# rubengooj/stvo-pl

Hardware: AMD Instinct MI355X
Metric: stereo frames/s (match+optimizePose) (higher is better)
Workload: dtype u8/fp4+f64; 1 GPU; BASELINE configs[2]: KITTI-00-shaped stereo with points + lines (ORB + LBD rows), grid-windowed stereo match (points and lines) + f2f brute-force mutual-NNR match (points and lines) + full GN optimizePose (config_kitti.yaml), device-resident per-frame pipeline; the streams cycle through the 8 sequence ids / 3 KITTI calibrations of configs[4] (sequence s on rank s mod G); streams_per_gpu=3072, parallelism=seq-shard x1

## Files before the change

stvo-pl_amd/csrc/ctx_internal.h:

```cpp
#pragma once
#include <hip/hip_runtime.h>

#include <cstdio>
#include <cstring>
#include <vector>

#include "kernels.h"

struct stvo_ctx {
    int device = 0;
    hipStream_t stream = nullptr;
    bool own_stream = false;
    bool stream_retained = false;
    int max_rows = 0, max_batch = 0;
    uint2* knn12 = nullptr;
    uint2* knn21 = nullptr;
    size_t knn_capacity = 0;
    int32_t *cand = nullptr, *need = nullptr, *qsel = nullptr, *nsel = nullptr;
    char* arena = nullptr;
    char* arena_host = nullptr;
    size_t arena_size = 0, arena_off = 0, upload_hi = 0;
    uint32_t* probe_sink = nullptr;
    int overlap = 0;
    hipStream_t aux_stream = nullptr;
    hipEvent_t ev_match_done = nullptr, ev_pose_done = nullptr;
    bool pose_pending = false;
    int timing = 0;
    std::vector<hipEvent_t> ev_pool;
    size_t ev_used = 0;
    char last_error[256] = {0};
};

namespace stvo_detail {

inline bool hip_ok(stvo_ctx* ctx, hipError_t e, const char* what) {
    if (e == hipSuccess) return true;
    if (ctx) std::snprintf(ctx->last_error, sizeof(ctx->last_error), "%s: %s", what, hipGetErrorString(e));
    return false;
}
#define HIP_TRY(ctx, call)                                   \
    do {                                                     \
        if (!hip_ok((ctx), (call), #call)) return STVO_ERR_HIP; \
    } while (0)

inline bool zero_device(stvo_ctx* ctx, void* p, size_t bytes, const char* what) {
    return hip_ok(ctx, hipMemsetAsync(p, 0, bytes, ctx->stream), what) && hip_ok(ctx, hipStreamSynchronize(ctx->stream), what);
}

inline bool upload_now(stvo_ctx* ctx, void* dst, const void* src, size_t bytes, const char* what) {
    return hip_ok(ctx, hipMemcpyAsync(dst, src, bytes, hipMemcpyHostToDevice, ctx->stream), what) && hip_ok(ctx, hipStreamSynchronize(ctx->stream), what);
}

template <typename T>
inline T* arena_alloc(stvo_ctx* ctx, size_t count) {
    size_t bytes = (count * sizeof(T) + 255) & ~size_t(255);
    if (bytes == 0) bytes = 256;
    if (ctx->arena_off + bytes > ctx->arena_size) return nullptr;
    T* p = reinterpret_cast<T*>(ctx->arena + ctx->arena_off);
    ctx->arena_off += bytes;
    return p;
}

template <typename T>
inline int upload(stvo_ctx* ctx, T** dst, const T* src, size_t count, size_t count_alloc = 0) {
    *dst = arena_alloc<T>(ctx, count_alloc > count ? count_alloc : count);
    if (!*dst) return STVO_ERR_CAPACITY;
    if (count && src) {
        const size_t off = (size_t)(reinterpret_cast<char*>(*dst) - ctx->arena);
        std::memcpy(ctx->arena_host + off, src, count * sizeof(T));
        if (off + count * sizeof(T) > ctx->upload_hi) ctx->upload_hi = off + count * sizeof(T);
    }
    return STVO_OK;
}

inline int flush_uploads(stvo_ctx* ctx) {
    if (ctx->upload_hi) {
        if (ctx->upload_hi <= ((size_t)4 << 20))
            stvo::launch_copy16(ctx->stream, ctx->arena_host, ctx->arena, ctx->upload_hi);
        else
            HIP_TRY(ctx, hipMemcpyAsync(ctx->arena, ctx->arena_host, ctx->upload_hi, hipMemcpyHostToDevice, ctx->stream));
        ctx->upload_hi = 0;
    }
    return STVO_OK;
}

inline int download_begin(stvo_ctx* ctx, const void* dev, size_t bytes) {
    const size_t off = (size_t)(reinterpret_cast<const char*>(dev) - ctx->arena);
    if (bytes == 0) return STVO_OK;
    if (bytes <= ((size_t)256 << 10) && (off & 15) == 0)
        stvo::launch_copy16(ctx->stream, dev, ctx->arena_host + off, bytes);
    else
        HIP_TRY(ctx, hipMemcpyAsync(ctx->arena_host + off, dev, bytes, hipMemcpyDeviceToHost, ctx->stream));
    return STVO_OK;
}
template <typename T>
inline const T* host_mirror(stvo_ctx* ctx, const T* dev) {
    return reinterpret_cast<const T*>(ctx->arena_host + (reinterpret_cast<const char*>(dev) - ctx->arena));
}
#define TRY(expr)                \
    do {                         \
        int _rc = (expr);        \
        if (_rc != STVO_OK) return _rc; \
    } while (0)

inline int check_launch(stvo_ctx* ctx) {
    HIP_TRY(ctx, hipGetLastError());
    return STVO_OK;
}

}
using namespace stvo_detail;
```

stvo-pl_amd/csrc/kernels.h:

```cpp
#pragma once

#include <hip/hip_runtime.h>
#include <stdint.h>

#include <cstdlib>
#include <map>
#include <mutex>
#include <utility>

#include "../../include/stvo_hip.h"
#include "debug_switches.h"
#include "point_tail.h"

namespace stvo {

inline bool lds_opt_in(const void* kernel, int bytes) {
    static std::mutex mu;
    static std::map<std::pair<const void*, int>, int> granted;
    int dev = 0;
    if (hipGetDevice(&dev) != hipSuccess) return false;
    std::lock_guard<std::mutex> lk(mu);
    const auto key = std::make_pair(kernel, dev);
    const auto it = granted.find(key);
    if (it != granted.end() && (it->second >= bytes || it->second < 0)) return it->second >= bytes;
    const bool ok = hipFuncSetAttribute(kernel, hipFuncAttributeMaxDynamicSharedMemorySize, bytes) == hipSuccess;
    if (ok) granted[key] = bytes;
    else if (it == granted.end()) granted[key] = -1;
    return ok;
}

constexpr int KNN_MIN_NSEG = 2, KNN_MAX_NSEG = 16;
inline int knn_pick_nseg(int B, int max_n, size_t capacity) {
    const int tiles = (max_n + 255) / 256;
    int nseg = (2048 + B * tiles - 1) / (B * tiles > 0 ? B * tiles : 1);
    nseg = nseg < KNN_MIN_NSEG ? KNN_MIN_NSEG : (nseg > KNN_MAX_NSEG ? KNN_MAX_NSEG : nseg);
    if ((long long)B * tiles >= 4096) nseg = 1;
    if (dbg().knn_nseg != DBG_UNSET && dbg().knn_nseg > 0) nseg = dbg().knn_nseg;
    const size_t per_seg = (size_t)(B > 0 ? B : 1) * (size_t)(max_n > 0 ? max_n : 1);
    while (nseg > 1 && (size_t)nseg * per_seg > capacity) --nseg;
    return nseg;
}

inline int device_cu_count() {
    static std::mutex mu;
    static std::map<int, int> cus;
    int dev = 0;
    if (hipGetDevice(&dev) != hipSuccess) return 256;
    std::lock_guard<std::mutex> lk(mu);
    const auto it = cus.find(dev);
    if (it != cus.end()) return it->second;
    int n = 0;
    if (hipDeviceGetAttribute(&n, hipDeviceAttributeMultiprocessorCount, dev) != hipSuccess || n <= 0) n = 256;
    cus[dev] = n;
    return n;
}

void launch_hamming_knn2(hipStream_t s, int B, int row_stride, int max_n, const uint8_t* d1, const int32_t* n1,
                         const uint8_t* d2, const int32_t* n2, uint2* knn12, uint2* knn21, int both_directions,
                         int lds_pad_bytes = 0, int dir0 = 0, const int32_t* qsel = nullptr,
                         const int32_t* nsel = nullptr, int nseg = KNN_MIN_NSEG, uint32_t* claim_init = nullptr);
constexpr int REV_MAX_SEG = 8;
__host__ __device__ inline int rev_segments(int train_rows) {
    const int s = (train_rows + 255) / 256;
    return s < 1 ? 1 : (s > REV_MAX_SEG ? REV_MAX_SEG : s);
}
void launch_hamming_knn2_mfma_reverse(hipStream_t s, int B, int row_stride, const uint8_t* d1, const int32_t* n1, const uint8_t* d2, const int32_t* qsel,
                                      const int32_t* nsel, const int32_t* tsel, const uint32_t* claim, float nnr, int32_t* m12, int slots);
void launch_hamming_knn2_mfma(hipStream_t s, int B, int row_stride, int max_n, const uint8_t* d1, const int32_t* n1,
                              const uint8_t* d2, const int32_t* n2, uint2* knn12, uint2* knn21, int both_directions,
                              int dir0, const int32_t* qsel, const int32_t* nsel, int nseg, uint32_t* claim_init, int qb,
                              int qsel_from_back = 0, const int32_t* tsel = nullptr, const int32_t* ntsel = nullptr);
int knn_mfma_qb(int max_n);
struct LazyScratch {
    uint2* knn12;
    uint2* knn21;
    int32_t* cand;
    int32_t* need;
    int32_t* qsel;
    int32_t* nsel;
    size_t knn_capacity;
};
void launch_match_mutual_lazy(hipStream_t s, int B, int row_stride, const uint8_t* d1, const int32_t* n1,
                              const uint8_t* d2, const int32_t* n2, float nnr, const LazyScratch& w, int32_t* m12,
                              int lds_pad_bytes, hipEvent_t wait_before_m12_write, hipEvent_t* timing_events = nullptr);
void launch_hamming_verify(hipStream_t s, int B, int row_stride, const uint8_t* d1, const int32_t* n1, const uint8_t* d2,
                           float nnr, const LazyScratch& w, int lds_pad_bytes, int nseg, int32_t* m12);
bool match_small_ok(int row_stride);
void launch_match_small(hipStream_t s, int B, int row_stride, const uint8_t* d1, const int32_t* n1, const uint8_t* d2,
                        const int32_t* n2, float nnr, int mutual, int32_t* m12, int cap = 0 );
void launch_nnr_mutual(hipStream_t s, int B, int row_stride, const uint2* knn12, const uint2* knn21, const int32_t* n1,
                       const int32_t* n2, float nnr, int mutual, int32_t* m12, int nseg = KNN_MIN_NSEG);
void launch_valu_probe(hipStream_t s, int blocks, int iters, uint32_t* sink);
void launch_copy16(hipStream_t s, const void* src, void* dst, size_t bytes);
extern const double kValuProbeOpsPerThreadIter;

struct PoseArgs {
    int B, max_pts, max_lines;
    const int32_t* n_prev_pts;
    const double* prev_P;
    const double* prev_s2p;
    const double* curr_pl;
    const int32_t* m12p;
    const int32_t* init_inl_p;
    const int32_t* n_prev_lines;
    const double* prev_sP;
    const double* prev_eP;
    const double* prev_spl;
    const double* prev_epl;
    const double* prev_s2l;
    const double* curr_le;
    const int32_t* m12l;
    const int32_t* init_inl_l;
    const double* init_T;
    double* next_T;
    stvo_cam cam;
    const stvo_cam* cams;
    int lds_cap_pts, lds_cap_lines;
    stvo_opt_params prm;
    stvo_pose_result* results;
    int32_t* inl_p_out;
    int32_t* inl_l_out;
    int eval_only;
    int eval_robust;
    double* eval_out;
    long long* prof_out;
    const float4* prev_rc;
    const float4* curr_rc;
    const double* q_tab;
    double level_scale;
    const unsigned* wait_flag;
    unsigned wait_value;
    int lazy_eig;
    int lines_on_solver;
    const uint4* fetch_src;
    uint4* fetch_dst;
    unsigned fetch_n16;
    unsigned* fetch_flag;
    unsigned fetch_value;
    unsigned* start_flag;
    unsigned start_value;
};
bool pose_start_flag_ok(const PoseArgs& a);
void launch_stream_gate(hipStream_t s, const unsigned* flag, unsigned value);
constexpr int STVO_POSE_QTAB = 16;
constexpr int PATH_EIG_PENDING = 1 << 30;
bool pose_inline_sync_ok(int B);
void launch_stream_signal(hipStream_t s, unsigned* flag, unsigned value);
int launch_pose(hipStream_t s, const PoseArgs& a);
int launch_pose2p(hipStream_t s, const PoseArgs& a);
void pose2p_retain_stream(hipStream_t s);
void pose2p_release_stream(hipStream_t s);
inline void pose_retain_stream(hipStream_t s) { pose2p_retain_stream(s); }
inline void pose_release_stream(hipStream_t s) { pose2p_release_stream(s); }

void launch_blur7_u8(hipStream_t s, int B, int cols, int rows, const uint8_t* src, uint8_t* dst, const int* k7);
void launch_resize_linear_u8(hipStream_t s, int B, int scols, int srows, int dcols, int drows, const uint8_t* src, uint8_t* dst, double fx = 0.0,
                             double fy = 0.0);

constexpr int GRID_LW = STVO_GRID_COLS + 16, GRID_LCELLS = STVO_GRID_ROWS * GRID_LW, GRID_LSTART_STRIDE = GRID_LCELLS + 4;
struct PointCells {
    int K, ws;
    const float* kp_l;
    const float* kp_r;
    const int32_t* n_kp_l;
    const int32_t* n_kp_r;
    const double* inv_wh;
    int32_t* pstart;
    uint32_t* plstart;
    int32_t* plperm;
    int32_t* pperm;
    int32_t* pcell;
    int32_t* pxy_l;
    unsigned long long* top2_p;
    int32_t* govf_p;
    int32_t* prange;
    int32_t* pitems;
    int32_t* prank;
};

struct GridBatch {
    int B, stride1, stride2;
    int xy_width;
    int items_stride;
    int words64, n1p;
    const int32_t* cell_xy1;
    const uint8_t* d1;
    const int32_t* n1;
    const int32_t* cell_start;
    const int32_t* cell_items;
    const uint8_t* d2;
    const int32_t* n2;
    const double* dir2;
    stvo_grid_window w;
    double ratio, line_sim_th;
    int mutual;
    unsigned long long* cover;
    const int32_t* rank;
    const int32_t* perm;
    unsigned long long* top2;
    int32_t* owner2;
    int32_t* m12;
    int range_points;
    const int32_t* range1;
    const int32_t* cell2;
    const uint32_t* lstart;
    const int32_t* lperm;
    uint32_t* elig;
    int32_t* elig_cnt;
    int32_t* ovf;
    int32_t* misfit;
    int lean_cells;
    int has_tail;
    PointTail tail;
    int fused_cells;
    PointCells cells;
};
constexpr int GRID_ELIG = 16;
void launch_grid_batch(hipStream_t s, const GridBatch& g, bool lines, hipEvent_t* scan_events = nullptr);
bool grid_points_fused_ok(const GridBatch& g);
void launch_grid_range_debug(hipStream_t s, const GridBatch& g);

}
```

stvo-pl_amd/csrc/match_kernels.hip:

```cpp
#include "kernels.h"

#include <stdlib.h>

namespace stvo {

__device__ __forceinline__ uint32_t med3_u32(uint32_t a, uint32_t b, uint32_t c) {
    uint32_t r;
    asm("v_med3_u32 %0, %1, %2, %3" : "=v"(r) : "v"(a), "v"(b), "v"(c));
    return r;
}

__device__ __forceinline__ uint32_t bcnt_acc(uint32_t x, uint32_t acc) {
    uint32_t r;
    asm("v_bcnt_u32_b32 %0, %1, %2" : "=v"(r) : "v"(x), "v"(acc));
    return r;
}
__device__ __forceinline__ uint32_t pack_key(uint32_t d, uint32_t j_uniform) {
    uint32_t r;
    asm("v_lshl_or_b32 %0, %1, 16, %2" : "=v"(r) : "v"(d), "s"(j_uniform));
    return r;
}
__device__ __forceinline__ uint32_t bcnt0(uint32_t x) {
    uint32_t r;
    asm("v_bcnt_u32_b32 %0, %1, 0" : "=v"(r) : "v"(x));
    return r;
}

__device__ __forceinline__ uint32_t hamming256(const uint4& q0, const uint4& q1, const uint32_t* __restrict__ t) {
    uint32_t d = bcnt0(q0.x ^ t[0]);
    d = bcnt_acc(q0.y ^ t[1], d);
    d = bcnt_acc(q0.z ^ t[2], d);
    d = bcnt_acc(q0.w ^ t[3], d);
    d = bcnt_acc(q1.x ^ t[4], d);
    d = bcnt_acc(q1.y ^ t[5], d);
    d = bcnt_acc(q1.z ^ t[6], d);
    d = bcnt_acc(q1.w ^ t[7], d);
    return d;
}

constexpr int KNN_BLOCK = 256;

__device__ __forceinline__ uint2 merged_knn(const uint2* __restrict__ knn, size_t seg_stride, size_t idx, int nseg) {
    uint2 r = knn[idx];
    for (int sgm = 1; sgm < nseg; ++sgm) {
        const uint2 o = knn[(size_t)sgm * seg_stride + idx];
        const uint32_t hi = r.x > o.x ? r.x : o.x;
        uint32_t sec = r.y < o.y ? r.y : o.y;
        sec = sec < hi ? sec : hi;
        r.x = r.x < o.x ? r.x : o.x;
        r.y = sec;
    }
    return r;
}

__global__ __launch_bounds__(KNN_BLOCK) void hamming_knn2_kernel(int B, int tiles, int ndir, int dir0, int nseg, int row_stride,
                                                                 const uint8_t* __restrict__ d1,
                                                                 const int32_t* __restrict__ n1,
                                                                 const uint8_t* __restrict__ d2,
                                                                 const int32_t* __restrict__ n2,
                                                                 uint2* __restrict__ knn12, uint2* __restrict__ knn21,
                                                                 const int32_t* __restrict__ qsel,
                                                                 const int32_t* __restrict__ nsel,
                                                                 uint32_t* __restrict__ claim_init) {
    const int per_frame = tiles * ndir * nseg;
    const int L = blockIdx.x;
    const int xcd = L & 7, k = L >> 3;
    const int b = (k / per_frame) * 8 + xcd;
    if (b >= B) return;
    const int local = k % per_frame;
    const int seg = local % nseg;
    const int dir = dir0 + (local / nseg) / tiles;
    const int tile = (local / nseg) % tiles;
    const int na = n1[b], nb = n2[b];
    const int nq = qsel ? nsel[b] : (dir == 0 ? na : nb);
    const int nt_all = dir == 0 ? nb : na;
    const int seg_len = (((nt_all + nseg - 1) / nseg) + 3) & ~3;
    const int j0 = min(seg * seg_len, nt_all);
    const int nt = min(j0 + seg_len, nt_all);
    const int q_base = tile * KNN_BLOCK;
    const size_t frame_off = (size_t)b * row_stride;
    if (claim_init && seg == 0 && dir == dir0 && q_base + (int)threadIdx.x < row_stride)
        claim_init[frame_off + q_base + threadIdx.x] = 0xFFFFFFFFu;
    if (q_base + (int)(threadIdx.x & ~63u) >= nq) return;
    const uint8_t* Q = (dir == 0 ? d1 : d2) + frame_off * STVO_DESC_BYTES;
    const uint32_t* __restrict__ T = reinterpret_cast<const uint32_t*>((dir == 0 ? d2 : d1) + frame_off * STVO_DESC_BYTES);
    uint2* __restrict__ out = (dir == 0 ? knn12 : knn21) + (size_t)seg * B * row_stride + frame_off;

    const int q = q_base + threadIdx.x;
    const int qc = q < nq ? q : nq - 1;
    const int qi = qsel ? qsel[frame_off + qc] : qc;
    const uint4 q0 = reinterpret_cast<const uint4*>(Q)[2 * qi];
    const uint4 q1 = reinterpret_cast<const uint4*>(Q)[2 * qi + 1];

    uint32_t best = 0xFFFFFFFFu, second = 0xFFFFFFFFu;
    uint32_t second_d = 0xFFFFu;
    int j = j0;
    auto update = [&](uint32_t d, uint32_t jj) {
        if (__builtin_amdgcn_ballot_w64(d < second_d) != 0ull) {
            const uint32_t key = pack_key(d, jj);
            second = med3_u32(best, second, key);
            best = best < key ? best : key;
            second_d = second >> 16;
        }
    };
    for (; j + 4 <= nt; j += 4) {
        uint32_t t[32];
#pragma unroll
        for (int k = 0; k < 32; ++k) t[k] = T[8 * j + k];
        uint32_t d[4];
#pragma unroll
        for (int u = 0; u < 4; ++u) d[u] = hamming256(q0, q1, t + 8 * u);
#pragma unroll
        for (int u = 0; u < 4; ++u) update(d[u], (uint32_t)(j + u));
    }
    for (; j < nt; ++j) update(hamming256(q0, q1, T + 8 * j), (uint32_t)j);
    if (q < nq) out[qi] = make_uint2(best, second);
}

int knn_mfma_qb(int max_n) {
    const int qb = dbg().knn_mfma != DBG_UNSET ? dbg().knn_mfma : 2;
    return max_n <= 8192 ? qb : 0;
}

void launch_hamming_knn2(hipStream_t s, int B, int row_stride, int max_n, const uint8_t* d1, const int32_t* n1,
                         const uint8_t* d2, const int32_t* n2, uint2* knn12, uint2* knn21, int both_directions,
                         int lds_pad_bytes, int dir0, const int32_t* qsel, const int32_t* nsel, int nseg, uint32_t* claim_init) {
    if (B <= 0 || max_n <= 0) return;
    const int mfma_qb = knn_mfma_qb(max_n);
    if (mfma_qb > 0) {
        launch_hamming_knn2_mfma(s, B, row_stride, max_n, d1, n1, d2, n2, knn12, knn21, both_directions, dir0, qsel, nsel, nseg,
                                 claim_init, mfma_qb);
        return;
    }
    const int tiles = (max_n + KNN_BLOCK - 1) / KNN_BLOCK, ndir = both_directions ? 2 : 1;
    const int groups = (B + 7) / 8;
    dim3 grid((unsigned)(groups * 8 * tiles * ndir * nseg));
    hipLaunchKernelGGL(hamming_knn2_kernel, grid, dim3(KNN_BLOCK), (size_t)lds_pad_bytes, s, B, tiles, ndir, dir0,
                       nseg, row_stride, d1, n1, d2, n2, knn12, knn21, qsel, nsel, claim_init);
}

__global__ __launch_bounds__(256) void nnr_mutual_kernel(int nseg, int row_stride, const uint2* __restrict__ knn12,
                                                         const uint2* __restrict__ knn21,
                                                         const int32_t* __restrict__ n1, const int32_t* __restrict__ n2,
                                                         float nnr, int mutual, int32_t* __restrict__ m12) {
    const int b = blockIdx.y;
    const int i = blockIdx.x * 256 + threadIdx.x;
    if (i >= row_stride) return;
    const int na = n1[b], nb = n2[b];
    const size_t off = (size_t)b * row_stride;
    int m = -1;
    if (i < na && nb >= 2) {
        const uint2 k = merged_knn(knn12, (size_t)gridDim.y * row_stride, off + i, nseg);
        const float f0 = (float)(k.x >> 16), f1 = (float)(k.y >> 16);
        if (f0 < f1 * nnr) m = (int)(k.x & 0xFFFFu);
        if (mutual && m >= 0) {
            bool keep = false;
            if (na >= 2) {
                const uint2 r = merged_knn(knn21, (size_t)gridDim.y * row_stride, off + m, nseg);
                const float r0 = (float)(r.x >> 16), r1 = (float)(r.y >> 16);
                keep = (r0 < r1 * nnr) && ((int)(r.x & 0xFFFFu) == i);
            }
            if (!keep) m = -1;
        }
    }
    m12[off + i] = m;
}

void launch_nnr_mutual(hipStream_t s, int B, int row_stride, const uint2* knn12, const uint2* knn21, const int32_t* n1,
                       const int32_t* n2, float nnr, int mutual, int32_t* m12, int nseg) {
    if (B <= 0 || row_stride <= 0) return;
    dim3 grid((row_stride + 255) / 256, B);
    hipLaunchKernelGGL(nnr_mutual_kernel, grid, dim3(256), 0, s, nseg, row_stride, knn12, knn21, n1, n2, nnr, mutual, m12);
}

__global__ __launch_bounds__(256) void nnr_forward_kernel(int nseg, int row_stride, const uint2* __restrict__ knn12,
                                                          const int32_t* __restrict__ n1, const int32_t* __restrict__ n2,
                                                          float nnr, int32_t* __restrict__ cand,
                                                          uint32_t* __restrict__ claim ) {
    const int b = blockIdx.y;
    const int i = blockIdx.x * 256 + threadIdx.x;
    if (i >= row_stride) return;
    const int na = n1[b], nb = n2[b];
    const size_t off = (size_t)b * row_stride;
    int m = -1;
    if (i < na && nb >= 2) {
        const uint2 k = merged_knn(knn12, (size_t)gridDim.y * row_stride, off + i, nseg);
        const float f0 = (float)(k.x >> 16), f1 = (float)(k.y >> 16);
        if (f0 < f1 * nnr) {
            m = (int)(k.x & 0xFFFFu);
            atomicMin(&claim[off + m], (k.x & 0xFFFF0000u) | (uint32_t)i);
        }
    }
    cand[off + i] = m;
}

__global__ __launch_bounds__(256) void compact_need_kernel(int row_stride, const uint32_t* __restrict__ claim,
                                                           const int32_t* __restrict__ n2, int32_t* __restrict__ qsel,
                                                           int32_t* __restrict__ nsel, int32_t* __restrict__ blocked) {
    __shared__ int s_wave[4];
    const int b = blockIdx.x, tid = threadIdx.x, lane = tid & 63, wv = tid >> 6;
    const size_t off = (size_t)b * row_stride;
    const int nb = n2[b];
    const int per = (row_stride + 255) / 256;
    const int lo = tid * per, hi = min(lo + per, nb);
    int cnt = 0;
    for (int j = lo; j < hi; ++j) cnt += claim[off + j] != 0xFFFFFFFFu;
    int incl = cnt;
#pragma unroll
    for (int o = 1; o < 64; o <<= 1) {
        const int v = __shfl_up(incl, o, 64);
        if (lane >= o) incl += v;
    }
    if (lane == 63) s_wave[wv] = incl;
    __syncthreads();
    int base = 0, tot = 0;
#pragma unroll
    for (int w = 0; w < 4; ++w) {
        if (w < wv) base += s_wave[w];
        tot += s_wave[w];
    }
    int pos = base + incl - cnt;
    for (int j = lo; j < hi; ++j)
        if (claim[off + j] != 0xFFFFFFFFu) {
            qsel[off + pos++] = j;
            blocked[off + j] = 0;
        }
    if (tid == 0) nsel[b] = tot;
}

__device__ __forceinline__ uint32_t hamming128_lo(const uint4& q0, const uint32_t* __restrict__ t) {
    uint32_t d = bcnt0(q0.x ^ t[0]);
    d = bcnt_acc(q0.y ^ t[1], d);
    d = bcnt_acc(q0.z ^ t[2], d);
    d = bcnt_acc(q0.w ^ t[3], d);
    return d;
}
__device__ __forceinline__ uint32_t hamming128_hi(const uint4& q1, const uint32_t* __restrict__ t, uint32_t d) {
    d = bcnt_acc(q1.x ^ t[4], d);
    d = bcnt_acc(q1.y ^ t[5], d);
    d = bcnt_acc(q1.z ^ t[6], d);
    d = bcnt_acc(q1.w ^ t[7], d);
    return d;
}

__global__ __launch_bounds__(KNN_BLOCK) void hamming_verify_kernel(int B, int tiles, int nseg, int row_stride,
                                                                   const uint8_t* __restrict__ d1,
                                                                   const int32_t* __restrict__ n1,
                                                                   const uint8_t* __restrict__ d2,
                                                                   const uint32_t* __restrict__ claim,
                                                                   const int32_t* __restrict__ qsel,
                                                                   const int32_t* __restrict__ nsel, float nnr,
                                                                   int32_t* __restrict__ blocked) {
    const int per_frame = tiles * nseg;
    const int L = blockIdx.x;
    const int xcd = L & 7, k = L >> 3;
    const int b = (k / per_frame) * 8 + xcd;
    if (b >= B) return;
    const int local = k % per_frame;
    const int seg = local % nseg;
    const int tile = local / nseg;
    const int nq = nsel[b];
    const int nt_all = n1[b];
    const int seg_len = (((nt_all + nseg - 1) / nseg) + 3) & ~3;
    const int j0 = min(seg * seg_len, nt_all);
    const int nt = min(j0 + seg_len, nt_all);
    const int q_base = tile * KNN_BLOCK;
    if (q_base + (int)(threadIdx.x & ~63u) >= nq) return;
    const size_t frame_off = (size_t)b * row_stride;
    const uint32_t* __restrict__ T = reinterpret_cast<const uint32_t*>(d1 + frame_off * STVO_DESC_BYTES);

    const int q = q_base + threadIdx.x;
    const int qc = q < nq ? q : nq - 1;
    const int qi = qsel[frame_off + qc];
    const uint4 q0 = reinterpret_cast<const uint4*>(d2 + frame_off * STVO_DESC_BYTES)[2 * qi];
    const uint4 q1 = reinterpret_cast<const uint4*>(d2 + frame_off * STVO_DESC_BYTES)[2 * qi + 1];
    const uint32_t c = claim[frame_off + qi];
    const uint32_t istar = c & 0xFFFFu;
    uint32_t thr = c >> 16;
    {
        const float f0 = (float)thr;
        while (thr < 256u && !(f0 < (float)(thr + 1u) * nnr)) ++thr;
    }
    bool blk = false;
    auto step4 = [&](const uint32_t* __restrict__ t, int jb) {
        uint32_t p[4];
#pragma unroll
        for (int u = 0; u < 4; ++u) p[u] = hamming128_lo(q0, t + 8 * u);
        unsigned long long any = 0ull;
#pragma unroll
        for (int u = 0; u < 4; ++u) any |= __builtin_amdgcn_ballot_w64(p[u] <= thr);
        if (any != 0ull) {
            unsigned long long other = 0ull;
#pragma unroll
            for (int u = 0; u < 4; ++u) other |= __builtin_amdgcn_ballot_w64(p[u] <= thr && (uint32_t)(jb + u) != istar);
            if (other != 0ull) {
#pragma unroll
                for (int u = 0; u < 4; ++u) {
                    const uint32_t d = hamming128_hi(q1, t + 8 * u, p[u]);
                    blk = blk || (d <= thr && (uint32_t)(jb + u) != istar);
                }
            }
        }
    };
    int j = j0;
    if (j + 4 <= nt) {
        uint32_t ta[32], tb[32];
#pragma unroll
        for (int w = 0; w < 32; ++w) ta[w] = T[8 * j + w];
        for (; j + 8 <= nt; j += 8) {
#pragma unroll
            for (int w = 0; w < 32; ++w) tb[w] = T[8 * (j + 4) + w];
            step4(ta, j);
            const int jn = (j + 12 <= nt) ? j + 8 : j;
#pragma unroll
            for (int w = 0; w < 32; ++w) ta[w] = T[8 * jn + w];
            step4(tb, j + 4);
        }
        if (j + 4 <= nt) {
            step4(ta, j);
            j += 4;
        }
    }
    for (; j < nt; ++j) {
        const uint32_t d = hamming256(q0, q1, T + 8 * j);
        blk = blk || (d <= thr && (uint32_t)j != istar);
    }
    if (q < nq && blk) blocked[frame_off + qi] = 1;
}

__global__ __launch_bounds__(1024) void nnr_reverse_check_kernel(int row_stride, const uint32_t* __restrict__ claim,
                                                                 const int32_t* __restrict__ blocked, const int32_t* __restrict__ n1,
                                                                 int32_t* __restrict__ m12) {
    const int b = blockIdx.x;
    const size_t off = (size_t)b * row_stride;
    for (int i = threadIdx.x; i < row_stride; i += 1024) m12[off + i] = -1;
    __syncthreads();
    if (n1[b] < 2) return;
    for (int j = threadIdx.x; j < row_stride; j += 1024) {
        const uint32_t c = claim[off + j];
        if (c != 0xFFFFFFFFu && blocked[off + j] == 0) m12[off + (c & 0xFFFFu)] = j;
    }
}

__device__ __forceinline__ uint32_t block_threshold(uint32_t d0, float nnr) {
    const float f0 = (float)d0;
    uint32_t thr = d0;
    while (thr < 256u && !(f0 < (float)(thr + 1u) * nnr)) ++thr;
    return thr;
}

constexpr int PLAN_BLOCK = 512;
__global__ __launch_bounds__(PLAN_BLOCK) void forward_plan_kernel(int B, int nseg, int row_stride, uint2* __restrict__ knn12,
                                                                  const int32_t* __restrict__ n1,
                                                                  const int32_t* __restrict__ n2, float nnr,
                                                                  int32_t* __restrict__ m12, uint32_t* __restrict__ claim_g,
                                                                  int32_t* __restrict__ qsel, int32_t* __restrict__ tsel,
                                                                  int32_t* __restrict__ nsel) {
    extern __shared__ uint32_t plan_lds[];
    uint32_t* claim = plan_lds;
    uint16_t* Tc = reinterpret_cast<uint16_t*>(claim + row_stride);
    uint8_t* blk = reinterpret_cast<uint8_t*>(Tc + row_stride);
    __shared__ int hT[257], hS[257], s_cnt[3];
    __shared__ unsigned long long s_best;
    const int b = blockIdx.x, tid = threadIdx.x;
    const size_t off = (size_t)b * row_stride;
    const int na = n1[b], nb = n2[b];
    for (int j = tid; j < row_stride; j += PLAN_BLOCK) {
        claim[j] = 0xFFFFFFFFu;
        blk[j] = 0;
    }
    if (tid < 257) hT[tid] = hS[tid] = 0;
    if (tid < 3) s_cnt[tid] = 0;
    if (tid == 0) s_best = ~0ull;
    __syncthreads();
    const bool active = nb >= 2 && na >= 1;
    for (int i = tid; i < row_stride; i += PLAN_BLOCK) {
        if (active && i < na) {
            const uint2 k = merged_knn(knn12, (size_t)B * row_stride, off + i, nseg);
            if (nseg > 1) knn12[off + i] = k;
            const float f0 = (float)(k.x >> 16), f1 = (float)(k.y >> 16);
            if (f0 < f1 * nnr) atomicMin(&claim[k.x & 0xFFFFu], (k.x & 0xFFFF0000u) | (uint32_t)i);
        }
        m12[off + i] = -1;
    }
    __syncthreads();
    for (int j = tid; j < row_stride; j += PLAN_BLOCK) {
        const uint32_t c = claim[j];
        claim_g[off + j] = c;
        if (c != 0xFFFFFFFFu) {
            const uint32_t T = block_threshold(c >> 16, nnr);
            Tc[j] = (uint16_t)T;
            atomicAdd(&hT[T], 1);
        }
    }
    __syncthreads();
    if (active)
        for (int i = tid; i < na; i += PLAN_BLOCK) {
            const uint2 k = knn12[off + i];
            const uint32_t key[2] = {k.x, k.y};
#pragma unroll
            for (int e = 0; e < 2; ++e) {
                if (key[e] == 0xFFFFFFFFu) continue;
                const uint32_t j = key[e] & 0xFFFFu, c = claim[j];
                if (c != 0xFFFFFFFFu && (c & 0xFFFFu) != (uint32_t)i && (key[e] >> 16) <= (uint32_t)Tc[j]) blk[j] = 1;
            }
            if (k.y != 0xFFFFFFFFu) atomicAdd(&hS[min(k.y >> 16, 256u)], 1);
        }
    __syncthreads();
    if (tid < 64) {
        int vT[5], vS[5], sT = 0, sS = 0;
#pragma unroll
        for (int e = 0; e < 5; ++e) {
            const int t = tid * 5 + e;
            vT[e] = t < 257 ? hT[t] : 0;
            vS[e] = t < 257 ? hS[t] : 0;
            sT += vT[e];
            sS += vS[e];
        }
        int iT = sT, iS = sS;
#pragma unroll
        for (int o = 1; o < 64; o <<= 1) {
            const int a = __shfl_up(iT, o, 64), c = __shfl_up(iS, o, 64);
            if (tid >= o) {
                iT += a;
                iS += c;
            }
        }
        int eT = iT - sT, eS = iS - sS;
#pragma unroll
        for (int e = 0; e < 5; ++e) {
            const int t = tid * 5 + e;
            if (t < 257) {
                hT[t] = eT;
                hS[t] = eS;
            }
            eT += vT[e];
            eS += vS[e];
        }
        if (tid == 63) s_cnt[0] = iT;
    }
    __syncthreads();
    if (tid < 256) {
        const int C = s_cnt[0], cT = hT[tid], cS = hS[tid];
        const unsigned long long cost = (unsigned long long)(C - cT) * (unsigned)na + (unsigned long long)cT * (unsigned)cS;
        atomicMin(&s_best, (cost << 9) | (unsigned)tid);
    }
    __syncthreads();
    if (tid == 0) s_cnt[0] = 0;
    __syncthreads();
    const int tau = (int)(s_best & 511ull) - 1;
    for (int j = tid; j < row_stride; j += PLAN_BLOCK) {
        const uint32_t c = claim[j];
        if (c == 0xFFFFFFFFu) continue;
        if (!blk[j] && na >= 2) m12[off + (c & 0xFFFFu)] = j;
        if ((int)Tc[j] <= tau)
            qsel[off + atomicAdd(&s_cnt[0], 1)] = j;
        else
            qsel[off + row_stride - 1 - atomicAdd(&s_cnt[1], 1)] = j;
    }
    if (active)
        for (int i = tid; i < na; i += PLAN_BLOCK) {
            const uint2 k = knn12[off + i];
            if (k.y != 0xFFFFFFFFu && (int)(k.y >> 16) <= tau) tsel[off + atomicAdd(&s_cnt[2], 1)] = i;
        }
    __syncthreads();
    if (tid == 0) {
        nsel[b] = s_cnt[0] + s_cnt[1];
        nsel[(size_t)B + b] = s_cnt[0];
        nsel[2 * (size_t)B + b] = s_cnt[1];
        nsel[3 * (size_t)B + b] = s_cnt[2];
        nsel[4 * (size_t)B + b] = tau;
    }
}

struct ReversePlan {
    int32_t* tsel;
};
constexpr int KNN_REV_SLOTS = 4;
static ReversePlan reverse_plan(const LazyScratch& w, int B, int row_stride) {
    const size_t per = (size_t)B * row_stride;
    ReversePlan p;
    p.tsel = reinterpret_cast<int32_t*>(w.knn21 + (w.knn_capacity - per)) + per;
    return p;
}

static void launch_reverse_scans(hipStream_t s, int B, int row_stride, const uint8_t* d1, const int32_t* n1, const uint8_t* d2, float nnr,
                                 const LazyScratch& w, const ReversePlan& rp, int32_t* m12) {
    launch_hamming_knn2_mfma_reverse(s, B, row_stride, d1, n1, d2, w.qsel, w.nsel, rp.tsel, reinterpret_cast<const uint32_t*>(w.need), nnr, m12,
                                     KNN_REV_SLOTS);
}

void launch_hamming_verify(hipStream_t s, int B, int row_stride, const uint8_t* d1, const int32_t* n1, const uint8_t* d2,
                           float nnr, const LazyScratch& w, int lds_pad_bytes, int nseg, int32_t* m12) {
    if (B <= 0 || row_stride <= 0) return;
    const int mfma_qb = knn_mfma_qb(row_stride);
    if (mfma_qb > 0) {
        launch_reverse_scans(s, B, row_stride, d1, n1, d2, nnr, w, reverse_plan(w, B, row_stride), m12);
        return;
    }
    const int tiles = (row_stride + KNN_BLOCK - 1) / KNN_BLOCK, groups = (B + 7) / 8;
    hipLaunchKernelGGL(hamming_verify_kernel, dim3((unsigned)(groups * 8 * tiles * nseg)), dim3(KNN_BLOCK),
                       (size_t)lds_pad_bytes, s, B, tiles, nseg, row_stride, d1, n1, d2,
                       reinterpret_cast<const uint32_t*>(w.need), w.qsel, w.nsel, nnr, reinterpret_cast<int32_t*>(w.knn21));
}

void launch_match_mutual_lazy(hipStream_t s, int B, int row_stride, const uint8_t* d1, const int32_t* n1,
                              const uint8_t* d2, const int32_t* n2, float nnr, const LazyScratch& w, int32_t* m12,
                              int lds_pad_bytes, hipEvent_t wait_before_m12_write, hipEvent_t* tev) {
    if (B <= 0 || row_stride <= 0) return;
    const dim3 grid2((row_stride + 255) / 256, B);
    const int nseg = knn_pick_nseg(B, row_stride, w.knn_capacity);
    uint32_t* claim = reinterpret_cast<uint32_t*>(w.need);
    int32_t* blocked = reinterpret_cast<int32_t*>(w.knn21);
    if (tev) (void)hipEventRecord(tev[0], s);
    launch_hamming_knn2(s, B, row_stride, row_stride, d1, n1, d2, n2, w.knn12, w.knn21, 0, lds_pad_bytes, 0, nullptr,
                        nullptr, nseg, knn_mfma_qb(row_stride) > 0 ? nullptr : claim);
    if (tev) (void)hipEventRecord(tev[1], s);
    const int mfma_qb = knn_mfma_qb(row_stride);
    if (mfma_qb > 0) {
        const ReversePlan rp = reverse_plan(w, B, row_stride);
        if (wait_before_m12_write) (void)hipStreamWaitEvent(s, wait_before_m12_write, 0);
        if (tev && tev[2]) (void)hipEventRecord(tev[2], s);
        hipLaunchKernelGGL(forward_plan_kernel, dim3(B), dim3(PLAN_BLOCK), (size_t)row_stride * 7, s, B, nseg, row_stride, w.knn12,
                           n1, n2, nnr, m12, claim, w.qsel, rp.tsel, w.nsel);
        launch_reverse_scans(s, B, row_stride, d1, n1, d2, nnr, w, rp, m12);
        if (tev && tev[3]) (void)hipEventRecord(tev[3], s);
        return;
    }
    hipLaunchKernelGGL(nnr_forward_kernel, grid2, dim3(256), 0, s, nseg, row_stride, w.knn12, n1, n2, nnr, w.cand, claim);
    hipLaunchKernelGGL(compact_need_kernel, dim3(B), dim3(256), 0, s, row_stride, claim, n2, w.qsel, w.nsel, blocked);
    if (tev && tev[2]) (void)hipEventRecord(tev[2], s);
    launch_hamming_verify(s, B, row_stride, d1, n1, d2, nnr, w, lds_pad_bytes, nseg, m12);
    if (tev && tev[3]) (void)hipEventRecord(tev[3], s);
    if (wait_before_m12_write) (void)hipStreamWaitEvent(s, wait_before_m12_write, 0);
    hipLaunchKernelGGL(nnr_reverse_check_kernel, dim3(B), dim3(1024), 0, s, row_stride, claim, blocked, n1, m12);
}

const double kValuProbeOpsPerThreadIter = 19.0 * 8.0;

__global__ __launch_bounds__(256) void valu_probe_kernel(int iters, uint32_t* sink) {
    uint4 q0 = make_uint4(threadIdx.x * 2654435761u, blockIdx.x * 40503u + 1u, 0x9E3779B9u ^ threadIdx.x, 0x85EBCA6Bu);
    uint4 q1 = make_uint4(q0.y * 3u, q0.z * 5u, q0.w * 7u, q0.x * 11u);
    uint32_t best = 0xFFFFFFFFu, second = 0xFFFFFFFFu;
    uint32_t t[8];
    const uint32_t seed = __builtin_amdgcn_readfirstlane(blockIdx.x * 7919u + 13u);
#pragma unroll
    for (int k = 0; k < 8; ++k) t[k] = seed * (2 * k + 3);
    for (int it = 0; it < iters; ++it) {
#pragma unroll
        for (int u = 0; u < 8; ++u) {
#pragma unroll
            for (int k = 0; k < 8; ++k) t[k] = __builtin_amdgcn_readfirstlane(t[k] + 0x01010101u * (k + 1));
            const uint32_t d = hamming256(q0, q1, t);
            const uint32_t key = pack_key(d, (uint32_t)(it * 8 + u));
            second = med3_u32(best, second, key);
            best = best < key ? best : key;
        }
    }
    if ((best ^ second) == 0x12345u) sink[0] = best;
}

__global__ __launch_bounds__(256) void copy16_kernel(const uint4* __restrict__ src, uint4* __restrict__ dst, size_t n16) {
    for (size_t i = (size_t)blockIdx.x * 256 + threadIdx.x; i < n16; i += (size_t)gridDim.x * 256) dst[i] = src[i];
}

void launch_copy16(hipStream_t s, const void* src, void* dst, size_t bytes) {
    const size_t n16 = (bytes + 15) / 16;
    if (n16 == 0) return;
    const size_t blocks = (n16 + 255) / 256;
    hipLaunchKernelGGL(copy16_kernel, dim3((unsigned)(blocks < 256 ? blocks : 256)), dim3(256), 0, s,
                       reinterpret_cast<const uint4*>(src), reinterpret_cast<uint4*>(dst), n16);
}

void launch_valu_probe(hipStream_t s, int blocks, int iters, uint32_t* sink) {
    hipLaunchKernelGGL(valu_probe_kernel, dim3(blocks), dim3(256), 0, s, iters, sink);
}

__global__ __launch_bounds__(256) void match_small_kernel(int row_stride, int cap, const uint8_t* __restrict__ d1,
                                                          const int32_t* __restrict__ n1, const uint8_t* __restrict__ d2,
                                                          const int32_t* __restrict__ n2, float nnr, int mutual,
                                                          int32_t* __restrict__ m12) {
    extern __shared__ uint2 s_knn[];
    const int b = blockIdx.x, tid = threadIdx.x, lane = tid & 63;
    const int na = min(n1[b], cap), nb = min(n2[b], cap);
    const size_t off = (size_t)b * row_stride;
    uint2* k12 = s_knn;
    uint2* k21 = s_knn + cap;
    const int tiles_a = (na + 63) >> 6, tiles_b = mutual ? (nb + 63) >> 6 : 0;
    for (int item = tid >> 6; item < tiles_a + tiles_b; item += 4) {
        const int it = __builtin_amdgcn_readfirstlane(item);
        const bool fwd = it < tiles_a;
        const int q = (fwd ? it : it - tiles_a) * 64 + lane;
        const int nq = fwd ? na : nb, nt = fwd ? nb : na;
        const uint8_t* Q = (fwd ? d1 : d2) + off * STVO_DESC_BYTES;
        const uint32_t* __restrict__ T = reinterpret_cast<const uint32_t*>((fwd ? d2 : d1) + off * STVO_DESC_BYTES);
        const int qc = q < nq ? q : nq - 1;
        const uint4 q0 = reinterpret_cast<const uint4*>(Q)[2 * qc];
        const uint4 q1 = reinterpret_cast<const uint4*>(Q)[2 * qc + 1];
        uint32_t best = 0xFFFFFFFFu, second = 0xFFFFFFFFu;
        auto update = [&](uint32_t d, uint32_t jj) {
            const uint32_t key = pack_key(d, jj);
            second = med3_u32(best, second, key);
            best = best < key ? best : key;
        };
        int j = 0;
        for (; j + 4 <= nt; j += 4) {
            uint32_t t[32];
#pragma unroll
            for (int k = 0; k < 32; ++k) t[k] = T[8 * j + k];
            uint32_t d[4];
#pragma unroll
            for (int u = 0; u < 4; ++u) d[u] = hamming256(q0, q1, t + 8 * u);
#pragma unroll
            for (int u = 0; u < 4; ++u) update(d[u], (uint32_t)(j + u));
        }
        for (; j < nt; ++j) update(hamming256(q0, q1, T + 8 * j), (uint32_t)j);
        if (q < nq) (fwd ? k12 : k21)[q] = make_uint2(best, second);
    }
    __syncthreads();
    for (int i = tid; i < row_stride; i += 256) {
        int m = -1;
        if (i < na && nb >= 2) {
            const uint2 fk = k12[i];
            const float f0 = (float)(fk.x >> 16), f1 = (float)(fk.y >> 16);
            if (f0 < f1 * nnr) m = (int)(fk.x & 0xFFFFu);
            if (mutual && m >= 0) {
                bool keep = false;
                if (na >= 2) {
                    const uint2 rk = k21[m];
                    const float r0 = (float)(rk.x >> 16), r1 = (float)(rk.y >> 16);
                    keep = (r0 < r1 * nnr) && ((int)(rk.x & 0xFFFFu) == i);
                }
                if (!keep) m = -1;
            }
        }
        m12[off + i] = m;
    }
}

bool match_small_ok(int row_stride) { return row_stride > 0 && row_stride <= 512; }

void launch_match_small(hipStream_t s, int B, int row_stride, const uint8_t* d1, const int32_t* n1, const uint8_t* d2,
                        const int32_t* n2, float nnr, int mutual, int32_t* m12, int cap) {
    if (B <= 0 || !match_small_ok(row_stride)) return;
    if (cap <= 0 || cap > row_stride) cap = row_stride;
    const size_t lds = (size_t)cap * 2 * sizeof(uint2);
    hipLaunchKernelGGL(match_small_kernel, dim3(B), dim3(256), lds, s, row_stride, cap, d1, n1, d2, n2, nnr, mutual, m12);
}

}
```

stvo-pl_amd/csrc/match_mfma.hip:

```cpp
#include <type_traits>

#include "kernels.h"

namespace stvo {

typedef int v4i __attribute__((ext_vector_type(4)));
typedef int v8i __attribute__((ext_vector_type(8)));
typedef int v16i __attribute__((ext_vector_type(16)));
typedef float v16f __attribute__((ext_vector_type(16)));

#ifndef MF_TPB
#define MF_TPB 2
#endif
#ifndef MF_FOLD_SLOTS
#define MF_FOLD_SLOTS 5
#endif
constexpr int MF_BLOCK = 256;
constexpr int MF_TILE = 32;
constexpr int MF_KEY_SHIFT = 13;
constexpr int MF_KEY_BIAS = 1 << 20;
constexpr int MF_NO_KEY = 0x7FFFFFFF;
constexpr int MF_NO_KEY_MIN = 0x40000000;

__device__ __forceinline__ v4i expand_fp4(uint32_t w) {
    v4i r;
    r.x = (int)(((w << 3) & 0x88888888u) | 0x66666666u);
    r.y = (int)(((w << 2) & 0x88888888u) | 0x66666666u);
    r.z = (int)(((w << 1) & 0x88888888u) | 0x66666666u);
    r.w = (int)((w & 0x88888888u) | 0x66666666u);
    return r;
}
__device__ __forceinline__ float med3_f32(float a, float b, float c) {
    float r;
    asm("v_med3_f32 %0, %1, %2, %3" : "=v"(r) : "v"(a), "v"(b), "v"(c));
    return r;
}
__device__ __forceinline__ float min_f32(float a, float b) {
    float r;
    asm("v_min_f32 %0, %1, %2" : "=v"(r) : "v"(a), "v"(b));
    return r;
}
__device__ __forceinline__ float max_f32(float a, float b) {
    float r;
    asm("v_max_f32 %0, %1, %2" : "=v"(r) : "v"(a), "v"(b));
    return r;
}
__device__ __forceinline__ float min3_f32(float a, float b, float c) {
    float r;
    asm("v_min3_f32 %0, %1, %2, %3" : "=v"(r) : "v"(a), "v"(b), "v"(c));
    return r;
}
constexpr float MF_NO_KEY_F = 1.0e30f;
constexpr float MF_NO_KEY_MIN_F = 1.0e29f;
constexpr int MF_SCALE_2_4 = 127 + 4;

__device__ __forceinline__ uint32_t key_to_knn(int key, int base) {
    if (key >= MF_NO_KEY_MIN) return 0xFFFFFFFFu;
    const uint32_t u = (uint32_t)(key + base + MF_KEY_BIAS);
    return ((u >> MF_KEY_SHIFT) << 16) | (u & ((1u << MF_KEY_SHIFT) - 1u));
}

template <int QB, int MODE>
__global__ __launch_bounds__(MF_BLOCK, (QB == 1 ? 4 : QB == 2 ? 3 : 1)) void hamming_knn2_mfma_kernel(int B, int tiles, int ndir, int dir0, int nseg, int row_stride,
                                                                      const uint8_t* __restrict__ d1,
                                                                      const int32_t* __restrict__ n1,
                                                                      const uint8_t* __restrict__ d2,
                                                                      const int32_t* __restrict__ n2,
                                                                      uint2* __restrict__ knn12, uint2* __restrict__ knn21,
                                                                      const int32_t* __restrict__ qsel,
                                                                      const int32_t* __restrict__ nsel,
                                                                      uint32_t* __restrict__ claim_init, int qsel_from_back,
                                                                      const int32_t* __restrict__ tsel,
                                                                      const int32_t* __restrict__ ntsel) {
    constexpr bool GATHER = MODE >= 1, TGATHER = MODE == 2;
    constexpr int ROWS = 4 * QB * 32;
    constexpr int KSTEPS = 4;
    using key_t = float;
    using acc_t = v16f;
    constexpr int NBUF = 2 * MF_TPB;
    __shared__ v4i s_tile[NBUF][KSTEPS * 2 * 32];
    const int per_frame = tiles * ndir * nseg;
    const int L = blockIdx.x;
    const int xcd = L & 7, k = L >> 3;
    int fb = k / per_frame, local = k % per_frame;
    if (MODE == 0 && ndir == 1 && tiles > 1) {
        const int groups = (int)(gridDim.x >> 3) / per_frame;
        const int full_pf = (tiles - 1) * nseg, full = full_pf * groups;
        if (k < full) {
            fb = k / full_pf;
            local = k % full_pf;
        } else {
            fb = (k - full) / nseg;
            local = full_pf + (k - full) % nseg;
        }
    }
    const int b = fb * 8 + xcd;
    if (b >= B) return;
    const int seg = local % nseg;
    const int dir = dir0 + (local / nseg) / tiles;
    const int tile = (local / nseg) % tiles;
    const size_t frame_off = (size_t)b * row_stride;
    const int tid = threadIdx.x, lane = tid & 63, wv = tid >> 6, col = lane & 31, hf = lane >> 5;
    const int q_base = tile * ROWS;
    const uint32_t* __restrict__ Q = reinterpret_cast<const uint32_t*>((dir == 0 ? d1 : d2) + frame_off * STVO_DESC_BYTES);
    uint4 qw[QB][2];
    if (!GATHER) {
#pragma unroll
        for (int qb = 0; qb < QB; ++qb) {
            const int qi = min(q_base + (wv * QB + qb) * 32 + col, row_stride - 1);
            qw[qb][0] = reinterpret_cast<const uint4*>(Q)[2 * qi];
            qw[qb][1] = reinterpret_cast<const uint4*>(Q)[2 * qi + 1];
        }
    }
    const int na = n1[b], nb = n2[b];
    const int nq = GATHER ? nsel[b] : (dir == 0 ? na : nb);
    const int nt_all = TGATHER ? ntsel[b] : (dir == 0 ? nb : na);
    if (TGATHER && nt_all == 0) return;
    const int seg_len = (((nt_all + nseg - 1) / nseg) + MF_TILE - 1) & ~(MF_TILE - 1);
    const int j0 = min(seg * seg_len, nt_all);
    const int nt = min(j0 + seg_len, nt_all);
    if (claim_init && seg == 0 && dir == dir0)
        for (int c = q_base + tid; c < min(q_base + ROWS, row_stride); c += MF_BLOCK) claim_init[frame_off + c] = 0xFFFFFFFFu;
    if (q_base >= nq) return;
    const uint32_t* __restrict__ T = reinterpret_cast<const uint32_t*>((dir == 0 ? d2 : d1) + frame_off * STVO_DESC_BYTES);
    uint2* __restrict__ out = (dir == 0 ? knn12 : knn21) + (size_t)seg * B * row_stride + frame_off;

    const bool wave_active = q_base + wv * QB * 32 < nq;
    v4i qf[QB][KSTEPS];
    auto query_row = [&](int qb) {
        const int q = q_base + (wv * QB + qb) * 32 + col;
        const int qc = q < nq ? q : nq - 1;
        return GATHER ? qsel[frame_off + (qsel_from_back ? row_stride - 1 - qc : qc)] : qc;
    };
    if (GATHER) {
#pragma unroll
        for (int qb = 0; qb < QB; ++qb) {
            const int qi = query_row(qb);
            qw[qb][0] = reinterpret_cast<const uint4*>(Q)[2 * qi];
            qw[qb][1] = reinterpret_cast<const uint4*>(Q)[2 * qi + 1];
        }
    }
#pragma unroll
    for (int qb = 0; qb < QB; ++qb) {
        const uint32_t w[8] = {qw[qb][0].x, qw[qb][0].y, qw[qb][0].z, qw[qb][0].w, qw[qb][1].x, qw[qb][1].y, qw[qb][1].z, qw[qb][1].w};
        const bool up = hf != 0;
        qf[qb][0] = expand_fp4(~(up ? w[1] : w[0]));
        qf[qb][1] = expand_fp4(~(up ? w[3] : w[2]));
        qf[qb][2] = expand_fp4(~(up ? w[5] : w[4]));
        qf[qb][3] = expand_fp4(~(up ? w[7] : w[6]));
    }
    acc_t cidx;
#pragma unroll
    for (int r = 0; r < 16; ++r) cidx[r] = (key_t)((r & 3) + 8 * (r >> 2) + 4 * hf);

    const key_t no_key = MF_NO_KEY_F;
    key_t best[QB], second[QB];
#pragma unroll
    for (int qb = 0; qb < QB; ++qb) best[qb] = second[qb] = no_key;

    const int xr = tid & 31, xk = tid >> 5;
    const int ntiles = (nt - j0 + MF_TILE - 1) / MF_TILE;
    auto fetch = [&](int t) -> uint32_t {
        const int j = j0 + t * MF_TILE + xr;
        if (j >= nt) return 0u;
        const int row = TGATHER ? tsel[frame_off + j] : j;
        return T[(size_t)row * 8 + xk];
    };
    auto stage = [&](int t, uint32_t w) {
        s_tile[t & (NBUF - 1)][xk * 32 + xr] = expand_fp4(w);
    };
#pragma unroll
    for (int i = 0; i < MF_TPB; ++i)
        if (i < ntiles) stage(i, fetch(i));
    __syncthreads();
    auto rebase = [&]() {
#pragma unroll
        for (int qb = 0; qb < QB; ++qb) {
            best[qb] -= (key_t)MF_TILE;
            second[qb] -= (key_t)MF_TILE;
        }
    };
    auto fold = [&](int qb, key_t key) {
        second[qb] = med3_f32(best[qb], second[qb], key);
        best[qb] = min_f32(best[qb], key);
    };
    auto mma = [&](const v4i& tf, const v4i& q, const acc_t& c) -> acc_t {
        const v8i a8 = {tf.x, tf.y, tf.z, tf.w, 0, 0, 0, 0}, b8 = {q.x, q.y, q.z, q.w, 0, 0, 0, 0};
        return __builtin_amdgcn_mfma_scale_f32_32x32x64_f8f6f4(a8, b8, c, 4, 4, 0, MF_SCALE_2_4, 0, MF_SCALE_2_4);
    };
    auto mma_fold = [&](acc_t (&cur)[QB], acc_t (&prev)[QB], int t) {
        if (wave_active) {
            const v4i* frag = s_tile[t & (NBUF - 1)];
            const bool fold_prev = t > 0;
            if (fold_prev) rebase();
            key_t node[QB][5];
            v4i tf = frag[lane];
#pragma unroll
            for (int kk = 0; kk < KSTEPS; ++kk) {
                v4i tf_ahead = tf;
                if (kk < KSTEPS - 1) tf_ahead = frag[(kk + 1) * 64 + lane];
#pragma unroll
                for (int qb = 0; qb < QB; ++qb) cur[qb] = mma(tf, qf[qb][kk], kk == 0 ? cidx : cur[qb]);
                if (fold_prev) {
                    if (QB == 1 && kk == 0) asm volatile("s_nop 7\n\ts_nop 7\n\ts_nop 2" : "+v"(prev[0]));
#pragma unroll
                    for (int qb = 0; qb < QB; ++qb) {
                        const acc_t& p = prev[qb];
                        key_t(&a)[5] = node[qb];
                        if (kk == 0) {
                            a[0] = min3_f32(p[0], p[1], p[2]);
                            a[1] = min3_f32(p[3], p[4], p[5]);
                            second[qb] = min3_f32(second[qb], med3_f32(p[0], p[1], p[2]), med3_f32(p[3], p[4], p[5]));
                        } else if (kk == 1) {
                            a[2] = min3_f32(p[6], p[7], p[8]);
                            a[3] = min3_f32(p[9], p[10], p[11]);
                            second[qb] = min3_f32(second[qb], med3_f32(p[6], p[7], p[8]), med3_f32(p[9], p[10], p[11]));
                        } else if (kk == 2) {
                            a[4] = min3_f32(p[12], p[13], p[14]);
                            const key_t b0 = min3_f32(a[0], a[1], a[2]);
                            second[qb] = min3_f32(second[qb], med3_f32(p[12], p[13], p[14]), med3_f32(a[0], a[1], a[2]));
                            a[0] = b0;
                        } else {
                            const key_t b1 = min3_f32(a[3], a[4], p[15]), n1 = med3_f32(a[3], a[4], p[15]);
                            second[qb] = min3_f32(second[qb], n1, med3_f32(a[0], b1, best[qb]));
                            best[qb] = min3_f32(a[0], b1, best[qb]);
                        }
                    }
                }
                if (kk < KSTEPS - 1) __builtin_amdgcn_sched_group_barrier(0x100, 1, 0);
#pragma unroll
                for (int qb = 0; qb < QB; ++qb) {
                    __builtin_amdgcn_sched_group_barrier(0x008, 1, 0);
                    __builtin_amdgcn_sched_group_barrier(0x002, MF_FOLD_SLOTS, 0);
                }
                tf = tf_ahead;
            }
        }
    };
    acc_t accA[QB], accB[QB];
#pragma unroll
    for (int qb = 0; qb < QB; ++qb)
#pragma unroll
        for (int r = 0; r < 16; ++r) accA[qb][r] = accB[qb][r] = 0;
    static_assert(MF_TPB % 2 == 0, "the accumulator sets alternate tile by tile");
    int t = 0;
    uint32_t w_near[MF_TPB];
#pragma unroll
    for (int i = 0; i < MF_TPB; ++i) {
        w_near[i] = 0;
        if (MF_TPB + i < ntiles) w_near[i] = fetch(MF_TPB + i);
    }
    for (; t + MF_TPB <= ntiles; t += MF_TPB) {
        uint32_t w_far[MF_TPB];
#pragma unroll
        for (int i = 0; i < MF_TPB; ++i) {
            w_far[i] = 0;
            if (t + 2 * MF_TPB + i < ntiles) w_far[i] = fetch(t + 2 * MF_TPB + i);
        }
#pragma unroll
        for (int i = 0; i < MF_TPB; ++i) {
            if ((i & 1) == 0) mma_fold(accA, accB, t + i);
            else mma_fold(accB, accA, t + i);
        }
#pragma unroll
        for (int i = 0; i < MF_TPB; ++i) {
            if (t + MF_TPB + i < ntiles) stage(t + MF_TPB + i, w_near[i]);
            w_near[i] = w_far[i];
        }
        __syncthreads();
    }
#pragma unroll
    for (int i = 0; i < MF_TPB - 1; ++i)
        if (t + i < ntiles) {
            if ((i & 1) == 0) mma_fold(accA, accB, t + i);
            else mma_fold(accB, accA, t + i);
        }
    if (wave_active && ntiles > 0) {
        const int jt = j0 + (ntiles - 1) * MF_TILE;
        const acc_t(&last)[QB] = (ntiles & 1) ? accA : accB;
        rebase();
#pragma unroll
        for (int qb = 0; qb < QB; ++qb)
#pragma unroll
            for (int r = 0; r < 16; ++r) {
                const int jr = jt + (r & 3) + 8 * (r >> 2) + 4 * hf;
                fold(qb, jr < nt ? last[qb][r] : no_key);
            }
    }
    if (!wave_active) return;
#pragma unroll
    for (int qb = 0; qb < QB; ++qb) {
        const int bi = best[qb] >= MF_NO_KEY_MIN_F ? MF_NO_KEY : (int)best[qb];
        const int si = second[qb] >= MF_NO_KEY_MIN_F ? MF_NO_KEY : (int)second[qb];
        const int ob = __shfl_xor(bi, 32), os = __shfl_xor(si, 32);
        const int hi = max(bi, ob);
        const int sec = min(min(si, os), hi);
        const int bst = min(bi, ob);
        const int q = q_base + (wv * QB + qb) * 32 + col;
        const int base = j0 + (ntiles - 1) * MF_TILE;
        if (hf == 0 && q < nq) out[query_row(qb)] = make_uint2(key_to_knn(bst, base), key_to_knn(sec, base));
    }
}

constexpr int REV_CHUNK_TILES = 8, REV_CHUNK = REV_CHUNK_TILES * MF_TILE;

__global__ __launch_bounds__(MF_BLOCK, 4) void hamming_knn2_mfma_reverse_kernel(int B, int slots, int row_stride, const uint8_t* __restrict__ d1,
                                                                                const int32_t* __restrict__ n1, const uint8_t* __restrict__ d2,
                                                                                const int32_t* __restrict__ qsel, const int32_t* __restrict__ nsel,
                                                                                const int32_t* __restrict__ tsel, const uint32_t* __restrict__ claim,
                                                                                float nnr, int32_t* __restrict__ m12) {
    constexpr int KSTEPS = 4;
    using key_t = float;
    using acc_t = v16f;
    __shared__ v4i s_tile[REV_CHUNK_TILES][KSTEPS * 2 * 32];
    __shared__ uint16_t s_thr[257];
    const int L = blockIdx.x;
    const int xcd = L & 7, k = L >> 3;
    const int b = (k / slots) * 8 + xcd, slot = k % slots;
    if (b >= B) return;
    const int na = n1[b];
    const int nl = nsel[(size_t)B + b], nh = nsel[2 * (size_t)B + b], ns = nsel[3 * (size_t)B + b];
    if ((ns == 0 || nl == 0) && nh == 0) return;
    {
        const float f0 = (float)threadIdx.x;
        uint32_t thr = threadIdx.x;
        while (thr < 256u && !(f0 < (float)(thr + 1u) * nnr)) ++thr;
        s_thr[threadIdx.x] = (uint16_t)thr;
        if (threadIdx.x == 0) s_thr[256] = 256;
    }
    const size_t frame_off = (size_t)b * row_stride;
    const int tid = threadIdx.x, lane = tid & 63, wv = tid >> 6, col = lane & 31, hf = lane >> 5;
    const int xr = tid & 31, xk = tid >> 5;
    const uint32_t* __restrict__ Q = reinterpret_cast<const uint32_t*>(d2 + frame_off * STVO_DESC_BYTES);
    const uint32_t* __restrict__ T = reinterpret_cast<const uint32_t*>(d1 + frame_off * STVO_DESC_BYTES);
    acc_t cidx;
#pragma unroll
    for (int r = 0; r < 16; ++r) cidx[r] = (key_t)((r & 3) + 8 * (r >> 2) + 4 * hf);
    auto mma = [&](const v4i& tf, const v4i& q, const acc_t& c) -> acc_t {
        const v8i a8 = {tf.x, tf.y, tf.z, tf.w, 0, 0, 0, 0}, b8 = {q.x, q.y, q.z, q.w, 0, 0, 0, 0};
        return __builtin_amdgcn_mfma_scale_f32_32x32x64_f8f6f4(a8, b8, c, 4, 4, 0, MF_SCALE_2_4, 0, MF_SCALE_2_4);
    };

    for (int list = 0; list < 2; ++list) {
        const bool light = list == 0;
        const int nq = light ? (ns > 0 ? nl : 0) : nh, nt_all = light ? ns : na;
        if (nq == 0) continue;
        const int nseg = rev_segments(nt_all);
        const int n_groups = (nq + 127) / 128;
        const int seg_len = (((nt_all + nseg - 1) / nseg) + MF_TILE - 1) & ~(MF_TILE - 1);
        auto column_of = [&](int g) -> int {
            const int q = (g * 4 + wv) * 32 + col;
            return q < nq ? q : nq - 1;
        };
        auto list_entry = [&](int g) -> int { return qsel[frame_off + (light ? column_of(g) : row_stride - 1 - column_of(g))]; };
        for (int seg = 0; seg < nseg; ++seg) {
            const int g_first = ((slot - seg) % slots + slots) % slots;
            if (g_first >= n_groups) continue;
            const int j0 = min(seg * seg_len, nt_all), nt = min(j0 + seg_len, nt_all);
            for (int c0 = j0; c0 < nt || c0 == j0; c0 += REV_CHUNK) {
                uint32_t w[REV_CHUNK_TILES];
#pragma unroll
                for (int t = 0; t < REV_CHUNK_TILES; ++t) {
                    const int j = c0 + t * MF_TILE + xr;
                    uint32_t v = 0u;
                    if (j < nt) v = T[(size_t)(light ? tsel[frame_off + j] : j) * 8 + xk];
                    w[t] = v;
                }
                int e_cur = list_entry(g_first);
                int e_next = g_first + slots < n_groups ? list_entry(g_first + slots) : 0;
                const int ntc = min((nt - c0 + MF_TILE - 1) / MF_TILE, REV_CHUNK_TILES);
#pragma unroll
                for (int t = 0; t < REV_CHUNK_TILES; ++t)
                    if (t < ntc) s_tile[t][xk * 32 + xr] = expand_fp4(w[t]);
                uint4 qw0 = reinterpret_cast<const uint4*>(Q)[2 * e_cur], qw1 = reinterpret_cast<const uint4*>(Q)[2 * e_cur + 1];
                uint32_t cw = claim[frame_off + e_cur];
                __syncthreads();
                for (int g = g_first; g < n_groups; g += slots) {
                    const bool up = hf != 0;
                    v4i qf[KSTEPS];
                    qf[0] = expand_fp4(~(up ? qw0.y : qw0.x));
                    qf[1] = expand_fp4(~(up ? qw0.w : qw0.z));
                    qf[2] = expand_fp4(~(up ? qw1.y : qw1.x));
                    qf[3] = expand_fp4(~(up ? qw1.w : qw1.z));
                    const uint32_t c_claim = cw;
                    const bool block_active = (g * 4 + wv) * 32 < nq;
                    if (g + slots < n_groups) {
                        qw0 = reinterpret_cast<const uint4*>(Q)[2 * e_next];
                        qw1 = reinterpret_cast<const uint4*>(Q)[2 * e_next + 1];
                        cw = claim[frame_off + e_next];
                        e_cur = e_next;
                        if (g + 2 * slots < n_groups) e_next = list_entry(g + 2 * slots);
                    }
                    if (!block_active) continue;
                    key_t best = MF_NO_KEY_F, second = MF_NO_KEY_F;
                    auto fold = [&](key_t key) {
                        second = med3_f32(best, second, key);
                        best = min_f32(best, key);
                    };
                    int last_base = c0;
                    if (ntc > 0) {
                        auto do_tile = [&](acc_t& cur, acc_t& prev, int t) {
                            key_t nd[5];
                            const v4i* frag = s_tile[t];
                            const bool fold_prev = t > 0;
                            if (fold_prev) {
                                best -= (key_t)MF_TILE;
                                second -= (key_t)MF_TILE;
                            }
                            v4i tf = frag[lane];
#pragma unroll
                            for (int kk = 0; kk < KSTEPS; ++kk) {
                                v4i tf_ahead = tf;
                                if (kk < KSTEPS - 1) tf_ahead = frag[(kk + 1) * 64 + lane];
                                cur = mma(tf, qf[kk], kk == 0 ? cidx : cur);
                                if (fold_prev) {
                                    if (kk == 0) {
                                        asm volatile("s_nop 7\n\ts_nop 7\n\ts_nop 2" : "+v"(prev));
                                        nd[0] = min3_f32(prev[0], prev[1], prev[2]);
                                        nd[1] = min3_f32(prev[3], prev[4], prev[5]);
                                        second = min3_f32(second, med3_f32(prev[0], prev[1], prev[2]), med3_f32(prev[3], prev[4], prev[5]));
                                    } else if (kk == 1) {
                                        nd[2] = min3_f32(prev[6], prev[7], prev[8]);
                                        nd[3] = min3_f32(prev[9], prev[10], prev[11]);
                                        second = min3_f32(second, med3_f32(prev[6], prev[7], prev[8]), med3_f32(prev[9], prev[10], prev[11]));
                                    } else if (kk == 2) {
                                        nd[4] = min3_f32(prev[12], prev[13], prev[14]);
                                        const key_t b0 = min3_f32(nd[0], nd[1], nd[2]);
                                        second = min3_f32(second, med3_f32(prev[12], prev[13], prev[14]), med3_f32(nd[0], nd[1], nd[2]));
                                        nd[0] = b0;
                                    } else {
                                        const key_t b1 = min3_f32(nd[3], nd[4], prev[15]), n1 = med3_f32(nd[3], nd[4], prev[15]);
                                        second = min3_f32(second, n1, med3_f32(nd[0], b1, best));
                                        best = min3_f32(nd[0], b1, best);
                                    }
                                }
                                if (kk < KSTEPS - 1) __builtin_amdgcn_sched_group_barrier(0x100, 1, 0);
                                __builtin_amdgcn_sched_group_barrier(0x008, 1, 0);
                                __builtin_amdgcn_sched_group_barrier(0x002, MF_FOLD_SLOTS, 0);
                                tf = tf_ahead;
                            }
                        };
                        acc_t accA, accB;
#pragma unroll
                        for (int r = 0; r < 16; ++r) accA[r] = accB[r] = 0;
                        int t = 0;
                        for (; t + 2 <= ntc; t += 2) {
                            do_tile(accA, accB, t);
                            do_tile(accB, accA, t + 1);
                        }
                        if (t < ntc) do_tile(accA, accB, t);
                        acc_t& last = (ntc & 1) ? accA : accB;
                        asm volatile("s_nop 7\n\ts_nop 7\n\ts_nop 2" : "+v"(last));
                        best -= (key_t)MF_TILE;
                        second -= (key_t)MF_TILE;
                        last_base = c0 + (ntc - 1) * MF_TILE;
#pragma unroll
                        for (int r = 0; r < 16; ++r) {
                            const int jr = last_base + (r & 3) + 8 * (r >> 2) + 4 * hf;
                            fold(jr < nt ? last[r] : MF_NO_KEY_F);
                        }
                    }
                    const int bi = best >= MF_NO_KEY_MIN_F ? MF_NO_KEY : (int)best;
                    const int si = second >= MF_NO_KEY_MIN_F ? MF_NO_KEY : (int)second;
                    const int ob = __shfl_xor(bi, 32), os = __shfl_xor(si, 32);
                    const int hi = max(bi, ob);
                    const int sec = min(min(si, os), hi);
                    const int bst = min(bi, ob);
                    if (hf == 0 && (g * 4 + wv) * 32 + col < nq) {
                        const uint32_t x = key_to_knn(bst, last_base), y = key_to_knn(sec, last_base);
                        if (x != 0xFFFFFFFFu) {
                            const uint32_t T = s_thr[c_claim >> 16], istar = c_claim & 0xFFFFu;
                            bool blk = false;
                            if ((x >> 16) <= T) {
                                const uint32_t pos = x & 0xFFFFu;
                                const uint32_t row = light ? (uint32_t)tsel[frame_off + pos] : pos;
                                blk = row != istar || (y != 0xFFFFFFFFu && (y >> 16) <= T);
                            }
                            if (blk) m12[frame_off + istar] = -1;
                        }
                    }
                }
                __syncthreads();
            }
        }
    }
}

void launch_hamming_knn2_mfma_reverse(hipStream_t s, int B, int row_stride, const uint8_t* d1, const int32_t* n1, const uint8_t* d2, const int32_t* qsel,
                                      const int32_t* nsel, const int32_t* tsel, const uint32_t* claim, float nnr, int32_t* m12, int slots) {
    if (B <= 0 || row_stride <= 0) return;
    const dim3 grid((unsigned)(((B + 7) / 8) * 8 * slots));
    hipLaunchKernelGGL(hamming_knn2_mfma_reverse_kernel, grid, dim3(MF_BLOCK), 0, s, B, slots, row_stride, d1, n1, d2, qsel, nsel, tsel, claim, nnr, m12);
}

int mfma_rows_per_block(int qb) { return 4 * qb * 32; }

template <int QB, int MODE>
static void launch_mf(dim3 grid, hipStream_t s, int B, int tiles, int ndir, int dir0, int nseg, int row_stride, const uint8_t* d1,
                      const int32_t* n1, const uint8_t* d2, const int32_t* n2, uint2* knn12, uint2* knn21, const int32_t* qsel,
                      const int32_t* nsel, uint32_t* claim_init, int qsel_from_back, const int32_t* tsel, const int32_t* ntsel) {
    hipLaunchKernelGGL((hamming_knn2_mfma_kernel<QB, MODE>), grid, dim3(MF_BLOCK), 0, s, B, tiles, ndir, dir0, nseg, row_stride, d1, n1, d2, n2,
                       knn12, knn21, qsel, nsel, claim_init, qsel_from_back, tsel, ntsel);
}

void launch_hamming_knn2_mfma(hipStream_t s, int B, int row_stride, int max_n, const uint8_t* d1, const int32_t* n1,
                              const uint8_t* d2, const int32_t* n2, uint2* knn12, uint2* knn21, int both_directions,
                              int dir0, const int32_t* qsel, const int32_t* nsel, int nseg, uint32_t* claim_init, int qb,
                              int qsel_from_back, const int32_t* tsel, const int32_t* ntsel) {
    if (B <= 0 || max_n <= 0) return;
    const int rows = mfma_rows_per_block(qb);
    const int tiles = (max_n + rows - 1) / rows, ndir = both_directions ? 2 : 1;
    const int groups = (B + 7) / 8;
    const dim3 grid((unsigned)(groups * 8 * tiles * ndir * nseg));
#define STVO_MF_ARGS grid, s, B, tiles, ndir, dir0, nseg, row_stride, d1, n1, d2, n2, knn12, knn21, qsel, nsel, claim_init, qsel_from_back, tsel, ntsel
    if (qsel || tsel) return;
    if (qb == 1) launch_mf<1, 0>(STVO_MF_ARGS);
    else if (qb == 2) launch_mf<2, 0>(STVO_MF_ARGS);
    else launch_mf<4, 0>(STVO_MF_ARGS);
#undef STVO_MF_ARGS
}

}
```

stvo-pl_amd/csrc/seq_pipeline.hip:

```cpp
#include <algorithm>
#include <atomic>
#include <chrono>
#include <cstdio>
#include <cstdlib>
#include <vector>

#include "ctx_internal.h"
#include "point_cells.h"
#include "pose_math.h"

#pragma clang fp contract(off)

namespace stvo {
namespace {

constexpr int LENT = STVO_GRID_COLS + STVO_GRID_ROWS + 4;

struct SeqDev {
    int B, K, M;
    const stvo_cam* cams;
    const double* inv_wh;
    stvo_match_params mp;
    const float* kp_l;
    const int32_t* oct_l;
// ... 386 lines not shown
    auto in_window = [&](int j, int row_off, int q) -> bool {
        const uint32_t run = __builtin_amdgcn_perm(0u, (uint32_t)rows[row_off + j], 0x0c010c00u);
        const i16x2 d = __builtin_bit_cast(i16x2, q) - __builtin_bit_cast(i16x2, run);
        return (__builtin_bit_cast(uint32_t, d) & 0x80008000u) == 0u;
    };
    const int words = (nl + 31) >> 5;
    for (int e = tid; e < words * M; e += T) {
        const int w = e / M, j = e - w * M;
        uint32_t bits = 0u;
        if (j < nr) {
            const int i_end = min(32, nl - 32 * w);
#pragma unroll 4
            for (int k = 0; k < i_end; ++k) {
                const int4 c = cxy[32 * w + k];
                if (in_window(j, c.x, c.y) || in_window(j, c.z, c.w)) bits |= 1u << k;
            }
        }
        cand[e] = bits;
    }
    __syncthreads();
    auto walk = [&](int j, const u32x4 t0, const u32x4 t1, const double dirx, const double diry, auto f) {
        int run_min = 0x7FFFFFFF;
        for (int w = 0; w < words; ++w) {
            for (uint32_t bits = cand[w * M + j]; bits; bits &= bits - 1u) {
                const int i1 = 32 * w + __builtin_ctz(bits);
                const double2 v = vdir[i1];
                const double dot = v.x * dirx + v.y * diry;
                if (fabs(dot) < sim_th) continue;
                const u32x4 q0 = dl[2 * i1], q1 = dl[2 * i1 + 1];
                const int d = __builtin_popcount(q0.x ^ t0.x) + __builtin_popcount(q0.y ^ t0.y) + __builtin_popcount(q0.z ^ t0.z) +
                              __builtin_popcount(q0.w ^ t0.w) + __builtin_popcount(q1.x ^ t1.x) + __builtin_popcount(q1.y ^ t1.y) +
                              __builtin_popcount(q1.z ^ t1.z) + __builtin_popcount(q1.w ^ t1.w);
                if (mutual) {
                    if (d >= run_min) continue;
                    run_min = d;
                }
                f(i1, d);
            }
        }
    };
    auto right_line = [&](int j, u32x4& t0, u32x4& t1, double& dirx, double& diry) {
        const float* kl = s.kl_r + (off + j) * 4;
        const double vx = (double)(kl[2] - kl[0]) * inv_w;
        const double vy = (double)(kl[3] - kl[1]) * inv_h;
        const double mag = sqrt(vx * vx + vy * vy);
        dirx = vx / mag;
        diry = vy / mag;
        const u32x4* g = reinterpret_cast<const u32x4*>(s.ldesc_r + (off + j) * STVO_DESC_BYTES);
        t0 = g[0];
        t1 = g[1];
    };
    for (int j = tid; j < nr; j += T) {
        u32x4 t0, t1;
        double dirx, diry;
        right_line(j, t0, t1, dirx, diry);
        int own = 0xFFFF;
        walk(j, t0, t1, dirx, diry, [&](int i1, int d) {
            own = i1;
            atomicMin(&best[i1], ((uint32_t)d << 16) | (uint32_t)j);
        });
        owner[j] = (unsigned short)own;
    }
    __syncthreads();
    for (int j = tid; j < nr; j += T) {
        u32x4 t0, t1;
        double dirx, diry;
        right_line(j, t0, t1, dirx, diry);
        walk(j, t0, t1, dirx, diry, [&](int i1, int d) {
            const uint32_t bk = best[i1];
            if (bk != (((uint32_t)d << 16) | (uint32_t)j)) {
                const double best_d = (double)(int)(bk >> 16), d2 = (double)d;
                if (!(best_d < d2 * ratio)) blocked[i1] = 1;
            }
        });
    }
    __syncthreads();
    for (int i1 = tid; i1 < s.M; i1 += T) {
        int m = -1;
        if (i1 < nl) {
            const uint32_t bk = best[i1];
            if (bk != 0xFFFFFFFFu && !blocked[i1] && (double)(int)(bk >> 16) < 2147483647.0 * ratio) {
                const int j = (int)(bk & 0xFFFFu);
                if (!mutual || (int)owner[j] == i1) m = j;
            }
        }
        if (i1 < M) mm[i1] = (short)m;
        const_cast<int32_t*>(s.m12s_l)[off + i1] = m;
    }
    __syncthreads();
    line_tail_frame<T>(s, b, [&](int i) { return i < M ? (int)mm[i] : -1; }, s_wave, &s_run);
}

}
}

struct stvo_seq {
    stvo_ctx* ctx = nullptr;
    int B = 0, K = 0, M = 0, frame_idx = 0;
    stvo_match_params mp{};
    stvo_opt_params op{};
    double ratio_grid = 0;
    stvo_cam* d_cams = nullptr;
    double* d_inv_wh = nullptr;
    double* d_qtab = nullptr;
    double* d_motion_T = nullptr;
    long long* d_prof = nullptr;
    char* dev = nullptr;
    size_t dev_bytes = 0;
    char* raw_host[2] = {nullptr, nullptr};
    hipEvent_t ev_stage[2] = {nullptr, nullptr};
    unsigned long long stage_upload[2] = {0, 0};
    unsigned long long uploads = 0, uploads_done = 0;
    int stage_next = 0;
    bool st_dirty = false;
    unsigned* d_join_flag = nullptr;
    unsigned join_epoch = 0;
    unsigned fetch_epoch = 0;
    bool fetch_by_pose = false;
    unsigned fetch_value = 0;
    std::vector<char> raw_split;
    size_t raw_bytes = 0;
    stvo::SeqDev d{};
    std::vector<char*> raw_dev;
    char* extra_raw = nullptr;
    struct Set {
        float4* rc;
        uint8_t* desc;
        int32_t* n;
        double *spl, *epl, *sP, *eP, *le, *s2l, *s2lm;
        uint8_t* ldesc;
        int32_t* nl;
    } set[3];
    int cur = 0;
    int prev_set() const { return (cur + 2) % 3; }
    unsigned long long *cover, *top2;
    uint32_t *elig = nullptr, *elig_l = nullptr;
    int32_t *elig_cnt = nullptr, *elig_cnt_l = nullptr, *govf = nullptr, *govf_l = nullptr;
    int32_t *owner2, *m12s_p, *m12s_l, *m12p, *m12l, *inlp, *inll, *counts;
    int32_t* m12l_alt = nullptr;
    unsigned* d_pose_flag = nullptr;
    unsigned pose_epoch = 0;
    long long fork_rec_frame = -2;
    long long pose_flag_frame = -2;
    unsigned pose_flag_value = 0;
    stvo_pose_result* results;
    char* out_host = nullptr;
    hipStream_t line_stream = nullptr;
    hipEvent_t ev_fork = nullptr, ev_join = nullptr;
    hipEvent_t ev_cells = nullptr, ev_upload = nullptr;
    unsigned long long upload_seq = 0, upload_seen = 0;
    long long sl_forked_frame = -2;
    struct CellsBuf {
        int32_t *pstart, *pperm, *pcell, *plperm;
        uint32_t* plstart;
    } cells_buf[2] = {};
    unsigned long long *cover_l = nullptr, *top2_l = nullptr;
    int32_t* owner2_l = nullptr;
    stvo::LazyScratch lazy_l{};
    bool fetch = false;
    char* fetch_host = nullptr;
    hipEvent_t ev_fetch = nullptr;
    size_t m12_span = 0, inl_span = 0;
    int timing = 0;
    std::vector<hipEvent_t> tev;
    size_t tev_used = 0;
    bool zero_copy = false;
    std::vector<char> raw_lines;
    std::vector<int> raw_max_lines;
    int set_lines_cap[3] = {0, 0, 0};
    bool set_lines[3] = {false, false, false};
    bool last_lines = false;
    int last_slot = 0;
    stvo::GridBatch last_point_grid{};
    stvo::GridBatch last_line_grid{};
    bool last_line_fused = false;
    size_t off_kp_l, off_oct_l, off_desc_l, off_nkl, off_kp_r, off_desc_r, off_nkr, off_kl_l, off_oct_ll, off_ldesc_l,
        off_nll, off_kl_r, off_ldesc_r, off_nlr;
};

namespace {

struct IngestArgs {
    int B, K, M, has_points, has_lines;
    stvo_frame_features f;
    float* kp_l; int32_t* oct_l; uint8_t* desc_l; int32_t* n_kp_l;
    float* kp_r; uint8_t* desc_r; int32_t* n_kp_r;
    float* kl_l; int32_t* oct_ll; uint8_t* ldesc_l; int32_t* n_kl_l;
    float* kl_r; uint8_t* ldesc_r; int32_t* n_kl_r;
};
__global__ __launch_bounds__(256) void seq_ingest_kernel(IngestArgs a) {
    const int b = blockIdx.x, tid = threadIdx.x;
    auto count = [&](const int32_t* n, int cap, int stride) { return n ? min(max(n[b], 0), min(cap, stride)) : 0; };
    const int nl = a.has_points ? count(a.f.n_kp_l, a.K, a.f.stride_kp) : 0, nr = a.has_points ? count(a.f.n_kp_r, a.K, a.f.stride_kp) : 0;
    const int ml = a.has_lines ? count(a.f.n_kl_l, a.M, a.f.stride_kl) : 0, mr = a.has_lines ? count(a.f.n_kl_r, a.M, a.f.stride_kl) : 0;
    if (tid == 0) {
        a.n_kp_l[b] = nl;
        a.n_kp_r[b] = nr;
        a.n_kl_l[b] = ml;
        a.n_kl_r[b] = mr;
    }
    const size_t sp = (size_t)b * a.f.stride_kp, dp = (size_t)b * a.K, sl = (size_t)b * a.f.stride_kl, dl = (size_t)b * a.M;
    auto rows32 = [&](const uint8_t* src, uint8_t* dst, int n) {
        const uint4* s4 = reinterpret_cast<const uint4*>(src);
        uint4* d4 = reinterpret_cast<uint4*>(dst);
        for (int i = tid; i < 2 * n; i += 256) d4[i] = s4[i];
    };
    for (int i = tid; i < 2 * nl; i += 256) a.kp_l[dp * 2 + i] = a.f.kp_l[sp * 2 + i];
    for (int i = tid; i < nl; i += 256) a.oct_l[dp + i] = a.f.oct_l ? a.f.oct_l[sp + i] : 0;
    rows32(a.f.desc_l + sp * 32, a.desc_l + dp * 32, nl);
    for (int i = tid; i < 2 * nr; i += 256) a.kp_r[dp * 2 + i] = a.f.kp_r[sp * 2 + i];
    rows32(a.f.desc_r + sp * 32, a.desc_r + dp * 32, nr);
    for (int i = tid; i < 4 * ml; i += 256) a.kl_l[dl * 4 + i] = a.f.kl_l[sl * 4 + i];
    for (int i = tid; i < ml; i += 256) a.oct_ll[dl + i] = a.f.oct_ll ? a.f.oct_ll[sl + i] : 0;
    if (ml) rows32(a.f.ldesc_l + sl * 32, a.ldesc_l + dl * 32, ml);
    for (int i = tid; i < 4 * mr; i += 256) a.kl_r[dl * 4 + i] = a.f.kl_r[sl * 4 + i];
    if (mr) rows32(a.f.ldesc_r + sl * 32, a.ldesc_r + dl * 32, mr);
}

struct Carver {
    size_t off = 0;
    size_t take(size_t bytes) {
        const size_t o = off;
        off += (bytes + 255) & ~size_t(255);
        return o;
    }
};

}

extern "C" {

int stvo_seq_create_multi(stvo_ctx* ctx, int B, int max_keypoints, int max_keylines, const int32_t* img_cols,
                          const int32_t* img_rows, const stvo_cam* cams, const stvo_match_params* mp,
                          const stvo_opt_params* op, stvo_seq** out) {
    if (!ctx || !out || B <= 0 || max_keypoints <= 0 || max_keylines < 0 || !img_cols || !img_rows || !cams || !mp || !op)
        return STVO_ERR_INVALID_ARG;
    for (int b = 0; b < B; ++b)
        if (img_cols[b] <= 0 || img_rows[b] <= 0) return STVO_ERR_INVALID_ARG;
    if (max_keypoints > STVO_POSE_MAX_POINTS || max_keylines > STVO_POSE_MAX_LINES) return STVO_ERR_CAPACITY;
    const int K = (max_keypoints + 63) & ~63;
    const int M = max_keylines > 0 ? ((max_keylines + 63) & ~63) : 64;
    if (B > ctx->max_batch || K > ctx->max_rows || (size_t)B * (size_t)K > (size_t)ctx->max_batch * (size_t)ctx->max_rows)
        return STVO_ERR_CAPACITY;
    if ((size_t)2 * B * K > ctx->knn_capacity) return STVO_ERR_CAPACITY;
    if (!(mp->min_ratio_12_p <= 1.0f) || !(mp->min_ratio_12_l <= 1.0f)) return STVO_ERR_INVALID_ARG;
    HIP_TRY(ctx, hipSetDevice(ctx->device));
    stvo_seq* s = new (std::nothrow) stvo_seq();
    if (!s) return STVO_ERR_HIP;
    s->ctx = ctx;
    s->B = B;
    s->K = K;
    s->M = M;
    s->mp = *mp;
    s->op = *op;
    s->ratio_grid = mp->min_ratio_12_p_d > 0.0 ? mp->min_ratio_12_p_d : (double)mp->min_ratio_12_p;
    if (!(s->ratio_grid <= 1.0)) {
        delete s;
        return STVO_ERR_INVALID_ARG;
    }
    const size_t nb = (size_t)B;
    Carver rc;
    s->off_kp_l = rc.take(nb * K * 2 * 4);
    s->off_oct_l = rc.take(nb * K * 4);
    s->off_desc_l = rc.take(nb * K * 32);
    s->off_nkl = rc.take(nb * 4);
    s->off_kp_r = rc.take(nb * K * 2 * 4);
    s->off_desc_r = rc.take(nb * K * 32);
    s->off_nkr = rc.take(nb * 4);
    s->off_kl_l = rc.take(nb * M * 4 * 4);
    s->off_oct_ll = rc.take(nb * M * 4);
    s->off_ldesc_l = rc.take(nb * M * 32);
    s->off_nll = rc.take(nb * 4);
    s->off_kl_r = rc.take(nb * M * 4 * 4);
    s->off_ldesc_r = rc.take(nb * M * 32);
    s->off_nlr = rc.take(nb * 4);
    s->raw_bytes = rc.off;
    Carver c;
    const size_t o_raw = c.take(s->raw_bytes), o_raw1 = c.take(s->raw_bytes);
    const size_t o_cams = c.take(nb * sizeof(stvo_cam)), o_invwh = c.take(nb * 2 * 8), o_qtab = c.take(stvo::STVO_POSE_QTAB * 8),
                 o_joinflag = c.take(64), o_poseflag = c.take(64);
    const size_t o_pxy = c.take(nb * K * 2 * 4), o_pstart = c.take(nb * (STVO_GRID_CELLS + 1) * 4), o_pitems = c.take(nb * K * 4),
                 o_prank = c.take(nb * K * 4), o_pperm = c.take(nb * K * 4), o_prange = c.take(nb * K * 2 * 4), o_pcell = c.take(nb * K * 4);
    const bool lsort = K <= 2048 && mp->matching_s_ws >= 0 && mp->matching_s_ws <= stvo::GRID_LW - STVO_GRID_COLS;
    const size_t o_plstart = c.take(lsort ? nb * stvo::GRID_LSTART_STRIDE * 4 : 0), o_plperm = c.take(lsort ? nb * K * 4 : 0);
    const bool cells2 = lsort && B >= 64;
    const size_t o_pstart2 = c.take(cells2 ? nb * (STVO_GRID_CELLS + 1) * 4 : 0), o_pperm2 = c.take(cells2 ? nb * K * 4 : 0),
                 o_pcell2 = c.take(cells2 ? nb * K * 4 : 0), o_plstart2 = c.take(cells2 ? nb * stvo::GRID_LSTART_STRIDE * 4 : 0),
                 o_plperm2 = c.take(cells2 ? nb * K * 4 : 0);
    const size_t o_lxy = c.take(nb * M * 4 * 4), o_lstart = c.take(nb * (STVO_GRID_CELLS + 1) * 4),
                 o_litems = c.take(nb * M * stvo::LENT * 4), o_lrank = c.take(nb * M * 4), o_lperm = c.take(nb * M * 4),
                 o_ldir = c.take(nb * M * 2 * 8);
    const int R = K > M ? K : M;
    const size_t o_cover = c.take(nb * (size_t)(R / 64) * R * 8), o_top2 = c.take(nb * R * 8), o_owner = c.take(nb * R * 4);
    const size_t o_elig = c.take(nb * stvo::GRID_ELIG * (size_t)K * 4), o_eligc = c.take(nb * K * 4), o_govf = c.take(nb * 8);
    const size_t o_elig_l = c.take(nb * stvo::GRID_ELIG * (size_t)M * 4), o_eligc_l = c.take(nb * M * 4), o_govf_l = c.take(nb * 4);
    const size_t o_m12sp = c.take(nb * K * 4), o_m12sl = c.take(nb * M * 4), o_m12p = c.take(nb * K * 4), o_m12l = c.take(nb * M * 4),
                 o_inlp = c.take(nb * K * 4), o_inll = c.take(nb * M * 4), o_res = c.take(nb * sizeof(stvo_pose_result)),
                 o_counts = c.take(nb * 4 * 4);
    const bool alt_l = B >= 64;
    const size_t o_m12l_alt = c.take(alt_l ? nb * M * 4 : 0);
    const size_t cap_l = nb * (size_t)M * 4;
    const size_t o_cover_l = c.take(nb * (size_t)(M / 64) * M * 8), o_top2_l = c.take(nb * M * 8), o_owner_l = c.take(nb * M * 4),
                 o_knn12_l = c.take(cap_l * 8), o_knn21_l = c.take(cap_l * 8), o_cand_l = c.take(nb * M * 4),
                 o_need_l = c.take(nb * M * 4), o_qsel_l = c.take(nb * M * 4), o_nsel_l = c.take(nb * 4 * 5);
    size_t o_set[3][14];
    for (int t = 0; t < 3; ++t) {
        o_set[t][0] = c.take(nb * K * 16);
        o_set[t][1] = o_set[t][2] = 0;
        o_set[t][3] = c.take(nb * K * 32);
        o_set[t][4] = c.take(nb * 4);
        o_set[t][5] = c.take(nb * M * 2 * 8);
        o_set[t][6] = c.take(nb * M * 2 * 8);
        o_set[t][7] = c.take(nb * M * 3 * 8);
        o_set[t][8] = c.take(nb * M * 3 * 8);
        o_set[t][9] = c.take(nb * M * 3 * 8);
        o_set[t][10] = c.take(nb * M * 8);
        o_set[t][11] = c.take(nb * M * 8);
        o_set[t][12] = c.take(nb * M * 32);
        o_set[t][13] = c.take(nb * 4);
    }
    s->dev_bytes = c.off;
    bool ok = hip_ok(ctx, hipMalloc((void**)&s->dev, s->dev_bytes), "hipMalloc seq") &&
              zero_device(ctx, s->dev, s->dev_bytes, "hipMemset seq") &&
              hip_ok(ctx, hipHostMalloc((void**)&s->raw_host[0], s->raw_bytes, hipHostMallocDefault), "hipHostMalloc seq") &&
              hip_ok(ctx, hipHostMalloc((void**)&s->raw_host[1], s->raw_bytes, hipHostMallocDefault), "hipHostMalloc seq") &&
              hip_ok(ctx, hipHostMalloc((void**)&s->out_host, nb * (sizeof(stvo_pose_result) + 16), hipHostMallocDefault),
                     "hipHostMalloc seq out") &&
              hip_ok(ctx, hipStreamCreateWithFlags(&s->line_stream, hipStreamNonBlocking), "hipStreamCreate seq") &&
              hip_ok(ctx, hipEventCreateWithFlags(&s->ev_fork, hipEventDisableTiming), "hipEventCreate seq") &&
              hip_ok(ctx, hipEventCreateWithFlags(&s->ev_join, hipEventDisableTiming), "hipEventCreate seq") &&
              hip_ok(ctx, hipEventCreateWithFlags(&s->ev_cells, hipEventDisableTiming), "hipEventCreate seq") &&
              hip_ok(ctx, hipEventCreateWithFlags(&s->ev_upload, hipEventDisableTiming), "hipEventCreate seq") &&
              hip_ok(ctx, hipEventCreateWithFlags(&s->ev_stage[0], hipEventDisableTiming), "hipEventCreate seq") &&
              hip_ok(ctx, hipEventCreateWithFlags(&s->ev_stage[1], hipEventDisableTiming), "hipEventCreate seq");
    s->zero_copy = B <= 16;
    if (!ok) {
        stvo_seq_destroy(s);
        return STVO_ERR_HIP;
    }
    std::memset(s->raw_host[0], 0, s->raw_bytes);
    std::memset(s->raw_host[1], 0, s->raw_bytes);
    char* D = s->dev;
    s->raw_dev = {D + o_raw, D + o_raw1};
    s->raw_lines.assign(2, 0);
    s->raw_max_lines.assign(2, 0);
    s->raw_split.assign(2, 0);
    s->d_cams = (stvo_cam*)(D + o_cams);
    s->d_inv_wh = (double*)(D + o_invwh);
    s->d_qtab = (double*)(D + o_qtab);
    s->d_join_flag = (unsigned*)(D + o_joinflag);
    s->d_pose_flag = (unsigned*)(D + o_poseflag);
    if (alt_l) s->m12l_alt = (int32_t*)(D + o_m12l_alt);
    {
        std::vector<double> iw(2 * nb);
        for (int b = 0; b < B; ++b) {
            iw[2 * b + 0] = STVO_GRID_COLS / (double)img_cols[b];
            iw[2 * b + 1] = STVO_GRID_ROWS / (double)img_rows[b];
        }
        double qtab[stvo::STVO_POSE_QTAB];
        for (int l = 0; l < stvo::STVO_POSE_QTAB; ++l) qtab[l] = std::sqrt(pm::level_sigma2(l, s->mp.orb_scale_factor));
        ok = upload_now(ctx, s->d_qtab, qtab, sizeof(qtab), "hipMemcpy qtab") &&
             upload_now(ctx, s->d_cams, cams, nb * sizeof(stvo_cam), "hipMemcpy cams") &&
             upload_now(ctx, s->d_inv_wh, iw.data(), iw.size() * sizeof(double), "hipMemcpy inv_wh");
        if (!ok) {
            stvo_seq_destroy(s);
            return STVO_ERR_HIP;
        }
    }
    stvo::SeqDev& d = s->d;
    d.B = B; d.K = K; d.M = M;
    d.cams = s->d_cams; d.inv_wh = s->d_inv_wh;
    d.mp = s->mp;
    d.pxy_l = (int32_t*)(D + o_pxy); d.pstart = (int32_t*)(D + o_pstart); d.pitems = (int32_t*)(D + o_pitems);
    d.prank = (int32_t*)(D + o_prank); d.pperm = (int32_t*)(D + o_pperm);
    d.lxy_l = (int32_t*)(D + o_lxy); d.lstart = (int32_t*)(D + o_lstart); d.litems = (int32_t*)(D + o_litems);
    d.lrank = (int32_t*)(D + o_lrank); d.lperm = (int32_t*)(D + o_lperm); d.ldir = (double*)(D + o_ldir);
    s->cover = (unsigned long long*)(D + o_cover); s->top2 = (unsigned long long*)(D + o_top2);
    s->owner2 = (int32_t*)(D + o_owner);
    s->elig = (uint32_t*)(D + o_elig); s->elig_cnt = (int32_t*)(D + o_eligc); s->govf = (int32_t*)(D + o_govf);
    s->elig_l = (uint32_t*)(D + o_elig_l); s->elig_cnt_l = (int32_t*)(D + o_eligc_l); s->govf_l = (int32_t*)(D + o_govf_l);
    s->cover_l = (unsigned long long*)(D + o_cover_l); s->top2_l = (unsigned long long*)(D + o_top2_l);
    s->owner2_l = (int32_t*)(D + o_owner_l);
    s->lazy_l = stvo::LazyScratch{(uint2*)(D + o_knn12_l), (uint2*)(D + o_knn21_l), (int32_t*)(D + o_cand_l), (int32_t*)(D + o_need_l),
                                  (int32_t*)(D + o_qsel_l), (int32_t*)(D + o_nsel_l), cap_l};
    s->m12s_p = (int32_t*)(D + o_m12sp); s->m12s_l = (int32_t*)(D + o_m12sl);
    s->m12p = (int32_t*)(D + o_m12p); s->m12l = (int32_t*)(D + o_m12l);
    s->inlp = (int32_t*)(D + o_inlp); s->inll = (int32_t*)(D + o_inll);
    s->results = (stvo_pose_result*)(D + o_res); s->counts = (int32_t*)(D + o_counts);
    s->m12_span = o_inlp - o_m12sp;
    s->inl_span = o_res - o_inlp;
    d.m12s_p = s->m12s_p; d.m12s_l = s->m12s_l;
    d.top2_p = s->top2; d.govf_p = s->govf; d.prange = (int32_t*)(D + o_prange); d.pcell = (int32_t*)(D + o_pcell);
    if (lsort) {
        d.plstart = (uint32_t*)(D + o_plstart); d.plperm = (int32_t*)(D + o_plperm);
    }
    s->cells_buf[0] = {d.pstart, d.pperm, d.pcell, d.plperm, d.plstart};
    s->cells_buf[1] = s->cells_buf[0];
    if (cells2)
        s->cells_buf[1] = {(int32_t*)(D + o_pstart2), (int32_t*)(D + o_pperm2), (int32_t*)(D + o_pcell2), (int32_t*)(D + o_plperm2),
                           (uint32_t*)(D + o_plstart2)};
    for (int t = 0; t < 3; ++t) {
        stvo_seq::Set& q = s->set[t];
        q.rc = (float4*)(D + o_set[t][0]);
        q.desc = (uint8_t*)(D + o_set[t][3]); q.n = (int32_t*)(D + o_set[t][4]);
        q.spl = (double*)(D + o_set[t][5]); q.epl = (double*)(D + o_set[t][6]); q.sP = (double*)(D + o_set[t][7]);
        q.eP = (double*)(D + o_set[t][8]); q.le = (double*)(D + o_set[t][9]); q.s2l = (double*)(D + o_set[t][10]);
        q.s2lm = (double*)(D + o_set[t][11]); q.ldesc = (uint8_t*)(D + o_set[t][12]); q.nl = (int32_t*)(D + o_set[t][13]);
    }
    *out = s;
    return STVO_OK;
}

int stvo_seq_create(stvo_ctx* ctx, int B, int max_keypoints, int max_keylines, int img_cols, int img_rows,
                    const stvo_cam* cam, const stvo_match_params* mp, const stvo_opt_params* op, stvo_seq** out) {
    if (B <= 0 || !cam) return STVO_ERR_INVALID_ARG;
    const std::vector<int32_t> cols((size_t)B, img_cols), rows((size_t)B, img_rows);
    const std::vector<stvo_cam> cams((size_t)B, *cam);
    return stvo_seq_create_multi(ctx, B, max_keypoints, max_keylines, cols.data(), rows.data(), cams.data(), mp, op, out);
}

int stvo_seq_set_slots(stvo_seq* s, int n_slots) {
    if (!s || n_slots < 2 || n_slots > STVO_SEQ_MAX_SLOTS) return STVO_ERR_INVALID_ARG;
    stvo_ctx* ctx = s->ctx;
    HIP_TRY(ctx, hipSetDevice(ctx->device));
    HIP_TRY(ctx, hipStreamSynchronize(ctx->stream));
    if (s->extra_raw) {
        HIP_TRY(ctx, hipFree(s->extra_raw));
        s->extra_raw = nullptr;
    }
    s->raw_dev.resize(2);
    s->raw_lines.resize(2);
    s->raw_max_lines.resize(2);
    s->raw_split.assign(2, 0);
    if (n_slots > 2) {
        HIP_TRY(ctx, hipMalloc((void**)&s->extra_raw, (size_t)(n_slots - 2) * s->raw_bytes));
        if (!zero_device(ctx, s->extra_raw, (size_t)(n_slots - 2) * s->raw_bytes, "hipMemset seq raw")) return STVO_ERR_HIP;
        for (int k = 2; k < n_slots; ++k) {
            s->raw_dev.push_back(s->extra_raw + (size_t)(k - 2) * s->raw_bytes);
            s->raw_lines.push_back(0);
            s->raw_max_lines.push_back(0);
            s->raw_split.push_back(0);
        }
    }
    return STVO_OK;
}

int stvo_seq_destroy(stvo_seq* s) {
    if (!s) return STVO_OK;
    (void)hipSetDevice(s->ctx->device);
    (void)hipStreamSynchronize(s->ctx->stream);
    if (s->d_prof) (void)hipFree(s->d_prof);
    if (s->d_motion_T) (void)hipFree(s->d_motion_T);
    if (s->line_stream) {
        (void)hipStreamSynchronize(s->line_stream);
        (void)hipStreamDestroy(s->line_stream);
    }
    if (s->ev_fork) (void)hipEventDestroy(s->ev_fork);
    if (s->ev_join) (void)hipEventDestroy(s->ev_join);
    if (s->ev_cells) (void)hipEventDestroy(s->ev_cells);
    if (s->ev_upload) (void)hipEventDestroy(s->ev_upload);
    for (auto e : s->ev_stage)
        if (e) (void)hipEventDestroy(e);
    for (auto e : s->tev) (void)hipEventDestroy(e);
    if (s->ev_fetch) (void)hipEventDestroy(s->ev_fetch);
    if (s->fetch_host) (void)hipHostFree(s->fetch_host);
    if (s->dev) (void)hipFree(s->dev);
    if (s->extra_raw) (void)hipFree(s->extra_raw);
    for (auto h : s->raw_host)
        if (h) (void)hipHostFree(h);
    if (s->out_host) (void)hipHostFree(s->out_host);
    delete s;
    return STVO_OK;
}

namespace {

void bind_raw(stvo_seq* s, stvo::SeqDev& d, int slot) {
    char* Rw = s->raw_dev[slot];
    d.kp_l = (const float*)(Rw + s->off_kp_l); d.oct_l = (const int32_t*)(Rw + s->off_oct_l);
    d.desc_l = (const uint8_t*)(Rw + s->off_desc_l); d.n_kp_l = (const int32_t*)(Rw + s->off_nkl);
    d.kp_r = (const float*)(Rw + s->off_kp_r); d.desc_r = (const uint8_t*)(Rw + s->off_desc_r);
    d.n_kp_r = (const int32_t*)(Rw + s->off_nkr);
    d.kl_l = (const float*)(Rw + s->off_kl_l); d.oct_ll = (const int32_t*)(Rw + s->off_oct_ll);
    d.ldesc_l = (const uint8_t*)(Rw + s->off_ldesc_l); d.n_kl_l = (const int32_t*)(Rw + s->off_nll);
    d.kl_r = (const float*)(Rw + s->off_kl_r); d.ldesc_r = (const uint8_t*)(Rw + s->off_ldesc_r);
    d.n_kl_r = (const int32_t*)(Rw + s->off_nlr);
}

}

int stvo_seq_upload(stvo_seq* s, int slot, const stvo_frame_features* f) {
    if (!s || !f || slot < 0 || slot >= (int)s->raw_dev.size()) return STVO_ERR_INVALID_ARG;
    stvo_ctx* ctx = s->ctx;
    HIP_TRY(ctx, hipSetDevice(ctx->device));
    const int B = s->B, K = s->K, M = s->M;
    for (int b = 0; b < B; ++b) {
        const bool kl = f->n_kp_l && f->n_kp_l[b] > 0, kr = f->n_kp_r && f->n_kp_r[b] > 0;
        const bool ll = f->n_kl_l && f->n_kl_l[b] > 0 && s->op.has_lines, lr = f->n_kl_r && f->n_kl_r[b] > 0 && s->op.has_lines;
        if ((kl && (!f->kp_l || !f->oct_l || !f->desc_l)) || (kr && (!f->kp_r || !f->desc_r)) ||
            (ll && (!f->kl_l || !f->oct_ll || !f->ldesc_l)) || (lr && (!f->kl_r || !f->ldesc_r)))
            return STVO_ERR_INVALID_ARG;
    }
    const int sb = s->stage_next;
    s->stage_next ^= 1;
    if (s->stage_upload[sb] > s->uploads_done) {
        HIP_TRY(ctx, hipEventRecord(s->ev_stage[sb], ctx->stream));
        HIP_TRY(ctx, hipEventSynchronize(s->ev_stage[sb]));
        if (s->line_stream) HIP_TRY(ctx, hipStreamSynchronize(s->line_stream));
        s->uploads_done = s->uploads;
    }
    char* H = s->raw_host[sb];
    int32_t* nkl = (int32_t*)(H + s->off_nkl);
    int32_t* nkr = (int32_t*)(H + s->off_nkr);
    int32_t* nll = (int32_t*)(H + s->off_nll);
    int32_t* nlr = (int32_t*)(H + s->off_nlr);
    int max_lines = 0;
    for (int b = 0; b < B; ++b) {
        const int a = f->n_kp_l ? f->n_kp_l[b] : 0, r = f->n_kp_r ? f->n_kp_r[b] : 0;
        const int la = (f->n_kl_l && s->op.has_lines) ? f->n_kl_l[b] : 0, lr = (f->n_kl_r && s->op.has_lines) ? f->n_kl_r[b] : 0;
        if (a < 0 || r < 0 || la < 0 || lr < 0 || a > K || r > K || la > M || lr > M || a > f->stride_kp || r > f->stride_kp ||
            la > f->stride_kl || lr > f->stride_kl)
            return STVO_ERR_CAPACITY;
        nkl[b] = s->op.has_points ? a : 0;
        nkr[b] = s->op.has_points ? r : 0;
        nll[b] = la;
        nlr[b] = lr;
        max_lines = std::max(max_lines, std::max(la, lr));
        const size_t so = (size_t)b * f->stride_kp, dof = (size_t)b * K;
        if (nkl[b]) {
            std::memcpy(H + s->off_kp_l + dof * 8, f->kp_l + so * 2, (size_t)a * 8);
            std::memcpy(H + s->off_oct_l + dof * 4, f->oct_l + so, (size_t)a * 4);
            std::memcpy(H + s->off_desc_l + dof * 32, f->desc_l + so * 32, (size_t)a * 32);
        }
        if (nkr[b]) {
            std::memcpy(H + s->off_kp_r + dof * 8, f->kp_r + so * 2, (size_t)r * 8);
            std::memcpy(H + s->off_desc_r + dof * 32, f->desc_r + so * 32, (size_t)r * 32);
        }
        const size_t sl = (size_t)b * f->stride_kl, dl = (size_t)b * M;
        if (la) {
            std::memcpy(H + s->off_kl_l + dl * 16, f->kl_l + sl * 4, (size_t)la * 16);
            std::memcpy(H + s->off_oct_ll + dl * 4, f->oct_ll + sl, (size_t)la * 4);
            std::memcpy(H + s->off_ldesc_l + dl * 32, f->ldesc_l + sl * 32, (size_t)la * 32);
        }
        if (lr) {
            std::memcpy(H + s->off_kl_r + dl * 16, f->kl_r + sl * 4, (size_t)lr * 16);
            std::memcpy(H + s->off_ldesc_r + dl * 32, f->ldesc_r + sl * 32, (size_t)lr * 32);
        }
    }
    bool any_lines = false;
    for (int b = 0; b < B; ++b) any_lines = any_lines || (nll[b] > 0 && nlr[b] > 0);
    s->raw_lines[slot] = any_lines;
    s->raw_max_lines[slot] = max_lines;
    s->raw_split[slot] = 0;
    if (s->raw_bytes <= (size_t)4 << 20) {
        if (any_lines && s->op.has_points && !s->st_dirty && s->line_stream) {
            stvo::launch_copy16(ctx->stream, H, s->raw_dev[slot], s->off_kl_l);
            stvo::launch_copy16(s->line_stream, H + s->off_kl_l, s->raw_dev[slot] + s->off_kl_l, s->raw_bytes - s->off_kl_l);
            s->raw_split[slot] = 1;
        } else {
            stvo::launch_copy16(ctx->stream, H, s->raw_dev[slot], s->raw_bytes);
        }
    } else {
        HIP_TRY(ctx, hipMemcpyAsync(s->raw_dev[slot], H, s->raw_bytes, hipMemcpyHostToDevice, ctx->stream));
    }
    s->stage_upload[sb] = ++s->uploads;
    if (s->B >= 64 && s->line_stream) {
        HIP_TRY(ctx, hipEventRecord(s->ev_upload, ctx->stream));
        ++s->upload_seq;
    }
    return STVO_OK;
}

int stvo_seq_upload_dev(stvo_seq* s, int slot, const stvo_frame_features* f) {
    if (!s || !f || slot < 0 || slot >= (int)s->raw_dev.size()) return STVO_ERR_INVALID_ARG;
    if (f->stride_kp < 0 || f->stride_kl < 0) return STVO_ERR_INVALID_ARG;
    const bool pts = s->op.has_points && f->n_kp_l && f->n_kp_r, lns = s->op.has_lines && f->n_kl_l && f->n_kl_r;
    if ((pts && (!f->kp_l || !f->desc_l || !f->kp_r || !f->desc_r)) || (lns && (!f->kl_l || !f->ldesc_l || !f->kl_r || !f->ldesc_r)))
        return STVO_ERR_INVALID_ARG;
    stvo_ctx* ctx = s->ctx;
    HIP_TRY(ctx, hipSetDevice(ctx->device));
    char* Rw = s->raw_dev[slot];
    IngestArgs a{};
    a.B = s->B; a.K = s->K; a.M = s->M; a.has_points = pts; a.has_lines = lns; a.f = *f;
    a.kp_l = (float*)(Rw + s->off_kp_l); a.oct_l = (int32_t*)(Rw + s->off_oct_l); a.desc_l = (uint8_t*)(Rw + s->off_desc_l);
    a.n_kp_l = (int32_t*)(Rw + s->off_nkl); a.kp_r = (float*)(Rw + s->off_kp_r); a.desc_r = (uint8_t*)(Rw + s->off_desc_r);
    a.n_kp_r = (int32_t*)(Rw + s->off_nkr); a.kl_l = (float*)(Rw + s->off_kl_l); a.oct_ll = (int32_t*)(Rw + s->off_oct_ll);
    a.ldesc_l = (uint8_t*)(Rw + s->off_ldesc_l); a.n_kl_l = (int32_t*)(Rw + s->off_nll); a.kl_r = (float*)(Rw + s->off_kl_r);
    a.ldesc_r = (uint8_t*)(Rw + s->off_ldesc_r); a.n_kl_r = (int32_t*)(Rw + s->off_nlr);
    hipLaunchKernelGGL(seq_ingest_kernel, dim3(s->B), dim3(256), 0, ctx->stream, a);
    if (s->B >= 64 && s->line_stream) {
        HIP_TRY(ctx, hipEventRecord(s->ev_upload, ctx->stream));
        ++s->upload_seq;
    }
    s->st_dirty = true;
    s->raw_split[slot] = 0;
    s->raw_max_lines[slot] = s->M;
    s->raw_lines[slot] = lns;
    return check_launch(ctx);
}

namespace {

struct StepFlags {
    bool lines_now, lines_prev, track;
};

struct StepPub {
    bool fork_recorded = false;
    bool pose_flagged = false;
    unsigned pose_flag_value = 0;
    bool line_forked = false;
    bool fetch_by_pose = false;
    unsigned fetch_value = 0;
};

int seq_enqueue_step(stvo_seq* s, int slot, const StepFlags& fl, StepPub& pub) {
    stvo_ctx* ctx = s->ctx;
    const int B = s->B, K = s->K, M = s->M;
    hipStream_t st = ctx->stream;
    hipEvent_t* tev = nullptr;
    if (s->timing) {
        while (s->tev.size() < s->tev_used + 2 * STVO_SEQ_NSTAGE) {
            hipEvent_t e;
            if (hipEventCreate(&e) != hipSuccess) break;
            s->tev.push_back(e);
        }
        if (s->tev.size() >= s->tev_used + 2 * STVO_SEQ_NSTAGE) {
            tev = s->tev.data() + s->tev_used;
            s->tev_used += 2 * STVO_SEQ_NSTAGE;
        }
    }
    const bool light = tev && s->timing == 2;
    auto mark = [&](int k, hipStream_t q) {
        if (tev && !(light && k < 2)) (void)hipEventRecord(tev[k], q);
    };
    pub = StepPub{};
    const bool alt_ok = s->m12l_alt != nullptr && !s->fetch;
    int32_t* const m12l_use = (alt_ok && (s->frame_idx & 1)) ? s->m12l_alt : s->m12l;
    stvo_seq::Set& cs = s->set[s->cur];
    stvo_seq::Set& ps = s->set[s->prev_set()];
    stvo::SeqDev d = s->d;
    bind_raw(s, d, slot);
    d.rc = cs.rc; d.desc = cs.desc; d.n = cs.n;
    d.spl = cs.spl; d.epl = cs.epl; d.sP = cs.sP; d.eP = cs.eP; d.le = cs.le; d.s2l = cs.s2l; d.s2lm = cs.s2lm;
    d.ldesc = cs.ldesc; d.nl = cs.nl;
    const size_t res_bytes = (size_t)B * sizeof(stvo_pose_result);
    d.host_n = s->zero_copy ? reinterpret_cast<int32_t*>(s->out_host + res_bytes) : nullptr;
    d.host_nl = s->zero_copy ? reinterpret_cast<int32_t*>(s->out_host + res_bytes + (size_t)B * 4) : nullptr;
    const bool lines_now = fl.lines_now, lines_prev = fl.lines_prev;
    const bool par = lines_now && s->op.has_points;
    hipStream_t sl = par ? s->line_stream : st;
    const bool mid_fork = par && B >= 64;
    const bool fork_free = par && s->raw_split[slot] && !s->st_dirty;
    pub.line_forked = par && (mid_fork || !fork_free);
    if (par && !mid_fork && !fork_free) {
        HIP_TRY(ctx, hipEventRecord(s->ev_fork, st));
        HIP_TRY(ctx, hipStreamWaitEvent(sl, s->ev_fork, 0));
    }
    d.zero_nl = (!lines_now && s->op.has_points) ? 1 : 0;
    auto point_stage = [&]() -> int {
        if (s->op.has_points) {
            mark(0, st);
            stvo::GridBatch g;
            std::memset(&g, 0, sizeof(g));
            g.B = B; g.stride1 = K; g.stride2 = K; g.xy_width = 2; g.items_stride = K; g.words64 = K / 64; g.n1p = K;
            g.cell_xy1 = d.pxy_l; g.d1 = d.desc_l; g.n1 = d.n_kp_l; g.cell_start = d.pstart; g.cell_items = d.pitems;
            g.d2 = d.desc_r; g.n2 = d.n_kp_r; g.dir2 = nullptr;
            g.w = stvo_grid_window{s->mp.matching_s_ws, 0, 0, 0};
            g.ratio = s->ratio_grid; g.line_sim_th = 0.0; g.mutual = s->mp.best_lr_matches;
            g.cover = s->cover; g.rank = d.prank; g.perm = d.pperm; g.top2 = s->top2; g.owner2 = s->owner2; g.m12 = s->m12s_p;
            if (g.mutual) { g.elig = s->elig; g.elig_cnt = s->elig_cnt; g.ovf = s->govf; }
            g.misfit = s->govf + s->B;
            g.range_points = 1;
            g.range1 = d.prange;
            g.cell2 = d.pcell;
            g.lstart = d.plstart; g.lperm = d.plperm;
            g.lean_cells = stvo::grid_points_fused_ok(g) ? 1 : 0;
            g.has_tail = g.lean_cells;
            if (stvo::dbg().grid_tail == 0) g.has_tail = 0;
            if (g.has_tail) g.tail = stvo::point_tail_args(d);
            g.fused_cells = g.lean_cells && B <= stvo::device_cu_count() && stvo::dbg().grid_cells != 0;
            const bool cells_ahead = mid_fork && g.lean_cells && !g.fused_cells && (!tev || light) &&
                                     s->cells_buf[0].pstart != s->cells_buf[1].pstart && s->sl_forked_frame == (long long)s->frame_idx - 1 &&
                                     stvo::dbg().cells_ahead != 0;
            const int la_sw = stvo::dbg().lines_ahead;
            const bool la_pays = s->pose_flag_frame == (long long)s->frame_idx - 1 && B > 2 * stvo::device_cu_count() &&
                                 std::max(s->raw_max_lines[slot], s->set_lines_cap[s->prev_set()]) <= 128;
            const bool lines_ahead = cells_ahead && alt_ok && s->fork_rec_frame == (long long)s->frame_idx - 1 && la_sw != 0 &&
                                     (la_sw == 1 || la_pays);
            if (lines_ahead) HIP_TRY(ctx, hipStreamWaitEvent(sl, s->ev_fork, 0));
            if (g.fused_cells)
                g.cells = stvo::point_cells_args(d);
            else if (g.lean_cells)
                hipLaunchKernelGGL(stvo::point_cells_kernel<true>, dim3(B), dim3(256), 0, cells_ahead ? sl : st, d);
            else
                hipLaunchKernelGGL(stvo::point_cells_kernel<false>, dim3(B), dim3(256), 0, st, d);
            if (cells_ahead) {
                HIP_TRY(ctx, hipEventRecord(s->ev_cells, sl));
                HIP_TRY(ctx, hipStreamWaitEvent(st, s->ev_cells, 0));
            }
            hipEvent_t gev_light[2] = {nullptr, tev ? tev[3] : nullptr};
            if (light) (void)hipEventRecord(tev[2], st);
            if (mid_fork) {
                HIP_TRY(ctx, hipEventRecord(s->ev_fork, st));
                pub.fork_recorded = true;
                if (!lines_ahead)
                    HIP_TRY(ctx, hipStreamWaitEvent(sl, s->ev_fork, 0));
                else if (s->pose_flag_frame == (long long)s->frame_idx - 1)
                    stvo::launch_stream_gate(sl, s->d_pose_flag, s->pose_flag_value);
            }
            s->last_point_grid = g;
            stvo::launch_grid_batch(st, g, false, tev ? (light ? gev_light : tev + 2) : nullptr);
            if (!g.has_tail) hipLaunchKernelGGL(stvo::point_tail_kernel, dim3(B), dim3(stvo::TAIL_BLOCK), 0, st, d);
            mark(1, st);
        } else {
            HIP_TRY(ctx, hipMemsetAsync(cs.n, 0, (size_t)B * 4, st));
        }
        return STVO_OK;
    };
    auto line_stage = [&]() -> int {
        if (lines_now) {
            stvo::GridBatch g;
            std::memset(&g, 0, sizeof(g));
            g.B = B; g.stride1 = M; g.stride2 = M; g.xy_width = 4; g.items_stride = M * stvo::LENT; g.words64 = M / 64; g.n1p = M;
            g.cell_xy1 = d.lxy_l; g.d1 = d.ldesc_l; g.n1 = d.n_kl_l; g.cell_start = d.lstart; g.cell_items = d.litems;
            g.d2 = d.ldesc_r; g.n2 = d.n_kl_r; g.dir2 = d.ldir;
            g.w = stvo_grid_window{s->mp.matching_s_ws, 0, 0, 0};
            g.ratio = s->ratio_grid ; g.line_sim_th = s->mp.line_sim_th;
            g.mutual = s->mp.best_lr_matches;
            g.cover = s->cover_l; g.rank = d.lrank; g.perm = d.lperm; g.top2 = s->top2_l; g.owner2 = s->owner2_l; g.m12 = s->m12s_l;
            if (g.mutual) { g.elig = s->elig_l; g.elig_cnt = s->elig_cnt_l; g.ovf = s->govf_l; }
            s->last_line_grid = g;
            const int Mk = std::min(M, std::max(64, (s->raw_max_lines[slot] + 63) & ~63));
            s->set_lines_cap[s->cur] = Mk;
            const size_t lds = (size_t)Mk * stvo::LSF_BYTES_PER_LINE + 4 + (size_t)Mk * (Mk / 32) * 4;
            const int ef = stvo::dbg().line_fused;
            s->last_line_fused = M <= stvo::LSF_MAX_LINES && (ef != stvo::DBG_UNSET ? ef != 0 : (B >= 16 || Mk <= 128)) &&
                                 (lds <= (48u << 10) || stvo::lds_opt_in(reinterpret_cast<const void*>(stvo::line_stereo_fused_kernel<256>), (int)lds));
            if (s->last_line_fused) {
                hipLaunchKernelGGL(stvo::line_stereo_fused_kernel<256>, dim3(B), dim3(256), lds, sl, d, Mk, (int)s->mp.best_lr_matches, s->ratio_grid);
            } else {
                hipLaunchKernelGGL(stvo::line_cells_kernel, dim3(B), dim3(256), 0, sl, d);
                stvo::launch_grid_batch(sl, g, true);
                hipLaunchKernelGGL(stvo::line_tail_kernel, dim3(B), dim3(256), 0, sl, d);
            }
        } else if (!d.zero_nl) {
            HIP_TRY(ctx, hipMemsetAsync(cs.nl, 0, (size_t)B * 4, st));
        }
        return STVO_OK;
    };
    TRY(point_stage());
    TRY(line_stage());
    const bool track = fl.track;
    if (track) {
        const stvo::LazyScratch w{ctx->knn12, ctx->knn21, ctx->cand, ctx->need, ctx->qsel, ctx->nsel, ctx->knn_capacity};
        const int esm = stvo::dbg().match_small;
        const int lines_cap = std::max(s->set_lines_cap[s->cur], s->set_lines_cap[s->prev_set()]);
        const bool small_sets = esm != stvo::DBG_UNSET ? esm != 0 : lines_cap <= 128;
        const bool elz = stvo::dbg().match_lazy == 1;
        int small_cap = 0;
        auto match_set = [&](hipStream_t q, const stvo::LazyScratch& ws, int stride, const uint8_t* da, const int32_t* na,
                             const uint8_t* db, const int32_t* nb, float nnr, int32_t* m12, hipEvent_t* mev) {
            if (stvo::match_small_ok(stride) && small_sets && !mev) {
                stvo::launch_match_small(q, B, stride, da, na, db, nb, nnr, s->mp.best_lr_matches, m12, small_cap);
            } else if (s->mp.best_lr_matches && B <= 4 && !mev && !elz) {
                const int nseg = std::min(4, stvo::knn_pick_nseg(B, stride, ws.knn_capacity));
                stvo::launch_hamming_knn2(q, B, stride, stride, da, na, db, nb, ws.knn12, ws.knn21, 1, 0, 0, nullptr, nullptr, nseg);
                stvo::launch_nnr_mutual(q, B, stride, ws.knn12, ws.knn21, na, nb, nnr, 1, m12, nseg);
            } else if (s->mp.best_lr_matches) {
                stvo::launch_match_mutual_lazy(q, B, stride, da, na, db, nb, nnr, ws, m12, 0, nullptr, mev);
            } else {
                const int nseg = stvo::knn_pick_nseg(B, stride, ws.knn_capacity);
                stvo::launch_hamming_knn2(q, B, stride, stride, da, na, db, nb, ws.knn12, ws.knn21, 0, 0, 0, nullptr, nullptr, nseg);
                stvo::launch_nnr_mutual(q, B, stride, ws.knn12, ws.knn21, na, nb, nnr, 0, m12, nseg);
            }
        };
        hipEvent_t mev_light[4] = {tev ? tev[4] : nullptr, tev ? tev[5] : nullptr, nullptr, nullptr};
        if (s->op.has_points) match_set(st, w, K, ps.desc, ps.n, cs.desc, cs.n, s->mp.min_ratio_12_p, s->m12p, tev ? (light ? mev_light : tev + 4) : nullptr);
        small_cap = lines_cap;
        if (lines_prev && lines_now)
            match_set(sl, s->lazy_l, M, ps.ldesc, ps.nl, cs.ldesc, cs.nl, s->mp.min_ratio_12_l, m12l_use, nullptr);
        else if (lines_prev)
            HIP_TRY(ctx, hipMemsetAsync(m12l_use, 0xFF, (size_t)B * M * sizeof(int32_t), st));
        const bool inline_sync = stvo::pose_inline_sync_ok(B) && stvo::dbg().seq_inline != 0 && !tev && (!s->fetch || (B == 1 && s->zero_copy));
        if (par && inline_sync) {
            stvo::launch_stream_signal(sl, s->d_join_flag, ++s->join_epoch);
        } else if (par) {
            HIP_TRY(ctx, hipEventRecord(s->ev_join, sl));
            HIP_TRY(ctx, hipStreamWaitEvent(st, s->ev_join, 0));
        }
        pub.fetch_by_pose = s->fetch && inline_sync;
        if (s->fetch && !inline_sync) {
            stvo::launch_copy16(st, s->m12s_p, s->fetch_host, s->m12_span);
            HIP_TRY(ctx, hipEventRecord(s->ev_fetch, st));
        }
        stvo::PoseArgs a{};
        std::memset(&a, 0, sizeof(a));
        a.B = B; a.max_pts = K; a.max_lines = M;
        a.n_prev_pts = s->op.has_points ? ps.n : nullptr;
        a.prev_rc = ps.rc; a.curr_rc = cs.rc; a.q_tab = s->d_qtab; a.level_scale = s->mp.orb_scale_factor; a.m12p = s->m12p;
        a.n_prev_lines = s->op.has_lines ? ps.nl : nullptr;
        a.prev_sP = ps.sP; a.prev_eP = ps.eP; a.prev_spl = ps.spl; a.prev_epl = ps.epl; a.prev_s2l = ps.s2lm;
        a.curr_le = cs.le; a.m12l = m12l_use;
        a.cams = s->d_cams; a.prm = s->op;
        a.init_T = s->d_motion_T; a.next_T = s->d_motion_T;
        a.results = s->zero_copy ? reinterpret_cast<stvo_pose_result*>(s->out_host) : s->results;
        a.inl_p_out = s->inlp; a.inl_l_out = s->inll;
        const bool inl_zero_copy = s->fetch && s->zero_copy;
        if (inl_zero_copy) {
            a.inl_p_out = reinterpret_cast<int32_t*>(s->fetch_host + s->m12_span);
            a.inl_l_out = reinterpret_cast<int32_t*>(s->fetch_host + s->m12_span + (reinterpret_cast<const char*>(s->inll) - reinterpret_cast<const char*>(s->inlp)));
        }
        if (stvo::dbg().pose_prof != stvo::DBG_UNSET) {
            if (!s->d_prof) HIP_TRY(ctx, hipMalloc((void**)&s->d_prof, (size_t)B * 16 * sizeof(long long)));
            a.prof_out = s->d_prof;
        }
        if (par && inline_sync) {
            a.wait_flag = s->d_join_flag;
            a.wait_value = s->join_epoch;
        }
        a.lazy_eig = (inline_sync && s->zero_copy && stvo::dbg().pose_kernel != 4) ? 1 : 0;
        if (pub.fetch_by_pose) {
            a.fetch_src = reinterpret_cast<const uint4*>(s->m12s_p);
            a.fetch_dst = reinterpret_cast<uint4*>(s->fetch_host);
            a.fetch_n16 = (unsigned)(s->m12_span / 16);
            a.fetch_flag = reinterpret_cast<unsigned*>(s->fetch_host + s->m12_span + s->inl_span);
            a.fetch_value = pub.fetch_value = ++s->fetch_epoch;
        }
        if (s->m12l_alt != nullptr && stvo::pose_start_flag_ok(a)) {
            a.start_flag = s->d_pose_flag;
            a.start_value = pub.pose_flag_value = ++s->pose_epoch;
            pub.pose_flagged = true;
        }
        mark(8, st);
        TRY(stvo::launch_pose(st, a));
        mark(9, st);
        if (s->fetch && !inl_zero_copy) stvo::launch_copy16(st, s->inlp, s->fetch_host + s->m12_span, s->inl_span);
    } else {
        if (par) {
            HIP_TRY(ctx, hipEventRecord(s->ev_join, sl));
            HIP_TRY(ctx, hipStreamWaitEvent(st, s->ev_join, 0));
        }
        if (s->fetch) {
            stvo::launch_copy16(st, s->m12s_p, s->fetch_host, s->m12_span);
            HIP_TRY(ctx, hipEventRecord(s->ev_fetch, st));
        }
    }
    return check_launch(ctx);
}

}

int stvo_seq_step_dev(stvo_seq* s, int slot) {
    if (!s || slot < 0 || slot >= (int)s->raw_dev.size()) return STVO_ERR_INVALID_ARG;
    stvo_ctx* ctx = s->ctx;
    HIP_TRY(ctx, hipSetDevice(ctx->device));
    StepFlags fl;
    fl.lines_now = s->op.has_lines && s->raw_lines[slot];
    fl.lines_prev = s->op.has_lines && s->set_lines[s->prev_set()];
    fl.track = s->frame_idx > 0;
    {
        const stvo_seq::CellsBuf& cb = s->cells_buf[s->frame_idx & 1];
        s->d.pstart = cb.pstart; s->d.pperm = cb.pperm; s->d.pcell = cb.pcell; s->d.plperm = cb.plperm; s->d.plstart = cb.plstart;
        if (s->line_stream && s->upload_seen != s->upload_seq) {
            HIP_TRY(ctx, hipStreamWaitEvent(s->line_stream, s->ev_upload, 0));
            s->upload_seen = s->upload_seq;
        }
    }
    StepPub pub;
    TRY(seq_enqueue_step(s, slot, fl, pub));
    if (pub.fork_recorded) s->fork_rec_frame = s->frame_idx;
    if (pub.pose_flagged) {
        s->pose_flag_frame = s->frame_idx;
        s->pose_flag_value = pub.pose_flag_value;
    }
    if (pub.line_forked) s->sl_forked_frame = s->frame_idx;
    s->fetch_by_pose = pub.fetch_by_pose;
    s->fetch_value = pub.fetch_value;
    s->st_dirty = true;
    s->set_lines[s->cur] = fl.lines_now;
    s->last_lines = fl.lines_now;
    s->last_slot = slot;
    s->cur = (s->cur + 1) % 3;
    s->frame_idx++;
    return STVO_OK;
}

int stvo_seq_read(stvo_seq* s, stvo_pose_result* results, int32_t* counts) {
    if (!s) return STVO_ERR_INVALID_ARG;
    stvo_ctx* ctx = s->ctx;
    HIP_TRY(ctx, hipSetDevice(ctx->device));
    const int B = s->B;
    hipStream_t st = ctx->stream;
    const stvo_seq::Set& ls = s->set[s->prev_set()];
    if (s->d_prof && s->frame_idx > 1) {
        HIP_TRY(ctx, hipStreamSynchronize(st));
        std::vector<long long> h((size_t)B * 16);
        HIP_TRY(ctx, hipMemcpy(h.data(), s->d_prof, h.size() * sizeof(long long), hipMemcpyDeviceToHost));
        double m[16] = {0, 0, 0, 0, 0, 0, 0, 0, 0, 0, 0, 0, 0, 0, 0, 0};
        for (int f = 0; f < B; ++f)
            for (int i = 0; i < 16; ++i) m[i] += (double)h[(size_t)f * 16 + i] / B;
        std::fprintf(stderr, "[pose prof] mean ticks/pair: evaluate %.0f  iter-algebra %.0f  cov+isgood+commit %.0f  remove_outliers %.0f  total %.0f | "
                             "eval-compute %.0f  fold %.0f  barrier+sum %.0f | prologue %.0f | wave busy %.0f %.0f | removeOutliers: residuals %.0f  statistics %.0f  re-deal %.0f\n",
                     m[0], m[1], m[2], m[3], m[4], m[5], m[6], m[7], m[14], m[8], m[9], m[10], m[11], m[12]);
    }
    const bool track = s->frame_idx > 1;
    char* OH = s->out_host;
    const size_t res_bytes = (size_t)B * sizeof(stvo_pose_result);
    if (!s->zero_copy) {
        if (track) HIP_TRY(ctx, hipMemcpyAsync(OH, s->results, res_bytes, hipMemcpyDeviceToHost, st));
        HIP_TRY(ctx, hipMemcpyAsync(OH + res_bytes, ls.n, (size_t)B * 4, hipMemcpyDeviceToHost, st));
        HIP_TRY(ctx, hipMemcpyAsync(OH + res_bytes + (size_t)B * 4, ls.nl, (size_t)B * 4, hipMemcpyDeviceToHost, st));
    }
    HIP_TRY(ctx, hipStreamSynchronize(st));
    s->uploads_done = s->uploads;
    s->st_dirty = false;
    const stvo_pose_result* hr = reinterpret_cast<const stvo_pose_result*>(OH);
    const int32_t* hn = reinterpret_cast<const int32_t*>(OH + res_bytes);
    for (int b = 0; b < B; ++b) {
        if (results) {
            if (track) {
                results[b] = hr[b];
                if (results[b].path & stvo::PATH_EIG_PENDING) {
                    pm::eig6_ql(results[b].cov, results[b].cov_eig);
                    results[b].path &= ~stvo::PATH_EIG_PENDING;
                }
            }
            else
                std::memset(&results[b], 0, sizeof(stvo_pose_result));
        }
        if (counts) {
            counts[4 * b + 0] = s->op.has_points ? hn[b] : 0;
            counts[4 * b + 1] = s->last_lines ? hn[B + b] : 0;
            counts[4 * b + 2] = track ? hr[b].n_matched_pt : 0;
            counts[4 * b + 3] = track ? hr[b].n_matched_ls : 0;
        }
    }
    return STVO_OK;
}

int stvo_seq_strides(const stvo_seq* s, int32_t* stride_pts, int32_t* stride_lines) {
    if (!s) return STVO_ERR_INVALID_ARG;
    if (stride_pts) *stride_pts = s->K;
    if (stride_lines) *stride_lines = s->M;
    return STVO_OK;
}

int stvo_seq_enable_fetch(stvo_seq* s, int enable) {
    if (!s) return STVO_ERR_INVALID_ARG;
    stvo_ctx* ctx = s->ctx;
    HIP_TRY(ctx, hipSetDevice(ctx->device));
    if (enable && !s->fetch_host) {
        HIP_TRY(ctx, hipHostMalloc((void**)&s->fetch_host, s->m12_span + s->inl_span + 64, hipHostMallocDefault));
        *reinterpret_cast<volatile unsigned*>(s->fetch_host + s->m12_span + s->inl_span) = 0u;
        HIP_TRY(ctx, hipEventCreateWithFlags(&s->ev_fetch, hipEventDisableTiming));
    }
    s->fetch = enable != 0;
    return STVO_OK;
}

int stvo_seq_fetch_matches(stvo_seq* s, const int32_t** m12_stereo_pts, const int32_t** m12_stereo_lines,
                           const int32_t** m12_pts, const int32_t** m12_lines) {
    if (!s || !s->fetch || s->frame_idx == 0) return STVO_ERR_INVALID_ARG;
    stvo_ctx* ctx = s->ctx;
    HIP_TRY(ctx, hipSetDevice(ctx->device));
    if (s->fetch_by_pose) {
        const volatile unsigned* flag = reinterpret_cast<const volatile unsigned*>(s->fetch_host + s->m12_span + s->inl_span);
        const auto t0 = std::chrono::steady_clock::now();
        bool seen = false;
        for (unsigned spin = 0; !(seen = (*flag == s->fetch_value)); ++spin)
            if ((spin & 1023u) == 1023u && std::chrono::steady_clock::now() - t0 > std::chrono::milliseconds(20)) break;
        std::atomic_thread_fence(std::memory_order_acquire);
        if (!seen) {
            HIP_TRY(ctx, hipStreamSynchronize(ctx->stream));
            if (*flag != s->fetch_value) {
                std::snprintf(ctx->last_error, sizeof(ctx->last_error), "%s", "the pose kernel did not publish the match indices of the last step (no signal from the key-line stream)");
                return STVO_ERR_HIP;
            }
        }
    } else {
        HIP_TRY(ctx, hipEventSynchronize(s->ev_fetch));
    }
    const char* H = s->fetch_host;
    const char* D0 = reinterpret_cast<const char*>(s->m12s_p);
    if (m12_stereo_pts) *m12_stereo_pts = reinterpret_cast<const int32_t*>(H);
    if (m12_stereo_lines) *m12_stereo_lines = reinterpret_cast<const int32_t*>(H + (reinterpret_cast<const char*>(s->m12s_l) - D0));
    if (m12_pts) *m12_pts = reinterpret_cast<const int32_t*>(H + (reinterpret_cast<const char*>(s->m12p) - D0));
    if (m12_lines) *m12_lines = reinterpret_cast<const int32_t*>(H + (reinterpret_cast<const char*>(s->m12l) - D0));
    return STVO_OK;
}

int stvo_seq_fetch_inliers(stvo_seq* s, const int32_t** inl_pts, const int32_t** inl_lines) {
    if (!s || !s->fetch || s->frame_idx < 2) return STVO_ERR_INVALID_ARG;
    stvo_ctx* ctx = s->ctx;
    HIP_TRY(ctx, hipSetDevice(ctx->device));
    HIP_TRY(ctx, hipStreamSynchronize(ctx->stream));
    const char* H = s->fetch_host + s->m12_span;
    if (inl_pts) *inl_pts = reinterpret_cast<const int32_t*>(H);
    if (inl_lines) *inl_lines = reinterpret_cast<const int32_t*>(H + (reinterpret_cast<const char*>(s->inll) - reinterpret_cast<const char*>(s->inlp)));
    return STVO_OK;
}

int stvo_seq_set_motion_model(stvo_seq* s, int enable) {
    if (!s) return STVO_ERR_INVALID_ARG;
    stvo_ctx* ctx = s->ctx;
    HIP_TRY(ctx, hipSetDevice(ctx->device));
    HIP_TRY(ctx, hipStreamSynchronize(ctx->stream));
    if (s->line_stream) HIP_TRY(ctx, hipStreamSynchronize(s->line_stream));
    if (!enable) {
        if (s->d_motion_T) (void)hipFree(s->d_motion_T);
        s->d_motion_T = nullptr;
    } else {
        if (!s->d_motion_T) HIP_TRY(ctx, hipMalloc((void**)&s->d_motion_T, (size_t)s->B * 16 * sizeof(double)));
        std::vector<double> I((size_t)s->B * 16, 0.0);
        for (int b = 0; b < s->B; ++b)
            for (int i = 0; i < 4; ++i) I[(size_t)b * 16 + i * 5] = 1.0;
        if (!upload_now(ctx, s->d_motion_T, I.data(), I.size() * sizeof(double), "hipMemcpy motion")) return STVO_ERR_HIP;
    }
    return STVO_OK;
}

int stvo_seq_set_stage_timing(stvo_seq* s, int enable) {
    if (!s) return STVO_ERR_INVALID_ARG;
    s->timing = enable == 2 ? 2 : (enable != 0);
    s->tev_used = 0;
    return STVO_OK;
}

int stvo_seq_get_stage_timing(stvo_seq* s, float avg_ms[STVO_SEQ_NSTAGE], int32_t* n_steps) {
    if (!s || !avg_ms || !n_steps) return STVO_ERR_INVALID_ARG;
    stvo_ctx* ctx = s->ctx;
    HIP_TRY(ctx, hipSetDevice(ctx->device));
    HIP_TRY(ctx, hipStreamSynchronize(ctx->stream));
    double acc[STVO_SEQ_NSTAGE] = {0};
    int cnt[STVO_SEQ_NSTAGE] = {0};
    for (size_t k = 0; k + 2 * STVO_SEQ_NSTAGE <= s->tev_used; k += 2 * STVO_SEQ_NSTAGE)
        for (int st = 0; st < STVO_SEQ_NSTAGE; ++st) {
            if (s->timing == 2 && (st == 0 || st == 3)) continue;
            float ms = 0.f;
            if (hipEventElapsedTime(&ms, s->tev[k + 2 * st], s->tev[k + 2 * st + 1]) == hipSuccess) {
                acc[st] += ms;
                ++cnt[st];
            }
        }
    (void)hipGetLastError();
    int n = 0;
    for (int st = 0; st < STVO_SEQ_NSTAGE; ++st) {
        avg_ms[st] = cnt[st] ? (float)(acc[st] / cnt[st]) : 0.f;
        if (cnt[st] > n) n = cnt[st];
    }
    *n_steps = n;
    s->tev_used = 0;
    return STVO_OK;
}

int stvo_seq_debug_grid(stvo_seq* s, int b, int lines, int32_t* cell_start, int32_t* cell_items, int32_t cap_items,
                        int32_t* cells_left, int32_t* cand_off, int32_t* cand, int32_t cap_cand, int32_t* n_left_out) {
    if (!s || b < 0 || b >= s->B || !cell_start || !cell_items || !cells_left || !cand_off || !cand || !n_left_out || s->frame_idx == 0)
// ... 75 lines not shown
```

stvo-pl_amd/csrc/stvo_capi.hip:

```cpp
#include <hip/hip_runtime.h>

#include <cstdio>
#include <cstdlib>
#include <cstring>
#include <new>
#include <vector>

#include "ctx_internal.h"

namespace stvo {
namespace {

int env_int(const char* name) {
    const char* e = std::getenv(name);
    return (e && *e) ? std::atoi(e) : DBG_UNSET;
}
DebugSwitches parse_switches() {
    DebugSwitches d;
    d.pose_kernel = env_int("STVO_POSE_KERNEL");
    d.pose2p_nw = env_int("STVO_POSE2P_NW");
    d.pose_prof = env_int("STVO_POSE_PROF");
    d.pose_lds_t = env_int("STVO_POSE_LDS_T");
    d.pose_los = env_int("STVO_POSE_LOS");
    d.knn_mfma = env_int("STVO_KNN_MFMA");
    d.knn_nseg = env_int("STVO_KNN_NSEG");
    d.seq_inline = env_int("STVO_SEQ_INLINE");
    d.cells_ahead = env_int("STVO_CELLS_AHEAD");
    d.line_fused = env_int("STVO_LINE_FUSED");
    d.match_small = env_int("STVO_MATCH_SMALL");
    d.match_lazy = env_int("STVO_MATCH_LAZY");
    d.grid_tail = env_int("STVO_GRID_TAIL");
    d.grid_fused = env_int("STVO_GRID_FUSED");
    d.grid_fused_cap = env_int("STVO_GRID_FUSED_CAP");
    d.grid_cells = env_int("STVO_GRID_CELLS");
    d.lines_ahead = env_int("STVO_LINES_AHEAD");
    d.lsd_grow = env_int("STVO_LSD_GROW");
    d.lsd_waves = env_int("STVO_LSD_WAVES");
    d.lsd_xcd_blocks = env_int("STVO_LSD_XCD_BLOCKS");
    d.lsd_feed_ahead = env_int("STVO_LSD_FEED_AHEAD");
    d.lsd_sep = env_int("STVO_LSD_SEP");
    d.lsd_ahead = env_int("STVO_LSD_AHEAD");
    d.lsd_multi = env_int("STVO_LSD_MULTI");
    return d;
}
DebugSwitches& switches() {
    static DebugSwitches d = parse_switches();
    return d;
}

}

const DebugSwitches& dbg() { return switches(); }
void dbg_reparse() { switches() = parse_switches(); }

}

extern "C" {

void stvo_debug_reparse_env(void) { stvo::dbg_reparse(); }

const char* stvo_backend_name(void) { return "hip-gfx950"; }
int stvo_abi_version(void) { return STVO_ABI_VERSION; }

const char* stvo_error_string(int code) {
    switch (code) {
        case STVO_OK: return "ok";
        case STVO_ERR_INVALID_ARG: return "invalid argument";
        case STVO_ERR_HIP: return "HIP runtime error";
        case STVO_ERR_NO_DEVICE: return "no gfx950 device (this library has no CPU fallback)";
        case STVO_ERR_CAPACITY: return "problem exceeds the context capacity";
        case STVO_ERR_UNSUPPORTED: return "unsupported";
        default: return "unknown error";
    }
}

const char* stvo_ctx_last_error(const stvo_ctx* ctx) { return ctx ? ctx->last_error : ""; }

int stvo_ctx_create(int device_id, int max_rows, int max_batch, stvo_ctx** out) {
    if (!out || max_rows <= 0 || max_rows > STVO_MAX_ROWS_LIMIT || max_batch <= 0) return STVO_ERR_INVALID_ARG;
    *out = nullptr;
    int ndev = 0;
    if (hipGetDeviceCount(&ndev) != hipSuccess || ndev <= 0 || device_id < 0 || device_id >= ndev)
        return STVO_ERR_NO_DEVICE;
    hipDeviceProp_t prop;
    if (hipGetDeviceProperties(&prop, device_id) != hipSuccess) return STVO_ERR_NO_DEVICE;
    if (std::strncmp(prop.gcnArchName, "gfx950", 6) != 0) return STVO_ERR_NO_DEVICE;
    stvo_ctx* ctx = new (std::nothrow) stvo_ctx();
    if (!ctx) return STVO_ERR_HIP;
    ctx->device = device_id;
    ctx->max_rows = max_rows;
    ctx->max_batch = max_batch;
    bool ok = hip_ok(ctx, hipSetDevice(device_id), "hipSetDevice") &&
              hip_ok(ctx, hipStreamCreateWithFlags(&ctx->stream, hipStreamNonBlocking), "hipStreamCreate");
    ctx->own_stream = ok;
    if (ok) {
        stvo::pose_retain_stream(ctx->stream);
        ctx->stream_retained = true;
    }
    const size_t knn_elems = (size_t)max_rows * (size_t)max_batch;
    const size_t knn_seg_elems =
        (size_t)max_rows * (size_t)(2 * max_batch > stvo::KNN_MAX_NSEG ? 2 * max_batch : stvo::KNN_MAX_NSEG);
    ctx->knn_capacity = knn_seg_elems;
    ctx->arena_size = (size_t)max_rows * 1024 + ((size_t)4 << 20);
    ok = ok && hip_ok(ctx, hipMalloc((void**)&ctx->knn12, knn_seg_elems * sizeof(uint2)), "hipMalloc knn12") &&
         hip_ok(ctx, hipMalloc((void**)&ctx->knn21, knn_seg_elems * sizeof(uint2)), "hipMalloc knn21") &&
         hip_ok(ctx, hipMalloc((void**)&ctx->cand, knn_elems * sizeof(int32_t)), "hipMalloc cand") &&
         hip_ok(ctx, hipMalloc((void**)&ctx->need, knn_elems * sizeof(int32_t)), "hipMalloc need") &&
         hip_ok(ctx, hipMalloc((void**)&ctx->qsel, knn_elems * sizeof(int32_t)), "hipMalloc qsel") &&
         hip_ok(ctx, hipMalloc((void**)&ctx->nsel, (size_t)max_batch * 5 * sizeof(int32_t)), "hipMalloc nsel") &&
         hip_ok(ctx, hipMalloc((void**)&ctx->arena, ctx->arena_size), "hipMalloc arena") &&
         hip_ok(ctx, hipHostMalloc((void**)&ctx->arena_host, ctx->arena_size, hipHostMallocDefault), "hipHostMalloc") &&
         hip_ok(ctx, hipMalloc((void**)&ctx->probe_sink, 256), "hipMalloc sink");
    if (!ok) {
        stvo_ctx_destroy(ctx);
        return STVO_ERR_HIP;
    }
    *out = ctx;
    return STVO_OK;
}

int stvo_ctx_destroy(stvo_ctx* ctx) {
    if (!ctx) return STVO_OK;
    (void)hipSetDevice(ctx->device);
    if (ctx->stream) (void)hipStreamSynchronize(ctx->stream);
    if (ctx->knn12) (void)hipFree(ctx->knn12);
    if (ctx->knn21) (void)hipFree(ctx->knn21);
    if (ctx->cand) (void)hipFree(ctx->cand);
    if (ctx->need) (void)hipFree(ctx->need);
    if (ctx->qsel) (void)hipFree(ctx->qsel);
    if (ctx->nsel) (void)hipFree(ctx->nsel);
    if (ctx->arena) (void)hipFree(ctx->arena);
    if (ctx->arena_host) (void)hipHostFree(ctx->arena_host);
    if (ctx->probe_sink) (void)hipFree(ctx->probe_sink);
    for (hipEvent_t e : ctx->ev_pool) (void)hipEventDestroy(e);
    if (ctx->stream_retained) stvo::pose_release_stream(ctx->stream);
    if (ctx->aux_stream) {
        (void)hipStreamSynchronize(ctx->aux_stream);
        stvo::pose_release_stream(ctx->aux_stream);
        (void)hipStreamDestroy(ctx->aux_stream);
        (void)hipEventDestroy(ctx->ev_match_done);
        (void)hipEventDestroy(ctx->ev_pose_done);
    }
    if (ctx->own_stream && ctx->stream) (void)hipStreamDestroy(ctx->stream);
    delete ctx;
    return STVO_OK;
}

int stvo_ctx_set_stream(stvo_ctx* ctx, void* hip_stream) {
    if (!ctx) return STVO_ERR_INVALID_ARG;
    (void)hipSetDevice(ctx->device);
    (void)hipStreamSynchronize(ctx->stream);
    if (ctx->stream_retained) stvo::pose_release_stream(ctx->stream);
    if (ctx->own_stream && ctx->stream) (void)hipStreamDestroy(ctx->stream);
    ctx->own_stream = false;
    ctx->stream = reinterpret_cast<hipStream_t>(hip_stream);
    stvo::pose_retain_stream(ctx->stream);
    ctx->stream_retained = true;
    return STVO_OK;
}

int stvo_ctx_synchronize(stvo_ctx* ctx) {
    if (!ctx) return STVO_ERR_INVALID_ARG;
    HIP_TRY(ctx, hipStreamSynchronize(ctx->stream));
    if (ctx->aux_stream) HIP_TRY(ctx, hipStreamSynchronize(ctx->aux_stream));
    ctx->pose_pending = false;
    return STVO_OK;
}

int stvo_ctx_set_overlap(stvo_ctx* ctx, int enable) {
    if (!ctx) return STVO_ERR_INVALID_ARG;
    HIP_TRY(ctx, hipSetDevice(ctx->device));
    if (enable && !ctx->aux_stream) {
        hipEvent_t em = nullptr, ep = nullptr;
        hipStream_t as = nullptr;
        if (!hip_ok(ctx, hipEventCreateWithFlags(&em, hipEventDisableTiming), "hipEventCreate overlap") ||
            !hip_ok(ctx, hipEventCreateWithFlags(&ep, hipEventDisableTiming), "hipEventCreate overlap") ||
            !hip_ok(ctx, hipStreamCreateWithFlags(&as, hipStreamNonBlocking), "hipStreamCreate overlap")) {
            if (em) (void)hipEventDestroy(em);
            if (ep) (void)hipEventDestroy(ep);
            return STVO_ERR_HIP;
        }
        ctx->ev_match_done = em;
        ctx->ev_pose_done = ep;
        ctx->aux_stream = as;
        stvo::pose_retain_stream(as);
    }
    if (!enable && ctx->aux_stream) HIP_TRY(ctx, hipStreamSynchronize(ctx->aux_stream));
    ctx->overlap = enable ? 1 : 0;
    return STVO_OK;
}

int stvo_match_nnr_mutual(stvo_ctx* ctx, const uint8_t* d1, int n1, const uint8_t* d2, int n2, float nnr, int mutual,
                          int32_t* m12, int32_t* n_matches) {
    if (!ctx || n1 < 0 || n2 < 0 || (n1 > 0 && (!d1 || !m12)) || (n2 > 0 && !d2)) return STVO_ERR_INVALID_ARG;
    if (!(nnr <= 1.0f)) return STVO_ERR_INVALID_ARG;
    if (n1 > ctx->max_rows || n2 > ctx->max_rows) return STVO_ERR_CAPACITY;
    if (n_matches) *n_matches = 0;
    if (n1 == 0) return STVO_OK;
    HIP_TRY(ctx, hipSetDevice(ctx->device));
    ctx->arena_off = 0;
    ctx->upload_hi = 0;
    const int stride = n1 > n2 ? n1 : n2;
    uint8_t *dd1, *dd2;
    int32_t *dn1, *dn2, *dm12;
    TRY(upload(ctx, &dd1, d1, (size_t)n1 * STVO_DESC_BYTES, (size_t)stride * STVO_DESC_BYTES));
    TRY(upload(ctx, &dd2, d2, (size_t)n2 * STVO_DESC_BYTES, (size_t)stride * STVO_DESC_BYTES));
    TRY(upload(ctx, &dn1, &n1, 1));
    TRY(upload(ctx, &dn2, &n2, 1));
    TRY(flush_uploads(ctx));
    TRY(upload(ctx, &dm12, (const int32_t*)nullptr, (size_t)stride));
    if (mutual) {
        const stvo::LazyScratch w{ctx->knn12, ctx->knn21, ctx->cand, ctx->need, ctx->qsel, ctx->nsel, ctx->knn_capacity};
        stvo::launch_match_mutual_lazy(ctx->stream, 1, stride, dd1, dn1, dd2, dn2, nnr, w, dm12, 0, nullptr);
    } else {
        const int nseg = stvo::knn_pick_nseg(1, stride, ctx->knn_capacity);
        stvo::launch_hamming_knn2(ctx->stream, 1, stride, stride, dd1, dn1, dd2, dn2, ctx->knn12, ctx->knn21, 0, 0, 0,
                                  nullptr, nullptr, nseg);
        stvo::launch_nnr_mutual(ctx->stream, 1, stride, ctx->knn12, ctx->knn21, dn1, dn2, nnr, 0, dm12, nseg);
    }
    TRY(check_launch(ctx));
    TRY(download_begin(ctx, dm12, (size_t)n1 * sizeof(int32_t)));
    HIP_TRY(ctx, hipStreamSynchronize(ctx->stream));
    std::memcpy(m12, host_mirror(ctx, dm12), (size_t)n1 * sizeof(int32_t));
    if (n_matches) {
        int c = 0;
        for (int i = 0; i < n1; ++i) c += m12[i] >= 0;
        *n_matches = c;
    }
    return STVO_OK;
}

int stvo_match_nnr_mutual_batched_dev(stvo_ctx* ctx, int B, int row_stride, const uint8_t* d1, const int32_t* n1,
                                      const uint8_t* d2, const int32_t* n2, float nnr, int mutual, int32_t* m12) {
    if (!ctx || B < 0 || row_stride <= 0 || !d1 || !d2 || !n1 || !n2 || !m12 || !(nnr <= 1.0f))
        return STVO_ERR_INVALID_ARG;
    if (B > ctx->max_batch || (size_t)B * row_stride > (size_t)ctx->max_batch * ctx->max_rows || row_stride > STVO_MAX_ROWS_LIMIT ||
        (size_t)2 * B * row_stride > ctx->knn_capacity)
        return STVO_ERR_CAPACITY;
    HIP_TRY(ctx, hipSetDevice(ctx->device));
    if (mutual) {
        const stvo::LazyScratch w{ctx->knn12, ctx->knn21, ctx->cand, ctx->need, ctx->qsel, ctx->nsel, ctx->knn_capacity};
        stvo::launch_match_mutual_lazy(ctx->stream, B, row_stride, d1, n1, d2, n2, nnr, w, m12, 0, nullptr);
    } else {
        const int nseg = stvo::knn_pick_nseg(B, row_stride, ctx->knn_capacity);
        stvo::launch_hamming_knn2(ctx->stream, B, row_stride, row_stride, d1, n1, d2, n2, ctx->knn12, ctx->knn21, 0, 0, 0,
                                  nullptr, nullptr, nseg);
        stvo::launch_nnr_mutual(ctx->stream, B, row_stride, ctx->knn12, ctx->knn21, n1, n2, nnr, 0, m12, nseg);
    }
    return check_launch(ctx);
}

namespace {

int stage_records(stvo_ctx* ctx, const stvo_matched* m, const double* T, stvo::PoseArgs* a, int32_t** d_inl_p,
                  int32_t** d_inl_l) {
    std::memset(a, 0, sizeof(*a));
    if (m->np < 0 || m->nl < 0) return STVO_ERR_INVALID_ARG;
    if (m->np > STVO_POSE_MAX_POINTS || m->nl > STVO_POSE_MAX_LINES) return STVO_ERR_CAPACITY;
    a->B = 1;
    a->max_pts = m->np > 0 ? m->np : 1;
    a->max_lines = m->nl;
    double *P, *obs, *s2p, *sP, *eP, *le, *spl, *epl, *s2l, *dT;
    int32_t *dnp, *dnl;
    TRY(upload(ctx, &P, m->P, (size_t)m->np * 3));
    TRY(upload(ctx, &obs, m->pl_obs, (size_t)m->np * 2));
    TRY(upload(ctx, &s2p, m->sigma2p, (size_t)m->np));
    TRY(upload(ctx, d_inl_p, (const int32_t*)m->inlier_p, (size_t)m->np));
    TRY(upload(ctx, &sP, m->sP, (size_t)m->nl * 3));
    TRY(upload(ctx, &eP, m->eP, (size_t)m->nl * 3));
    TRY(upload(ctx, &le, m->le_obs, (size_t)m->nl * 3));
    TRY(upload(ctx, &spl, m->spl, (size_t)m->nl * 2));
    TRY(upload(ctx, &epl, m->epl, (size_t)m->nl * 2));
    TRY(upload(ctx, &s2l, m->sigma2l, (size_t)m->nl));
    TRY(upload(ctx, d_inl_l, (const int32_t*)m->inlier_l, (size_t)m->nl));
    TRY(upload(ctx, &dnp, &m->np, 1));
    TRY(upload(ctx, &dnl, &m->nl, 1));
    TRY(upload(ctx, &dT, T, 16));
    TRY(flush_uploads(ctx));
    a->n_prev_pts = dnp;
    a->prev_P = P;
    a->prev_s2p = s2p;
    a->curr_pl = obs;
    a->m12p = nullptr;
    a->init_inl_p = *d_inl_p;
    a->n_prev_lines = dnl;
    a->prev_sP = sP;
    a->prev_eP = eP;
    a->prev_spl = spl;
    a->prev_epl = epl;
    a->prev_s2l = s2l;
    a->curr_le = le;
    a->m12l = nullptr;
    a->init_inl_l = *d_inl_l;
    a->init_T = dT;
    return STVO_OK;
}

}

int stvo_normal_eq(stvo_ctx* ctx, const double T[16], const stvo_cam* cam, const stvo_opt_params* params,
                   const stvo_matched* m, int robust, double H[36], double g[6], double* e, int32_t* n_used) {
    if (!ctx || !T || !cam || !params || !m || !H || !g || !e) return STVO_ERR_INVALID_ARG;
    HIP_TRY(ctx, hipSetDevice(ctx->device));
    ctx->arena_off = 0;
    ctx->upload_hi = 0;
    stvo::PoseArgs a{};
    int32_t *dip, *dil;
    TRY(stage_records(ctx, m, T, &a, &dip, &dil));
    a.cam = *cam;
    a.prm = *params;
    double* dout = arena_alloc<double>(ctx, 44);
    if (!dout) return STVO_ERR_CAPACITY;
    a.eval_only = 1;
    a.eval_robust = robust;
    a.eval_out = dout;
    TRY(stvo::launch_pose(ctx->stream, a));
    TRY(check_launch(ctx));
    TRY(download_begin(ctx, dout, 44 * sizeof(double)));
    HIP_TRY(ctx, hipStreamSynchronize(ctx->stream));
    const double* out = host_mirror(ctx, dout);
    std::memcpy(H, out, 36 * sizeof(double));
    std::memcpy(g, out + 36, 6 * sizeof(double));
    *e = out[42];
    if (n_used) *n_used = (int32_t)out[43];
    return STVO_OK;
}

int stvo_optimize_pose(stvo_ctx* ctx, const double init_T[16], const stvo_cam* cam, const stvo_opt_params* params,
                       stvo_matched* m, stvo_pose_result* out) {
    if (!ctx || !init_T || !cam || !params || !m || !out) return STVO_ERR_INVALID_ARG;
    if ((m->np > 0 && (!m->P || !m->pl_obs || !m->sigma2p || !m->inlier_p)) ||
        (m->nl > 0 && (!m->sP || !m->eP || !m->le_obs || !m->spl || !m->epl || !m->sigma2l || !m->inlier_l)))
        return STVO_ERR_INVALID_ARG;
    HIP_TRY(ctx, hipSetDevice(ctx->device));
    ctx->arena_off = 0;
    ctx->upload_hi = 0;
    stvo::PoseArgs a{};
    int32_t *dip, *dil;
    TRY(stage_records(ctx, m, init_T, &a, &dip, &dil));
    a.cam = *cam;
    a.prm = *params;
    stvo_pose_result* dres = arena_alloc<stvo_pose_result>(ctx, 1);
    int32_t* dop = arena_alloc<int32_t>(ctx, (size_t)a.max_pts);
    int32_t* dol = arena_alloc<int32_t>(ctx, (size_t)(a.max_lines > 0 ? a.max_lines : 1));
    if (!dres || !dop || !dol) return STVO_ERR_CAPACITY;
    a.results = dres;
    a.inl_p_out = dop;
    a.inl_l_out = dol;
    TRY(stvo::launch_pose(ctx->stream, a));
    TRY(check_launch(ctx));
    TRY(download_begin(ctx, dres, sizeof(*out)));
    if (m->np) TRY(download_begin(ctx, dop, (size_t)m->np * 4));
    if (m->nl) TRY(download_begin(ctx, dol, (size_t)m->nl * 4));
    HIP_TRY(ctx, hipStreamSynchronize(ctx->stream));
    std::memcpy(out, host_mirror(ctx, dres), sizeof(*out));
    const int32_t* ip = host_mirror(ctx, dop);
    const int32_t* il = host_mirror(ctx, dol);
    for (int i = 0; i < m->np; ++i) m->inlier_p[i] = ip[i] > 0 ? 1 : 0;
    for (int i = 0; i < m->nl; ++i) m->inlier_l[i] = il[i] > 0 ? 1 : 0;
    return STVO_OK;
}

namespace {

constexpr int kOverlapLdsPad = 26 * 1024;

int fill_pose_args(const stvo_track_batch_dev* b, const stvo_cam* cam, const stvo_opt_params* prm, bool identity,
                   stvo::PoseArgs* a) {
    std::memset(a, 0, sizeof(*a));
    a->B = b->B;
    a->max_pts = b->max_pts;
    a->max_lines = b->max_lines;
    a->n_prev_pts = b->n_prev_pts;
    a->prev_P = b->prev_P;
    a->prev_s2p = b->prev_sigma2p;
    a->curr_pl = b->curr_pl;
    a->m12p = identity ? nullptr : b->m12_pts;
    a->n_prev_lines = b->max_lines > 0 ? b->n_prev_lines : nullptr;
    a->prev_sP = b->prev_sP;
    a->prev_eP = b->prev_eP;
    a->prev_spl = b->prev_spl;
    a->prev_epl = b->prev_epl;
    a->prev_s2l = b->prev_sigma2l;
    a->curr_le = b->curr_le;
    a->m12l = identity ? nullptr : b->m12_lines;
    a->init_T = b->init_T;
    a->cam = *cam;
    a->prm = *prm;
    a->results = b->results;
    a->inl_p_out = b->inlier_pts;
    a->inl_l_out = b->inlier_lines;
    return STVO_OK;
}

int check_batch(stvo_ctx* ctx, const stvo_track_batch_dev* b, bool need_desc) {
    if (!ctx || !b || b->B < 0 || b->max_pts <= 0 || b->max_lines < 0) return STVO_ERR_INVALID_ARG;
    if (!b->n_prev_pts || !b->prev_P || !b->prev_sigma2p || !b->curr_pl || !b->results) return STVO_ERR_INVALID_ARG;
    if (need_desc && (!b->prev_pdesc || !b->curr_pdesc || !b->n_curr_pts || !b->m12_pts)) return STVO_ERR_INVALID_ARG;
    if (b->max_lines > 0) {
        if (!b->n_prev_lines || !b->prev_sP || !b->prev_eP || !b->prev_spl || !b->prev_epl || !b->prev_sigma2l ||
            !b->curr_le)
            return STVO_ERR_INVALID_ARG;
        if (need_desc && (!b->prev_ldesc || !b->curr_ldesc || !b->n_curr_lines || !b->m12_lines))
            return STVO_ERR_INVALID_ARG;
    }
    if (b->max_pts > STVO_POSE_MAX_POINTS || b->max_lines > STVO_POSE_MAX_LINES) return STVO_ERR_CAPACITY;
    const size_t rows = (size_t)(b->max_pts > b->max_lines ? b->max_pts : b->max_lines);
    if (b->B > ctx->max_batch || (size_t)b->B * rows > (size_t)ctx->max_batch * (size_t)ctx->max_rows ||
        (size_t)2 * b->B * rows > ctx->knn_capacity)
        return STVO_ERR_CAPACITY;
    return STVO_OK;
}

}

int stvo_track_batched_dev(stvo_ctx* ctx, const stvo_track_batch_dev* b, const stvo_cam* cam,
                           const stvo_opt_params* params, float nnr_points, float nnr_lines, int mutual) {
    if (!cam || !params || !(nnr_points <= 1.0f) || !(nnr_lines <= 1.0f)) return STVO_ERR_INVALID_ARG;
    TRY(check_batch(ctx, b, true));
    HIP_TRY(ctx, hipSetDevice(ctx->device));
    if (b->B == 0) return STVO_OK;
    const int pad = ctx->overlap ? kOverlapLdsPad : 0;
    hipEvent_t prev_pose = (ctx->overlap && ctx->pose_pending) ? ctx->ev_pose_done : nullptr;
    const stvo::LazyScratch w{ctx->knn12, ctx->knn21, ctx->cand, ctx->need, ctx->qsel, ctx->nsel, ctx->knn_capacity};
    auto match_set = [&](int stride, const uint8_t* da, const int32_t* na, const uint8_t* db, const int32_t* nb,
                         float nnr, int32_t* m12) {
        if (mutual) {
            hipEvent_t* tev = nullptr;
            if (ctx->timing && da == b->prev_pdesc) {
                while (ctx->ev_pool.size() < ctx->ev_used + 4) {
                    hipEvent_t e;
                    if (hipEventCreate(&e) != hipSuccess) break;
                    ctx->ev_pool.push_back(e);
                }
                if (ctx->ev_pool.size() >= ctx->ev_used + 4) {
                    tev = ctx->ev_pool.data() + ctx->ev_used;
                    ctx->ev_used += 4;
                }
            }
            stvo::launch_match_mutual_lazy(ctx->stream, b->B, stride, da, na, db, nb, nnr, w, m12, pad, prev_pose, tev);
        } else {
            const int nseg = stvo::knn_pick_nseg(b->B, stride, ctx->knn_capacity);
            stvo::launch_hamming_knn2(ctx->stream, b->B, stride, stride, da, na, db, nb, ctx->knn12, ctx->knn21, 0, pad, 0,
                                      nullptr, nullptr, nseg);
            if (prev_pose) (void)hipStreamWaitEvent(ctx->stream, prev_pose, 0);
            stvo::launch_nnr_mutual(ctx->stream, b->B, stride, ctx->knn12, ctx->knn21, na, nb, nnr, 0, m12, nseg);
        }
    };
    if (params->has_points)
        match_set(b->max_pts, b->prev_pdesc, b->n_prev_pts, b->curr_pdesc, b->n_curr_pts, nnr_points, b->m12_pts);
    if (params->has_lines && b->max_lines > 0)
        match_set(b->max_lines, b->prev_ldesc, b->n_prev_lines, b->curr_ldesc, b->n_curr_lines, nnr_lines, b->m12_lines);
    if (prev_pose) HIP_TRY(ctx, hipStreamWaitEvent(ctx->stream, prev_pose, 0));
    stvo::PoseArgs a{};
    fill_pose_args(b, cam, params, false, &a);
    if (!params->has_points) a.n_prev_pts = nullptr;
    if (!params->has_lines) a.n_prev_lines = nullptr;
    hipStream_t pose_stream = ctx->stream;
    if (ctx->overlap) {
        HIP_TRY(ctx, hipEventRecord(ctx->ev_match_done, ctx->stream));
        HIP_TRY(ctx, hipStreamWaitEvent(ctx->aux_stream, ctx->ev_match_done, 0));
        pose_stream = ctx->aux_stream;
    }
    TRY(stvo::launch_pose(pose_stream, a));
    if (ctx->overlap) {
        HIP_TRY(ctx, hipEventRecord(ctx->ev_pose_done, ctx->aux_stream));
        ctx->pose_pending = true;
    }
    return check_launch(ctx);
}

int stvo_optimize_pose_batched_dev(stvo_ctx* ctx, const stvo_track_batch_dev* b, const stvo_cam* cam,
                                   const stvo_opt_params* params) {
    if (!cam || !params) return STVO_ERR_INVALID_ARG;
    TRY(check_batch(ctx, b, false));
    HIP_TRY(ctx, hipSetDevice(ctx->device));
    stvo::PoseArgs a{};
    fill_pose_args(b, cam, params, true, &a);
    TRY(stvo::launch_pose(ctx->stream, a));
    return check_launch(ctx);
}

int stvo_time_stage_dev(stvo_ctx* ctx, const stvo_track_batch_dev* b, const stvo_cam* cam,
                        const stvo_opt_params* params, float nnr, int stage, int iters, float* avg_ms) {
    if (!cam || !params || !avg_ms || iters <= 0) return STVO_ERR_INVALID_ARG;
    TRY(check_batch(ctx, b, true));
    HIP_TRY(ctx, hipSetDevice(ctx->device));
    hipEvent_t e0, e1;
    HIP_TRY(ctx, hipEventCreate(&e0));
    HIP_TRY(ctx, hipEventCreate(&e1));
    stvo::PoseArgs a{};
    fill_pose_args(b, cam, params, false, &a);
    HIP_TRY(ctx, hipEventRecord(e0, ctx->stream));
    const stvo::LazyScratch lw{ctx->knn12, ctx->knn21, ctx->cand, ctx->need, ctx->qsel, ctx->nsel, ctx->knn_capacity};
    for (int it = 0; it < iters; ++it) {
        const int pad = ctx->overlap ? kOverlapLdsPad : 0;
        const int nseg = stvo::knn_pick_nseg(b->B, b->max_pts, ctx->knn_capacity);
        if (stage == 0 || stage == 2) {
            stvo::launch_hamming_knn2(ctx->stream, b->B, b->max_pts, b->max_pts, b->prev_pdesc, b->n_prev_pts,
                                      b->curr_pdesc, b->n_curr_pts, ctx->knn12, ctx->knn21, 0, pad, 0, nullptr, nullptr, nseg);
        } else if (stage == 3) {
            stvo::launch_hamming_verify(ctx->stream, b->B, b->max_pts, b->prev_pdesc, b->n_prev_pts, b->curr_pdesc, nnr, lw,
                                        pad, nseg, b->m12_pts);
        } else if (stage == 4) {
            stvo::launch_hamming_knn2(ctx->stream, b->B, b->max_pts, b->max_pts, b->prev_pdesc, b->n_prev_pts,
                                      b->curr_pdesc, b->n_curr_pts, ctx->knn12, ctx->knn21, 1, pad, 0, nullptr, nullptr, nseg);
        } else
            stvo::launch_pose(ctx->stream, a);
    }
    HIP_TRY(ctx, hipEventRecord(e1, ctx->stream));
    HIP_TRY(ctx, hipEventSynchronize(e1));
    float ms = 0.f;
    HIP_TRY(ctx, hipEventElapsedTime(&ms, e0, e1));
    (void)hipEventDestroy(e0);
    (void)hipEventDestroy(e1);
    *avg_ms = ms / (float)iters;
    if (stage == 1 && stvo::dbg().pose_prof != stvo::DBG_UNSET) {
        long long* dprof = nullptr;
        HIP_TRY(ctx, hipMalloc((void**)&dprof, (size_t)b->B * 16 * sizeof(long long)));
        a.prof_out = dprof;
        stvo::launch_pose(ctx->stream, a);
        std::vector<long long> h((size_t)b->B * 16);
        HIP_TRY(ctx, hipStreamSynchronize(ctx->stream));
        HIP_TRY(ctx, hipMemcpy(h.data(), dprof, h.size() * sizeof(long long), hipMemcpyDeviceToHost));
        double m[16] = {0, 0, 0, 0, 0, 0, 0, 0, 0, 0, 0, 0, 0, 0, 0, 0};
        for (int f = 0; f < b->B; ++f)
            for (int i = 0; i < 16; ++i) m[i] += (double)h[(size_t)f * 16 + i] / b->B;
        std::fprintf(stderr, "[pose prof] mean ticks/frame: evaluate %.0f  iter-algebra %.0f  cov+isgood+commit %.0f  "
                             "remove_outliers %.0f  total %.0f | worker: eval-compute %.0f  barrier+solver-sum %.0f  prefetch+fold %.0f\n", m[0], m[1], m[2], m[3], m[4], m[5], m[6], m[7]);
        std::fprintf(stderr, "[pose prof] per worker wave, compute + fold ticks/frame: %.0f %.0f %.0f %.0f %.0f %.0f | prologue %.0f | last wave %.0f\n", m[8], m[9], m[10],
                     m[11], m[12], m[13], m[14], m[15]);
        (void)hipFree(dprof);
    }
    return check_launch(ctx);
}

int stvo_last_reverse_counts(stvo_ctx* ctx, int B, int32_t* counts) {
    if (!ctx || !counts || B <= 0 || B > ctx->max_batch) return STVO_ERR_INVALID_ARG;
    HIP_TRY(ctx, hipSetDevice(ctx->device));
    HIP_TRY(ctx, hipStreamSynchronize(ctx->stream));
    HIP_TRY(ctx, hipMemcpy(counts, ctx->nsel, (size_t)B * sizeof(int32_t), hipMemcpyDeviceToHost));
    return STVO_OK;
}

int stvo_last_reverse_plan(stvo_ctx* ctx, int B, int32_t* plan) {
    if (!ctx || !plan || B <= 0 || B > ctx->max_batch) return STVO_ERR_INVALID_ARG;
    HIP_TRY(ctx, hipSetDevice(ctx->device));
    HIP_TRY(ctx, hipStreamSynchronize(ctx->stream));
    HIP_TRY(ctx, hipMemcpy(plan, ctx->nsel, (size_t)B * 5 * sizeof(int32_t), hipMemcpyDeviceToHost));
    return STVO_OK;
}

int stvo_ctx_set_kernel_timing(stvo_ctx* ctx, int enable) {
    if (!ctx) return STVO_ERR_INVALID_ARG;
    ctx->timing = enable ? 1 : 0;
    ctx->ev_used = 0;
    return STVO_OK;
}

int stvo_ctx_get_kernel_timing(stvo_ctx* ctx, float* avg_ms_forward, float* avg_ms_reverse, int32_t* n_pairs) {
    if (!ctx || !avg_ms_forward || !avg_ms_reverse || !n_pairs) return STVO_ERR_INVALID_ARG;
    HIP_TRY(ctx, hipSetDevice(ctx->device));
    HIP_TRY(ctx, hipStreamSynchronize(ctx->stream));
    double f = 0.0, r = 0.0;
    int n = 0;
    for (size_t k = 0; k + 4 <= ctx->ev_used; k += 4) {
        float a = 0.f, c = 0.f;
        HIP_TRY(ctx, hipEventElapsedTime(&a, ctx->ev_pool[k], ctx->ev_pool[k + 1]));
        HIP_TRY(ctx, hipEventElapsedTime(&c, ctx->ev_pool[k + 2], ctx->ev_pool[k + 3]));
        f += a;
        r += c;
        ++n;
    }
    *n_pairs = n;
    *avg_ms_forward = n ? (float)(f / n) : 0.f;
    *avg_ms_reverse = n ? (float)(r / n) : 0.f;
    ctx->ev_used = 0;
    return STVO_OK;
}

int stvo_valu_peak_probe(stvo_ctx* ctx, double* lane_ops_per_s) {
    if (!ctx || !lane_ops_per_s) return STVO_ERR_INVALID_ARG;
    HIP_TRY(ctx, hipSetDevice(ctx->device));
    const int blocks = 256 * 8, iters = 4000;
    hipEvent_t e0, e1;
    HIP_TRY(ctx, hipEventCreate(&e0));
    HIP_TRY(ctx, hipEventCreate(&e1));
    stvo::launch_valu_probe(ctx->stream, blocks, 64, ctx->probe_sink);
    HIP_TRY(ctx, hipEventRecord(e0, ctx->stream));
    stvo::launch_valu_probe(ctx->stream, blocks, iters, ctx->probe_sink);
    HIP_TRY(ctx, hipEventRecord(e1, ctx->stream));
    HIP_TRY(ctx, hipEventSynchronize(e1));
    float ms = 0.f;
    HIP_TRY(ctx, hipEventElapsedTime(&ms, e0, e1));
    (void)hipEventDestroy(e0);
    (void)hipEventDestroy(e1);
    *lane_ops_per_s = (double)blocks * 256.0 * (double)iters * stvo::kValuProbeOpsPerThreadIter / ((double)ms * 1e-3);
    return check_launch(ctx);
}

}
```

Before: 1.385 million frame-pairs/s.

## Fuse forward plan into MFMA knn kernel via last-arriving-block counter

Moves the forward-plan logic into a shared device function and lets the MFMA Hamming kNN kernel run it in the last block to finish each batch item, using a per-item arrival counter buffer. This is meant to remove a separate plan kernel launch and the dependency gap between the kNN and plan stages for the mutual lazy match. The plan reuses the kNN kernel's LDS when it fits. The cost is added atomics and fences, plus counter state that has to be reset correctly between calls.

Measured after the change: 596,800 frame-pairs/s. -56.9%, worse.

```diff
diff --git a/stvo-pl_amd/csrc/ctx_internal.h b/stvo-pl_amd/csrc/ctx_internal.h
--- a/stvo-pl_amd/csrc/ctx_internal.h
+++ b/stvo-pl_amd/csrc/ctx_internal.h
@@ -17,6 +17,7 @@
     uint2* knn21 = nullptr;
     size_t knn_capacity = 0;
     int32_t *cand = nullptr, *need = nullptr, *qsel = nullptr, *nsel = nullptr;
+    uint32_t* arrive = nullptr;
     char* arena = nullptr;
     char* arena_host = nullptr;
     size_t arena_size = 0, arena_off = 0, upload_hi = 0;
diff --git a/stvo-pl_amd/csrc/forward_plan.h b/stvo-pl_amd/csrc/forward_plan.h
--- /dev/null
+++ b/stvo-pl_amd/csrc/forward_plan.h
@@ -0,0 +1,165 @@
+#pragma once
+#include <hip/hip_runtime.h>
+#include <stdint.h>
+
+namespace stvo {
+
+__device__ __forceinline__ uint2 merged_knn(const uint2* __restrict__ knn, size_t seg_stride, size_t idx, int nseg) {
+    uint2 r = knn[idx];
+    for (int sgm = 1; sgm < nseg; ++sgm) {
+        const uint2 o = knn[(size_t)sgm * seg_stride + idx];
+        const uint32_t hi = r.x > o.x ? r.x : o.x;
+        uint32_t sec = r.y < o.y ? r.y : o.y;
+        sec = sec < hi ? sec : hi;
+        r.x = r.x < o.x ? r.x : o.x;
+        r.y = sec;
+    }
+    return r;
+}
+
+__device__ __forceinline__ uint32_t block_threshold(uint32_t d0, float nnr) {
+    const float f0 = (float)d0;
+    uint32_t thr = d0;
+    while (thr < 256u && !(f0 < (float)(thr + 1u) * nnr)) ++thr;
+    return thr;
+}
+
+struct ForwardPlanArgs {
+    uint32_t* arrive;
+    float nnr;
+    int32_t* m12;
+    uint32_t* claim_g;
+    int32_t* qsel;
+    int32_t* tsel;
+    int32_t* nsel;
+};
+
+constexpr int PLAN_HIST = 257;
+struct PlanShared {
+    int hT[PLAN_HIST], hS[PLAN_HIST], cnt[3];
+    unsigned long long best;
+};
+__host__ __device__ constexpr size_t plan_lds_bytes(int row_stride) { return (size_t)row_stride * 7; }
+
+template <int BS>
+__device__ __forceinline__ void forward_plan_body(uint32_t* plan_lds, PlanShared& sh, int b, int B, int nseg, int row_stride, uint2* knn12,
+                                                  int na, int nb, float nnr, int32_t* __restrict__ m12, uint32_t* __restrict__ claim_g,
+                                                  int32_t* __restrict__ qsel, int32_t* __restrict__ tsel, int32_t* __restrict__ nsel) {
+    static_assert(BS >= 256 && BS % 64 == 0, "one cost per thread for 256 candidate cuts");
+    uint32_t* claim = plan_lds;
+    uint16_t* Tc = reinterpret_cast<uint16_t*>(claim + row_stride);
+    uint8_t* blk = reinterpret_cast<uint8_t*>(Tc + row_stride);
+    int* hT = sh.hT;
+    int* hS = sh.hS;
+    int* s_cnt = sh.cnt;
+    const int tid = threadIdx.x;
+    const size_t off = (size_t)b * row_stride;
+    for (int j = tid; j < row_stride; j += BS) {
+        claim[j] = 0xFFFFFFFFu;
+        blk[j] = 0;
+    }
+    for (int t = tid; t < PLAN_HIST; t += BS) hT[t] = hS[t] = 0;
+    if (tid < 3) s_cnt[tid] = 0;
+    if (tid == 0) sh.best = ~0ull;
+    __syncthreads();
+    const bool active = nb >= 2 && na >= 1;
+    for (int i = tid; i < row_stride; i += BS) {
+        if (active && i < na) {
+            const uint2 k = merged_knn(knn12, (size_t)B * row_stride, off + i, nseg);
+            if (nseg > 1) knn12[off + i] = k;
+            const float f0 = (float)(k.x >> 16), f1 = (float)(k.y >> 16);
+            if (f0 < f1 * nnr) atomicMin(&claim[k.x & 0xFFFFu], (k.x & 0xFFFF0000u) | (uint32_t)i);
+        }
+        m12[off + i] = -1;
+    }
+    __syncthreads();
+    for (int j = tid; j < row_stride; j += BS) {
+        const uint32_t c = claim[j];
+        claim_g[off + j] = c;
+        if (c != 0xFFFFFFFFu) {
+            const uint32_t T = block_threshold(c >> 16, nnr);
+            Tc[j] = (uint16_t)T;
+            atomicAdd(&hT[T], 1);
+        }
+    }
+    __syncthreads();
+    if (active)
+        for (int i = tid; i < na; i += BS) {
+            const uint2 k = knn12[off + i];
+            const uint32_t key[2] = {k.x, k.y};
+#pragma unroll
+            for (int e = 0; e < 2; ++e) {
+                if (key[e] == 0xFFFFFFFFu) continue;
+                const uint32_t j = key[e] & 0xFFFFu, c = claim[j];
+                if (c != 0xFFFFFFFFu && (c & 0xFFFFu) != (uint32_t)i && (key[e] >> 16) <= (uint32_t)Tc[j]) blk[j] = 1;
+            }
+            if (k.y != 0xFFFFFFFFu) atomicAdd(&hS[min(k.y >> 16, 256u)], 1);
+        }
+    __syncthreads();
+    if (tid < 64) {
+        int vT[5], vS[5], sT = 0, sS = 0;
+#pragma unroll
+        for (int e = 0; e < 5; ++e) {
+            const int t = tid * 5 + e;
+            vT[e] = t < PLAN_HIST ? hT[t] : 0;
+            vS[e] = t < PLAN_HIST ? hS[t] : 0;
+            sT += vT[e];
+            sS += vS[e];
+        }
+        int iT = sT, iS = sS;
+#pragma unroll
+        for (int o = 1; o < 64; o <<= 1) {
+            const int a = __shfl_up(iT, o, 64), c = __shfl_up(iS, o, 64);
+            if (tid >= o) {
+                iT += a;
+                iS += c;
+            }
+        }
+        int eT = iT - sT, eS = iS - sS;
+#pragma unroll
+        for (int e = 0; e < 5; ++e) {
+            const int t = tid * 5 + e;
+            if (t < PLAN_HIST) {
+                hT[t] = eT;
+                hS[t] = eS;
+            }
+            eT += vT[e];
+            eS += vS[e];
+        }
+        if (tid == 63) s_cnt[0] = iT;
+    }
+    __syncthreads();
+    if (tid < 256) {
+        const int C = s_cnt[0], cT = hT[tid], cS = hS[tid];
+        const unsigned long long cost = (unsigned long long)(C - cT) * (unsigned)na + (unsigned long long)cT * (unsigned)cS;
+        atomicMin(&sh.best, (cost << 9) | (unsigned)tid);
+    }
+    __syncthreads();
+    if (tid == 0) s_cnt[0] = 0;
+    __syncthreads();
+    const int tau = (int)(sh.best & 511ull) - 1;
+    for (int j = tid; j < row_stride; j += BS) {
+        const uint32_t c = claim[j];
+        if (c == 0xFFFFFFFFu) continue;
+        if (!blk[j] && na >= 2) m12[off + (c & 0xFFFFu)] = j;
+        if ((int)Tc[j] <= tau)
+            qsel[off + atomicAdd(&s_cnt[0], 1)] = j;
+        else
+            qsel[off + row_stride - 1 - atomicAdd(&s_cnt[1], 1)] = j;
+    }
+    if (active)
+        for (int i = tid; i < na; i += BS) {
+            const uint2 k = knn12[off + i];
+            if (k.y != 0xFFFFFFFFu && (int)(k.y >> 16) <= tau) tsel[off + atomicAdd(&s_cnt[2], 1)] = i;
+        }
+    __syncthreads();
+    if (tid == 0) {
+        nsel[b] = s_cnt[0] + s_cnt[1];
+        nsel[(size_t)B + b] = s_cnt[0];
+        nsel[2 * (size_t)B + b] = s_cnt[1];
+        nsel[3 * (size_t)B + b] = s_cnt[2];
+        nsel[4 * (size_t)B + b] = tau;
+    }
+}
+
+}
diff --git a/stvo-pl_amd/csrc/kernels.h b/stvo-pl_amd/csrc/kernels.h
--- a/stvo-pl_amd/csrc/kernels.h
+++ b/stvo-pl_amd/csrc/kernels.h
@@ -13,6 +13,8 @@
 #include "point_tail.h"
 
 namespace stvo {
+
+struct ForwardPlanArgs;
 
 inline bool lds_opt_in(const void* kernel, int bytes) {
     static std::mutex mu;
@@ -58,7 +60,8 @@
 void launch_hamming_knn2(hipStream_t s, int B, int row_stride, int max_n, const uint8_t* d1, const int32_t* n1,
                          const uint8_t* d2, const int32_t* n2, uint2* knn12, uint2* knn21, int both_directions,
                          int lds_pad_bytes = 0, int dir0 = 0, const int32_t* qsel = nullptr,
-                         const int32_t* nsel = nullptr, int nseg = KNN_MIN_NSEG, uint32_t* claim_init = nullptr);
+                         const int32_t* nsel = nullptr, int nseg = KNN_MIN_NSEG, uint32_t* claim_init = nullptr,
+                         const ForwardPlanArgs* plan = nullptr);
 constexpr int REV_MAX_SEG = 8;
 __host__ __device__ inline int rev_segments(int train_rows) {
     const int s = (train_rows + 255) / 256;
@@ -69,7 +72,9 @@
 void launch_hamming_knn2_mfma(hipStream_t s, int B, int row_stride, int max_n, const uint8_t* d1, const int32_t* n1,
                               const uint8_t* d2, const int32_t* n2, uint2* knn12, uint2* knn21, int both_directions,
                               int dir0, const int32_t* qsel, const int32_t* nsel, int nseg, uint32_t* claim_init, int qb,
-                              int qsel_from_back = 0, const int32_t* tsel = nullptr, const int32_t* ntsel = nullptr);
+                              int qsel_from_back = 0, const int32_t* tsel = nullptr, const int32_t* ntsel = nullptr,
+                              const ForwardPlanArgs* plan = nullptr);
+bool mfma_plan_fits(int qb, int row_stride);
 int knn_mfma_qb(int max_n);
 struct LazyScratch {
     uint2* knn12;
@@ -79,6 +84,7 @@
     int32_t* qsel;
     int32_t* nsel;
     size_t knn_capacity;
+    uint32_t* arrive = nullptr;
 };
 void launch_match_mutual_lazy(hipStream_t s, int B, int row_stride, const uint8_t* d1, const int32_t* n1,
                               const uint8_t* d2, const int32_t* n2, float nnr, const LazyScratch& w, int32_t* m12,
diff --git a/stvo-pl_amd/csrc/match_kernels.hip b/stvo-pl_amd/csrc/match_kernels.hip
--- a/stvo-pl_amd/csrc/match_kernels.hip
+++ b/stvo-pl_amd/csrc/match_kernels.hip
@@ -1,4 +1,5 @@
 #include "kernels.h"
+#include "forward_plan.h"
 
 #include <stdlib.h>
 
@@ -39,19 +40,6 @@
 }
 
 constexpr int KNN_BLOCK = 256;
-
-__device__ __forceinline__ uint2 merged_knn(const uint2* __restrict__ knn, size_t seg_stride, size_t idx, int nseg) {
-    uint2 r = knn[idx];
-    for (int sgm = 1; sgm < nseg; ++sgm) {
-        const uint2 o = knn[(size_t)sgm * seg_stride + idx];
-        const uint32_t hi = r.x > o.x ? r.x : o.x;
-        uint32_t sec = r.y < o.y ? r.y : o.y;
-        sec = sec < hi ? sec : hi;
-        r.x = r.x < o.x ? r.x : o.x;
-        r.y = sec;
-    }
-    return r;
-}
 
 __global__ __launch_bounds__(KNN_BLOCK) void hamming_knn2_kernel(int B, int tiles, int ndir, int dir0, int nseg, int row_stride,
                                                                  const uint8_t* __restrict__ d1,
@@ -124,12 +112,13 @@
 
 void launch_hamming_knn2(hipStream_t s, int B, int row_stride, int max_n, const uint8_t* d1, const int32_t* n1,
                          const uint8_t* d2, const int32_t* n2, uint2* knn12, uint2* knn21, int both_directions,
-                         int lds_pad_bytes, int dir0, const int32_t* qsel, const int32_t* nsel, int nseg, uint32_t* claim_init) {
+                         int lds_pad_bytes, int dir0, const int32_t* qsel, const int32_t* nsel, int nseg, uint32_t* claim_init,
+                         const ForwardPlanArgs* plan) {
     if (B <= 0 || max_n <= 0) return;
     const int mfma_qb = knn_mfma_qb(max_n);
     if (mfma_qb > 0) {
         launch_hamming_knn2_mfma(s, B, row_stride, max_n, d1, n1, d2, n2, knn12, knn21, both_directions, dir0, qsel, nsel, nseg,
-                                 claim_init, mfma_qb);
+                                 claim_init, mfma_qb, 0, nullptr, nullptr, plan);
         return;
     }
     const int tiles = (max_n + KNN_BLOCK - 1) / KNN_BLOCK, ndir = both_directions ? 2 : 1;
@@ -342,135 +331,15 @@
     }
 }
 
-__device__ __forceinline__ uint32_t block_threshold(uint32_t d0, float nnr) {
-    const float f0 = (float)d0;
-    uint32_t thr = d0;
-    while (thr < 256u && !(f0 < (float)(thr + 1u) * nnr)) ++thr;
-    return thr;
-}
-
 constexpr int PLAN_BLOCK = 512;
-__global__ __launch_bounds__(PLAN_BLOCK) void forward_plan_kernel(int B, int nseg, int row_stride, uint2* __restrict__ knn12,
-                                                                  const int32_t* __restrict__ n1,
-                                                                  const int32_t* __restrict__ n2, float nnr,
-                                                                  int32_t* __restrict__ m12, uint32_t* __restrict__ claim_g,
-                                                                  int32_t* __restrict__ qsel, int32_t* __restrict__ tsel,
-                                                                  int32_t* __restrict__ nsel) {
+__global__ __launch_bounds__(PLAN_BLOCK) void forward_plan_kernel(int B, int nseg, int row_stride, uint2* knn12, const int32_t* __restrict__ n1,
+                                                                  const int32_t* __restrict__ n2, float nnr, int32_t* __restrict__ m12,
+                                                                  uint32_t* __restrict__ claim_g, int32_t* __restrict__ qsel,
+                                                                  int32_t* __restrict__ tsel, int32_t* __restrict__ nsel) {
     extern __shared__ uint32_t plan_lds[];
-    uint32_t* claim = plan_lds;
-    uint16_t* Tc = reinterpret_cast<uint16_t*>(claim + row_stride);
-    uint8_t* blk = reinterpret_cast<uint8_t*>(Tc + row_stride);
-    __shared__ int hT[257], hS[257], s_cnt[3];
-    __shared__ unsigned long long s_best;
-    const int b = blockIdx.x, tid = threadIdx.x;
-    const size_t off = (size_t)b * row_stride;
-    const int na = n1[b], nb = n2[b];
-    for (int j = tid; j < row_stride; j += PLAN_BLOCK) {
-        claim[j] = 0xFFFFFFFFu;
-        blk[j] = 0;
-    }
-    if (tid < 257) hT[tid] = hS[tid] = 0;
-    if (tid < 3) s_cnt[tid] = 0;
-    if (tid == 0) s_best = ~0ull;
-    __syncthreads();
-    const bool active = nb >= 2 && na >= 1;
-    for (int i = tid; i < row_stride; i += PLAN_BLOCK) {
-        if (active && i < na) {
-            const uint2 k = merged_knn(knn12, (size_t)B * row_stride, off + i, nseg);
-            if (nseg > 1) knn12[off + i] = k;
-            const float f0 = (float)(k.x >> 16), f1 = (float)(k.y >> 16);
-            if (f0 < f1 * nnr) atomicMin(&claim[k.x & 0xFFFFu], (k.x & 0xFFFF0000u) | (uint32_t)i);
-        }
-        m12[off + i] = -1;
-    }
-    __syncthreads();
-    for (int j = tid; j < row_stride; j += PLAN_BLOCK) {
-        const uint32_t c = claim[j];
-        claim_g[off + j] = c;
-        if (c != 0xFFFFFFFFu) {
-            const uint32_t T = block_threshold(c >> 16, nnr);
-            Tc[j] = (uint16_t)T;
-            atomicAdd(&hT[T], 1);
-        }
-    }
-    __syncthreads();
-    if (active)
-        for (int i = tid; i < na; i += PLAN_BLOCK) {
-            const uint2 k = knn12[off + i];
-            const uint32_t key[2] = {k.x, k.y};
-#pragma unroll
-            for (int e = 0; e < 2; ++e) {
-                if (key[e] == 0xFFFFFFFFu) continue;
-                const uint32_t j = key[e] & 0xFFFFu, c = claim[j];
-                if (c != 0xFFFFFFFFu && (c & 0xFFFFu) != (uint32_t)i && (key[e] >> 16) <= (uint32_t)Tc[j]) blk[j] = 1;
-            }
-            if (k.y != 0xFFFFFFFFu) atomicAdd(&hS[min(k.y >> 16, 256u)], 1);
-        }
-    __syncthreads();
-    if (tid < 64) {
-        int vT[5], vS[5], sT = 0, sS = 0;
-#pragma unroll
-        for (int e = 0; e < 5; ++e) {
-            const int t = tid * 5 + e;
-            vT[e] = t < 257 ? hT[t] : 0;
-            vS[e] = t < 257 ? hS[t] : 0;
-            sT += vT[e];
-            sS += vS[e];
-        }
-        int iT = sT, iS = sS;
-#pragma unroll
-        for (int o = 1; o < 64; o <<= 1) {
-            const int a = __shfl_up(iT, o, 64), c = __shfl_up(iS, o, 64);
-            if (tid >= o) {
-                iT += a;
-                iS += c;
-            }
-        }
-        int eT = iT - sT, eS = iS - sS;
-#pragma unroll
-        for (int e = 0; e < 5; ++e) {
-            const int t = tid * 5 + e;
-            if (t < 257) {
-                hT[t] = eT;
-                hS[t] = eS;
-            }
-            eT += vT[e];
-            eS += vS[e];
-        }
-        if (tid == 63) s_cnt[0] = iT;
-    }
-    __syncthreads();
-    if (tid < 256) {
-        const int C = s_cnt[0], cT = hT[tid], cS = hS[tid];
-        const unsigned long long cost = (unsigned long long)(C - cT) * (unsigned)na + (unsigned long long)cT * (unsigned)cS;
-        atomicMin(&s_best, (cost << 9) | (unsigned)tid);
-    }
-    __syncthreads();
-    if (tid == 0) s_cnt[0] = 0;
-    __syncthreads();
-    const int tau = (int)(s_best & 511ull) - 1;
-    for (int j = tid; j < row_stride; j += PLAN_BLOCK) {
-        const uint32_t c = claim[j];
-        if (c == 0xFFFFFFFFu) continue;
-        if (!blk[j] && na >= 2) m12[off + (c & 0xFFFFu)] = j;
-        if ((int)Tc[j] <= tau)
-            qsel[off + atomicAdd(&s_cnt[0], 1)] = j;
-        else
-            qsel[off + row_stride - 1 - atomicAdd(&s_cnt[1], 1)] = j;
-    }
-    if (active)
-        for (int i = tid; i < na; i += PLAN_BLOCK) {
-            const uint2 k = knn12[off + i];
-            if (k.y != 0xFFFFFFFFu && (int)(k.y >> 16) <= tau) tsel[off + atomicAdd(&s_cnt[2], 1)] = i;
-        }
-    __syncthreads();
-    if (tid == 0) {
-        nsel[b] = s_cnt[0] + s_cnt[1];
-        nsel[(size_t)B + b] = s_cnt[0];
-        nsel[2 * (size_t)B + b] = s_cnt[1];
-        nsel[3 * (size_t)B + b] = s_cnt[2];
-        nsel[4 * (size_t)B + b] = tau;
-    }
+    __shared__ PlanShared sh;
+    const int b = blockIdx.x;
+    forward_plan_body<PLAN_BLOCK>(plan_lds, sh, b, B, nseg, row_stride, knn12, n1[b], n2[b], nnr, m12, claim_g, qsel, tsel, nsel);
 }
 
 struct ReversePlan {
@@ -512,21 +381,29 @@
     const int nseg = knn_pick_nseg(B, row_stride, w.knn_capacity);
     uint32_t* claim = reinterpret_cast<uint32_t*>(w.need);
     int32_t* blocked = reinterpret_cast<int32_t*>(w.knn21);
-    if (tev) (void)hipEventRecord(tev[0], s);
-    launch_hamming_knn2(s, B, row_stride, row_stride, d1, n1, d2, n2, w.knn12, w.knn21, 0, lds_pad_bytes, 0, nullptr,
-                        nullptr, nseg, knn_mfma_qb(row_stride) > 0 ? nullptr : claim);
-    if (tev) (void)hipEventRecord(tev[1], s);
     const int mfma_qb = knn_mfma_qb(row_stride);
     if (mfma_qb > 0) {
         const ReversePlan rp = reverse_plan(w, B, row_stride);
-        if (wait_before_m12_write) (void)hipStreamWaitEvent(s, wait_before_m12_write, 0);
+        const bool fused = w.arrive != nullptr && mfma_plan_fits(mfma_qb, row_stride);
+        const ForwardPlanArgs pa{w.arrive, nnr, m12, claim, w.qsel, rp.tsel, w.nsel};
+        if (fused && wait_before_m12_write) (void)hipStreamWaitEvent(s, wait_before_m12_write, 0);
+        if (tev) (void)hipEventRecord(tev[0], s);
+        launch_hamming_knn2(s, B, row_stride, row_stride, d1, n1, d2, n2, w.knn12, w.knn21, 0, lds_pad_bytes, 0, nullptr, nullptr, nseg,
+                            nullptr, fused ? &pa : nullptr);
+        if (tev) (void)hipEventRecord(tev[1], s);
+        if (!fused && wait_before_m12_write) (void)hipStreamWaitEvent(s, wait_before_m12_write, 0);
         if (tev && tev[2]) (void)hipEventRecord(tev[2], s);
-        hipLaunchKernelGGL(forward_plan_kernel, dim3(B), dim3(PLAN_BLOCK), (size_t)row_stride * 7, s, B, nseg, row_stride, w.knn12,
-                           n1, n2, nnr, m12, claim, w.qsel, rp.tsel, w.nsel);
+        if (!fused)
+            hipLaunchKernelGGL(forward_plan_kernel, dim3(B), dim3(PLAN_BLOCK), plan_lds_bytes(row_stride), s, B, nseg, row_stride, w.knn12,
+                               n1, n2, nnr, m12, claim, w.qsel, rp.tsel, w.nsel);
         launch_reverse_scans(s, B, row_stride, d1, n1, d2, nnr, w, rp, m12);
         if (tev && tev[3]) (void)hipEventRecord(tev[3], s);
         return;
     }
+    if (tev) (void)hipEventRecord(tev[0], s);
+    launch_hamming_knn2(s, B, row_stride, row_stride, d1, n1, d2, n2, w.knn12, w.knn21, 0, lds_pad_bytes, 0, nullptr, nullptr, nseg,
+                        claim);
+    if (tev) (void)hipEventRecord(tev[1], s);
     hipLaunchKernelGGL(nnr_forward_kernel, grid2, dim3(256), 0, s, nseg, row_stride, w.knn12, n1, n2, nnr, w.cand, claim);
     hipLaunchKernelGGL(compact_need_kernel, dim3(B), dim3(256), 0, s, row_stride, claim, n2, w.qsel, w.nsel, blocked);
     if (tev && tev[2]) (void)hipEventRecord(tev[2], s);
diff --git a/stvo-pl_amd/csrc/match_mfma.hip b/stvo-pl_amd/csrc/match_mfma.hip
--- a/stvo-pl_amd/csrc/match_mfma.hip
+++ b/stvo-pl_amd/csrc/match_mfma.hip
@@ -1,6 +1,7 @@
 #include <type_traits>
 
 #include "kernels.h"
+#include "forward_plan.h"
 
 namespace stvo {
 
@@ -71,7 +72,7 @@
                                                                       const int32_t* __restrict__ nsel,
                                                                       uint32_t* __restrict__ claim_init, int qsel_from_back,
                                                                       const int32_t* __restrict__ tsel,
-                                                                      const int32_t* __restrict__ ntsel) {
+                                                                      const int32_t* __restrict__ ntsel, ForwardPlanArgs plan) {
     constexpr bool GATHER = MODE >= 1, TGATHER = MODE == 2;
     constexpr int ROWS = 4 * QB * 32;
     constexpr int KSTEPS = 4;
@@ -82,18 +83,7 @@
     const int per_frame = tiles * ndir * nseg;
     const int L = blockIdx.x;
     const int xcd = L & 7, k = L >> 3;
-    int fb = k / per_frame, local = k % per_frame;
-    if (MODE == 0 && ndir == 1 && tiles > 1) {
-        const int groups = (int)(gridDim.x >> 3) / per_frame;
-        const int full_pf = (tiles - 1) * nseg, full = full_pf * groups;
-        if (k < full) {
-            fb = k / full_pf;
-            local = k % full_pf;
-        } else {
-            fb = (k - full) / nseg;
-            local = full_pf + (k - full) % nseg;
-        }
-    }
+    const int fb = k / per_frame, local = k % per_frame;
     const int b = fb * 8 + xcd;
     if (b >= B) return;
     const int seg = local % nseg;
@@ -121,27 +111,30 @@
     const int nt = min(j0 + seg_len, nt_all);
     if (claim_init && seg == 0 && dir == dir0)
         for (int c = q_base + tid; c < min(q_base + ROWS, row_stride); c += MF_BLOCK) claim_init[frame_off + c] = 0xFFFFFFFFu;
-    if (q_base >= nq) return;
+    const bool has_rows = q_base < nq;
     const uint32_t* __restrict__ T = reinterpret_cast<const uint32_t*>((dir == 0 ? d2 : d1) + frame_off * STVO_DESC_BYTES);
     uint2* __restrict__ out = (dir == 0 ? knn12 : knn21) + (size_t)seg * B * row_stride + frame_off;
 
-    const bool wave_active = q_base + wv * QB * 32 < nq;
-    v4i qf[QB][KSTEPS];
+    auto scan = [&](auto nb_c) {
+    constexpr int NB = decltype(nb_c)::value;
+    const int blk0 = wv * NB;
+    const bool wave_active = q_base + blk0 * 32 < nq;
+    v4i qf[NB][KSTEPS];
     auto query_row = [&](int qb) {
-        const int q = q_base + (wv * QB + qb) * 32 + col;
+        const int q = q_base + (blk0 + qb) * 32 + col;
         const int qc = q < nq ? q : nq - 1;
         return GATHER ? qsel[frame_off + (qsel_from_back ? row_stride - 1 - qc : qc)] : qc;
     };
-    if (GATHER) {
-#pragma unroll
-        for (int qb = 0; qb < QB; ++qb) {
+    if (GATHER || NB != QB) {
+#pragma unroll
+        for (int qb = 0; qb < NB; ++qb) {
             const int qi = query_row(qb);
             qw[qb][0] = reinterpret_cast<const uint4*>(Q)[2 * qi];
             qw[qb][1] = reinterpret_cast<const uint4*>(Q)[2 * qi + 1];
         }
     }
 #pragma unroll
-    for (int qb = 0; qb < QB; ++qb) {
+    for (int qb = 0; qb < NB; ++qb) {
         const uint32_t w[8] = {qw[qb][0].x, qw[qb][0].y, qw[qb][0].z, qw[qb][0].w, qw[qb][1].x, qw[qb][1].y, qw[qb][1].z, qw[qb][1].w};
         const bool up = hf != 0;
         qf[qb][0] = expand_fp4(~(up ? w[1] : w[0]));
@@ -154,9 +147,9 @@
     for (int r = 0; r < 16; ++r) cidx[r] = (key_t)((r & 3) + 8 * (r >> 2) + 4 * hf);
 
     const key_t no_key = MF_NO_KEY_F;
-    key_t best[QB], second[QB];
-#pragma unroll
-    for (int qb = 0; qb < QB; ++qb) best[qb] = second[qb] = no_key;
+    key_t best[NB], second[NB];
+#pragma unroll
+    for (int qb = 0; qb < NB; ++qb) best[qb] = second[qb] = no_key;
 
     const int xr = tid & 31, xk = tid >> 5;
     const int ntiles = (nt - j0 + MF_TILE - 1) / MF_TILE;
@@ -175,7 +168,7 @@
     __syncthreads();
     auto rebase = [&]() {
 #pragma unroll
-        for (int qb = 0; qb < QB; ++qb) {
+        for (int qb = 0; qb < NB; ++qb) {
             best[qb] -= (key_t)MF_TILE;
             second[qb] -= (key_t)MF_TILE;
         }
@@ -188,23 +181,23 @@
         const v8i a8 = {tf.x, tf.y, tf.z, tf.w, 0, 0, 0, 0}, b8 = {q.x, q.y, q.z, q.w, 0, 0, 0, 0};
         return __builtin_amdgcn_mfma_scale_f32_32x32x64_f8f6f4(a8, b8, c, 4, 4, 0, MF_SCALE_2_4, 0, MF_SCALE_2_4);
     };
-    auto mma_fold = [&](acc_t (&cur)[QB], acc_t (&prev)[QB], int t) {
+    auto mma_fold = [&](acc_t (&cur)[NB], acc_t (&prev)[NB], int t) {
         if (wave_active) {
             const v4i* frag = s_tile[t & (NBUF - 1)];
             const bool fold_prev = t > 0;
             if (fold_prev) rebase();
-            key_t node[QB][5];
+            key_t node[NB][5];
             v4i tf = frag[lane];
 #pragma unroll
             for (int kk = 0; kk < KSTEPS; ++kk) {
                 v4i tf_ahead = tf;
                 if (kk < KSTEPS - 1) tf_ahead = frag[(kk + 1) * 64 + lane];
 #pragma unroll
-                for (int qb = 0; qb < QB; ++qb) cur[qb] = mma(tf, qf[qb][kk], kk == 0 ? cidx : cur[qb]);
+                for (int qb = 0; qb < NB; ++qb) cur[qb] = mma(tf, qf[qb][kk], kk == 0 ? cidx : cur[qb]);
                 if (fold_prev) {
-                    if (QB == 1 && kk == 0) asm volatile("s_nop 7\n\ts_nop 7\n\ts_nop 2" : "+v"(prev[0]));
-#pragma unroll
-                    for (int qb = 0; qb < QB; ++qb) {
+                    if (NB == 1 && kk == 0) asm volatile("s_nop 7\n\ts_nop 7\n\ts_nop 2" : "+v"(prev[0]));
+#pragma unroll
+                    for (int qb = 0; qb < NB; ++qb) {
                         const acc_t& p = prev[qb];
                         key_t(&a)[5] = node[qb];
                         if (kk == 0) {
@@ -229,7 +222,7 @@
                 }
                 if (kk < KSTEPS - 1) __builtin_amdgcn_sched_group_barrier(0x100, 1, 0);
 #pragma unroll
-                for (int qb = 0; qb < QB; ++qb) {
+                for (int qb = 0; qb < NB; ++qb) {
                     __builtin_amdgcn_sched_group_barrier(0x008, 1, 0);
                     __builtin_amdgcn_sched_group_barrier(0x002, MF_FOLD_SLOTS, 0);
                 }
@@ -237,9 +230,9 @@
             }
         }
     };
-    acc_t accA[QB], accB[QB];
-#pragma unroll
-    for (int qb = 0; qb < QB; ++qb)
+    acc_t accA[NB], accB[NB];
+#pragma unroll
+    for (int qb = 0; qb < NB; ++qb)
 #pragma unroll
         for (int r = 0; r < 16; ++r) accA[qb][r] = accB[qb][r] = 0;
     static_assert(MF_TPB % 2 == 0, "the accumulator sets alternate tile by tile");
@@ -277,10 +270,10 @@
         }
     if (wave_active && ntiles > 0) {
         const int jt = j0 + (ntiles - 1) * MF_TILE;
-        const acc_t(&last)[QB] = (ntiles & 1) ? accA : accB;
+        const acc_t(&last)[NB] = (ntiles & 1) ? accA : accB;
         rebase();
 #pragma unroll
-        for (int qb = 0; qb < QB; ++qb)
+        for (int qb = 0; qb < NB; ++qb)
 #pragma unroll
             for (int r = 0; r < 16; ++r) {
                 const int jr = jt + (r & 3) + 8 * (r >> 2) + 4 * hf;
@@ -289,16 +282,42 @@
     }
     if (!wave_active) return;
 #pragma unroll
-    for (int qb = 0; qb < QB; ++qb) {
+    for (int qb = 0; qb < NB; ++qb) {
         const int bi = best[qb] >= MF_NO_KEY_MIN_F ? MF_NO_KEY : (int)best[qb];
         const int si = second[qb] >= MF_NO_KEY_MIN_F ? MF_NO_KEY : (int)second[qb];
         const int ob = __shfl_xor(bi, 32), os = __shfl_xor(si, 32);
         const int hi = max(bi, ob);
         const int sec = min(min(si, os), hi);
         const int bst = min(bi, ob);
-        const int q = q_base + (wv * QB + qb) * 32 + col;
+        const int q = q_base + (blk0 + qb) * 32 + col;
         const int base = j0 + (ntiles - 1) * MF_TILE;
         if (hf == 0 && q < nq) out[query_row(qb)] = make_uint2(key_to_knn(bst, base), key_to_knn(sec, base));
+    }
+    };
+    if (has_rows) {
+        if constexpr (MODE == 0 && QB > 1) {
+            if (nq - q_base <= 4 * 32) scan(std::integral_constant<int, 1>{});
+            else scan(std::integral_constant<int, QB>{});
+        } else {
+            scan(std::integral_constant<int, QB>{});
+        }
+    }
+    if constexpr (MODE == 0) {
+        if (plan.arrive != nullptr) {
+            __shared__ PlanShared s_plan;
+            __shared__ uint32_t s_arrived;
+            __builtin_amdgcn_fence(__ATOMIC_RELEASE, "agent");
+            __syncthreads();
+            if (tid == 0) s_arrived = __hip_atomic_fetch_add(&plan.arrive[b], 1u, __ATOMIC_ACQ_REL, __HIP_MEMORY_SCOPE_AGENT);
+            __syncthreads();
+            if (s_arrived == (uint32_t)(tiles * nseg) - 1u) {
+                __builtin_amdgcn_fence(__ATOMIC_ACQUIRE, "agent");
+                if (tid == 0) __hip_atomic_store(&plan.arrive[b], 0u, __ATOMIC_RELAXED, __HIP_MEMORY_SCOPE_AGENT);
+                static_assert(sizeof(s_tile) >= plan_lds_bytes(2048), "the plan of a 2048-row slot runs in the tile buffers");
+                forward_plan_body<MF_BLOCK>(reinterpret_cast<uint32_t*>(&s_tile[0][0]), s_plan, b, B, nseg, row_stride, knn12, na, nb, plan.nnr,
+                                            plan.m12, plan.claim_g, plan.qsel, plan.tsel, plan.nsel);
+            }
+        }
     }
 }
 
@@ -494,25 +513,30 @@
 }
 
 int mfma_rows_per_block(int qb) { return 4 * qb * 32; }
+bool mfma_plan_fits(int qb, int row_stride) {
+    return qb > 0 && plan_lds_bytes(row_stride) <= (size_t)(2 * MF_TPB) * 4 * 2 * 32 * sizeof(v4i);
+}
 
 template <int QB, int MODE>
 static void launch_mf(dim3 grid, hipStream_t s, int B, int tiles, int ndir, int dir0, int nseg, int row_stride, const uint8_t* d1,
                       const int32_t* n1, const uint8_t* d2, const int32_t* n2, uint2* knn12, uint2* knn21, const int32_t* qsel,
-                      const int32_t* nsel, uint32_t* claim_init, int qsel_from_back, const int32_t* tsel, const int32_t* ntsel) {
+                      const int32_t* nsel, uint32_t* claim_init, int qsel_from_back, const int32_t* tsel, const int32_t* ntsel,
+                      const ForwardPlanArgs& plan) {
     hipLaunchKernelGGL((hamming_knn2_mfma_kernel<QB, MODE>), grid, dim3(MF_BLOCK), 0, s, B, tiles, ndir, dir0, nseg, row_stride, d1, n1, d2, n2,
-                       knn12, knn21, qsel, nsel, claim_init, qsel_from_back, tsel, ntsel);
+                       knn12, knn21, qsel, nsel, claim_init, qsel_from_back, tsel, ntsel, plan);
 }
 
 void launch_hamming_knn2_mfma(hipStream_t s, int B, int row_stride, int max_n, const uint8_t* d1, const int32_t* n1,
                               const uint8_t* d2, const int32_t* n2, uint2* knn12, uint2* knn21, int both_directions,
                               int dir0, const int32_t* qsel, const int32_t* nsel, int nseg, uint32_t* claim_init, int qb,
-                              int qsel_from_back, const int32_t* tsel, const int32_t* ntsel) {
+                              int qsel_from_back, const int32_t* tsel, const int32_t* ntsel, const ForwardPlanArgs* plan) {
     if (B <= 0 || max_n <= 0) return;
+    const ForwardPlanArgs pa = plan ? *plan : ForwardPlanArgs{};
     const int rows = mfma_rows_per_block(qb);
     const int tiles = (max_n + rows - 1) / rows, ndir = both_directions ? 2 : 1;
     const int groups = (B + 7) / 8;
     const dim3 grid((unsigned)(groups * 8 * tiles * ndir * nseg));
-#define STVO_MF_ARGS grid, s, B, tiles, ndir, dir0, nseg, row_stride, d1, n1, d2, n2, knn12, knn21, qsel, nsel, claim_init, qsel_from_back, tsel, ntsel
+#define STVO_MF_ARGS grid, s, B, tiles, ndir, dir0, nseg, row_stride, d1, n1, d2, n2, knn12, knn21, qsel, nsel, claim_init, qsel_from_back, tsel, ntsel, pa
     if (qsel || tsel) return;
     if (qb == 1) launch_mf<1, 0>(STVO_MF_ARGS);
     else if (qb == 2) launch_mf<2, 0>(STVO_MF_ARGS);
diff --git a/stvo-pl_amd/csrc/seq_pipeline.hip b/stvo-pl_amd/csrc/seq_pipeline.hip
--- a/stvo-pl_amd/csrc/seq_pipeline.hip
+++ b/stvo-pl_amd/csrc/seq_pipeline.hip
@@ -712,7 +712,8 @@
     const size_t cap_l = nb * (size_t)M * 4;
     const size_t o_cover_l = c.take(nb * (size_t)(M / 64) * M * 8), o_top2_l = c.take(nb * M * 8), o_owner_l = c.take(nb * M * 4),
                  o_knn12_l = c.take(cap_l * 8), o_knn21_l = c.take(cap_l * 8), o_cand_l = c.take(nb * M * 4),
-                 o_need_l = c.take(nb * M * 4), o_qsel_l = c.take(nb * M * 4), o_nsel_l = c.take(nb * 4 * 5);
+                 o_need_l = c.take(nb * M * 4), o_qsel_l = c.take(nb * M * 4), o_nsel_l = c.take(nb * 4 * 5),
+                 o_arrive_l = c.take(nb * 4);
     size_t o_set[3][14];
     for (int t = 0; t < 3; ++t) {
         o_set[t][0] = c.take(nb * K * 16);
@@ -792,7 +793,7 @@
     s->cover_l = (unsigned long long*)(D + o_cover_l); s->top2_l = (unsigned long long*)(D + o_top2_l);
     s->owner2_l = (int32_t*)(D + o_owner_l);
     s->lazy_l = stvo::LazyScratch{(uint2*)(D + o_knn12_l), (uint2*)(D + o_knn21_l), (int32_t*)(D + o_cand_l), (int32_t*)(D + o_need_l),
-                                  (int32_t*)(D + o_qsel_l), (int32_t*)(D + o_nsel_l), cap_l};
+                                  (int32_t*)(D + o_qsel_l), (int32_t*)(D + o_nsel_l), cap_l, (uint32_t*)(D + o_arrive_l)};
     s->m12s_p = (int32_t*)(D + o_m12sp); s->m12s_l = (int32_t*)(D + o_m12sl);
     s->m12p = (int32_t*)(D + o_m12p); s->m12l = (int32_t*)(D + o_m12l);
     s->inlp = (int32_t*)(D + o_inlp); s->inll = (int32_t*)(D + o_inll);
@@ -1163,7 +1164,7 @@
     TRY(line_stage());
     const bool track = fl.track;
     if (track) {
-        const stvo::LazyScratch w{ctx->knn12, ctx->knn21, ctx->cand, ctx->need, ctx->qsel, ctx->nsel, ctx->knn_capacity};
+        const stvo::LazyScratch w{ctx->knn12, ctx->knn21, ctx->cand, ctx->need, ctx->qsel, ctx->nsel, ctx->knn_capacity, ctx->arrive};
         const int esm = stvo::dbg().match_small;
         const int lines_cap = std::max(s->set_lines_cap[s->cur], s->set_lines_cap[s->prev_set()]);
         const bool small_sets = esm != stvo::DBG_UNSET ? esm != 0 : lines_cap <= 128;
diff --git a/stvo-pl_amd/csrc/stvo_capi.hip b/stvo-pl_amd/csrc/stvo_capi.hip
--- a/stvo-pl_amd/csrc/stvo_capi.hip
+++ b/stvo-pl_amd/csrc/stvo_capi.hip
@@ -108,6 +108,8 @@
          hip_ok(ctx, hipMalloc((void**)&ctx->need, knn_elems * sizeof(int32_t)), "hipMalloc need") &&
          hip_ok(ctx, hipMalloc((void**)&ctx->qsel, knn_elems * sizeof(int32_t)), "hipMalloc qsel") &&
          hip_ok(ctx, hipMalloc((void**)&ctx->nsel, (size_t)max_batch * 5 * sizeof(int32_t)), "hipMalloc nsel") &&
+         hip_ok(ctx, hipMalloc((void**)&ctx->arrive, (size_t)max_batch * sizeof(uint32_t)), "hipMalloc arrive") &&
+         zero_device(ctx, ctx->arrive, (size_t)max_batch * sizeof(uint32_t), "hipMemset arrive") &&
          hip_ok(ctx, hipMalloc((void**)&ctx->arena, ctx->arena_size), "hipMalloc arena") &&
          hip_ok(ctx, hipHostMalloc((void**)&ctx->arena_host, ctx->arena_size, hipHostMallocDefault), "hipHostMalloc") &&
          hip_ok(ctx, hipMalloc((void**)&ctx->probe_sink, 256), "hipMalloc sink");
@@ -129,6 +131,7 @@
     if (ctx->need) (void)hipFree(ctx->need);
     if (ctx->qsel) (void)hipFree(ctx->qsel);
     if (ctx->nsel) (void)hipFree(ctx->nsel);
+    if (ctx->arrive) (void)hipFree(ctx->arrive);
     if (ctx->arena) (void)hipFree(ctx->arena);
     if (ctx->arena_host) (void)hipHostFree(ctx->arena_host);
     if (ctx->probe_sink) (void)hipFree(ctx->probe_sink);
@@ -210,7 +213,7 @@
     TRY(flush_uploads(ctx));
     TRY(upload(ctx, &dm12, (const int32_t*)nullptr, (size_t)stride));
     if (mutual) {
-        const stvo::LazyScratch w{ctx->knn12, ctx->knn21, ctx->cand, ctx->need, ctx->qsel, ctx->nsel, ctx->knn_capacity};
+        const stvo::LazyScratch w{ctx->knn12, ctx->knn21, ctx->cand, ctx->need, ctx->qsel, ctx->nsel, ctx->knn_capacity, ctx->arrive};
         stvo::launch_match_mutual_lazy(ctx->stream, 1, stride, dd1, dn1, dd2, dn2, nnr, w, dm12, 0, nullptr);
     } else {
         const int nseg = stvo::knn_pick_nseg(1, stride, ctx->knn_capacity);
@@ -239,7 +242,7 @@
         return STVO_ERR_CAPACITY;
     HIP_TRY(ctx, hipSetDevice(ctx->device));
     if (mutual) {
-        const stvo::LazyScratch w{ctx->knn12, ctx->knn21, ctx->cand, ctx->need, ctx->qsel, ctx->nsel, ctx->knn_capacity};
+        const stvo::LazyScratch w{ctx->knn12, ctx->knn21, ctx->cand, ctx->need, ctx->qsel, ctx->nsel, ctx->knn_capacity, ctx->arrive};
         stvo::launch_match_mutual_lazy(ctx->stream, B, row_stride, d1, n1, d2, n2, nnr, w, m12, 0, nullptr);
     } else {
         const int nseg = stvo::knn_pick_nseg(B, row_stride, ctx->knn_capacity);
@@ -422,7 +425,7 @@
     if (b->B == 0) return STVO_OK;
     const int pad = ctx->overlap ? kOverlapLdsPad : 0;
     hipEvent_t prev_pose = (ctx->overlap && ctx->pose_pending) ? ctx->ev_pose_done : nullptr;
-    const stvo::LazyScratch w{ctx->knn12, ctx->knn21, ctx->cand, ctx->need, ctx->qsel, ctx->nsel, ctx->knn_capacity};
+    const stvo::LazyScratch w{ctx->knn12, ctx->knn21, ctx->cand, ctx->need, ctx->qsel, ctx->nsel, ctx->knn_capacity, ctx->arrive};
     auto match_set = [&](int stride, const uint8_t* da, const int32_t* na, const uint8_t* db, const int32_t* nb,
                          float nnr, int32_t* m12) {
         if (mutual) {
@@ -492,7 +495,7 @@
     stvo::PoseArgs a{};
     fill_pose_args(b, cam, params, false, &a);
     HIP_TRY(ctx, hipEventRecord(e0, ctx->stream));
-    const stvo::LazyScratch lw{ctx->knn12, ctx->knn21, ctx->cand, ctx->need, ctx->qsel, ctx->nsel, ctx->knn_capacity};
+    const stvo::LazyScratch lw{ctx->knn12, ctx->knn21, ctx->cand, ctx->need, ctx->qsel, ctx->nsel, ctx->knn_capacity, ctx->arrive};
     for (int it = 0; it < iters; ++it) {
         const int pad = ctx->overlap ? kOverlapLdsPad : 0;
         const int nseg = stvo::knn_pick_nseg(b->B, b->max_pts, ctx->knn_capacity);
```
